# privacy-scaling-explorations/zkevm-specs

Measured on AMD Instinct MI355X. Metric: BN254 constraint-rows/sec, higher is better.
Workload: dtype u256 (BN254 Fr: 4xu64 canonical cells, u32-limb Montgomery); 1 GPU; EVM circuit, 2^18 execution steps per GPU, mixed-opcode synthetic trace (BASELINE configs[2]); RW table 816377 rows, bytecode table 43913 rows; steps_per_gpu=262144, rw_rows=816377, bytecode_rows=43913, witness_copies=3

## Files before the change

### zkevm_specs_amd/csrc/cpu_backend.cpp

```cpp
#include <stdio.h>
#include <string.h>
#include <chrono>
#include <functional>
#include <string>
#include <vector>

#include "../../include/zkevm_hip.h"
#include "dist_tally.hpp"
#include "state_circuit.hpp"
#include "evm_circuit.hpp"
#include "host_index.hpp"
#include "row_circuits.hpp"
#include "copy_circuit.hpp"
#include "sign_circuit.hpp"
#include "keccak_table.hpp"
#include "secp256k1.hpp"
#include "pi_circuit.hpp"
#include "state_assign.hpp"
#include "bytecode_assign.hpp"
#include "state_rekey.hpp"
#include "ecc_circuit.hpp"
#include "withdrawal_circuit.hpp"
#include "tx_assign.hpp"
#include "sig_assign.hpp"
// ... 42 lines not shown
    std::function<u32(u64)> row;
    std::vector<u32> status;
    u32 launches = 0;
    double ms = 0;
    u64 fail_count = 0, first_row = ~0ull;
    u32 first_code = 0;
    bool range_ok = false;
    bool range_may_be_empty = false;
    std::vector<u64> a64[4];
    std::vector<u32> a32[4];
    std::vector<uint8_t> a8, a8b;
    std::vector<uint16_t> a16;
    std::vector<u64> w64[4];
    std::vector<u32> out32;
    void (*pass)(zk_session*) = nullptr;
    int assign_kind = 0;
    u64 n_ops = 0;
    std::vector<u32> rekey_plan;
    std::vector<u32> rekey_jobs;
    u64 n_mpt = 0;
    CpuTable tab[12];
    std::vector<u64> keccak_rows;
    StateArgs state;
    EvmArgs evm;
    BytecodeArgs bytecode;
    ExpArgs exp;
    CopyArgs copy;
    SignArgs sign;
    PiArgs pi;
    PiCopyArgs picopy;
    AssignArgs assign;
    BcaArgs bca;
    std::vector<BcaChunk> bca_chunks;
    std::vector<uint8_t> bca_map;
    CpaArgs cpa;
    CpaPlan cpa_plan;
    EcdsaArgs ecdsa;
    KeccakGenArgs kgen;
    TxAssignArgs txa;
    SigAssignArgs sga;
    std::vector<u64> sga64[8];
    std::vector<u32> sga32[3];
    u64 n_sig_rows = 0;
    ExaArgs exa;
    ExaSizes exa_sizes;
    PiaArgs pia;
    PiaSizes pia_sizes;
    KeccakGenArgs pia_kgen;
    EccArgs ecc_assign;
    std::vector<u64> pia64[20];
    std::vector<u32> pia32[6];
    std::vector<uint8_t> pia8[4];
    std::vector<u64> txa_out64[4];
    std::vector<u32> txa_out32[3];
    u64 n_keccak = 0;
    ZkRwMeta rw_meta;
    HostCodeDir dir;
    std::vector<u64> aux64;
    bool status_external = false;
};

static void run_pass(zk_session* s, u32* status_out) {
    const auto t0 = std::chrono::steady_clock::now();
    u32* st = status_out ? status_out : s->status.data();
    const long long lo = (long long)s->lo, hi = (long long)s->hi;
    if (s->pass) {
        s->pass(s);
        if (status_out) memcpy(status_out, s->status.data(), s->n * sizeof(u32));
    } else {
#pragma omp parallel for schedule(dynamic, 256)
        for (long long i = lo; i < hi; i++) st[i] = s->row((u64)i);
    }
    u64 fails = 0, first = ~0ull;
    for (long long i = lo; i < hi; i++)
        if (st[i]) {
            if (!fails) first = (u64)i;
            fails++;
        }
    s->fail_count = fails;
    s->first_row = first;
    s->first_code = fails ? st[first] : 0u;
    s->ms += std::chrono::duration<double, std::milli>(std::chrono::steady_clock::now() - t0).count();
    s->launches++;
}
extern "C" int zk_launch(zk_session* s, uint32_t* status_dev) {
    ARG_TRY(s, "zk_launch: null session");
    s->status_external = status_dev != nullptr;
    run_pass(s, status_dev);
    return 0;
}
extern "C" int zk_collect(zk_session* s, zk_result* r) {
    ARG_TRY(s && r, "zk_collect: bad arguments");
    r->fail_count = s->fail_count;
    r->first_fail_row = s->first_row == ~0ull ? UINT64_MAX : s->first_row;
    r->first_fail_code = s->first_code;
    r->launches = s->launches;
    r->rows_evaluated = s->hi - s->lo;
    r->kernel_ms = s->launches ? s->ms / s->launches : 0.0;
    s->launches = 0;
    s->ms = 0;
    return 0;
}
extern "C" int zk_read_status(zk_session* s, uint32_t* status_host) {
    ARG_TRY(s && status_host, "zk_read_status: bad arguments");
    ARG_TRY(!s->status_external, "zk_read_status: the last pass wrote its statuses to the caller's status_dev buffer, not the session's");
    memcpy(status_host, s->status.data(), s->n * sizeof(u32));
    return 0;
}
extern "C" int zk_close(zk_session* s) {
    delete s;
    return 0;
}
extern "C" int zk_session_set_stream(zk_session*, void*) { return 0; }
extern "C" int zk_session_timing(zk_session*, double* open_ms, double* span_ms) {
    if (open_ms) *open_ms = -1.0;
    if (span_ms) *span_ms = -1.0;
    return 0;
}
struct zk_comm {
    int rank = 0, world = 1;
    void* nccl = nullptr;
    std::vector<uint64_t> buf;
};
#define RCCL_TRY(expr, what)                                                                                                                   \
    do {                                                                                                                                       \
        const int r_ = (expr);                                                                                                                 \
        if (r_ != 0) {                                                                                                                         \
            char buf_[256];                                                                                                                    \
            snprintf(buf_, sizeof buf_, "%s: RCCL error %d (%s)", what, r_, zkdist::rccl().GetErrorString ? zkdist::rccl().GetErrorString(r_) : "?"); \
            g_err = buf_;                                                                                                                      \
            return -3;                                                                                                                         \
        }                                                                                                                                      \
    } while (0)
static bool host_collective() { return getenv("ZK_RCCL_LIB") && zkdist::rccl().ok && zkdist::rccl().named_by_env && zkdist::rccl().buffers == 0; }
extern "C" int zk_dist_unique_id(uint8_t* id) {
    ARG_TRY(id, "zk_dist_unique_id: id is null");
    memset(id, 0, ZK_DIST_ID_BYTES);
    if (host_collective()) {
        zkdist::RcclId u;
        RCCL_TRY(zkdist::rccl().GetUniqueId(&u), "ncclGetUniqueId");
        memcpy(id, u.internal, ZK_DIST_ID_BYTES);
    }
    return 0;
}
extern "C" int zk_dist_close(zk_comm* c) {
    if (c && c->nccl) (void)zkdist::rccl().CommDestroy(c->nccl);
    delete c;
    return 0;
}
extern "C" int zk_dist_init(const uint8_t* id, int rank, int world, zk_comm** out) {
    ARG_TRY(id && out && world >= 1 && rank >= 0 && rank < world, "zk_dist_init: bad arguments");
    ARG_TRY(world == 1 || host_collective(),
            "zk_dist_init: the CPU backend has no collective of its own (world must be 1, or ZK_RCCL_LIB must name a library that gathers host buffers); reduce on the host");
    zk_comm* c = new zk_comm();
    c->rank = rank;
    c->world = world;
    c->buf.assign((size_t)(world + 1) * zkdist::TALLY_WORDS, 0);
    if (world > 1) {
        zkdist::RcclId u;
        memcpy(u.internal, id, ZK_DIST_ID_BYTES);
        if (int r = zkdist::rccl().CommInitRank(&c->nccl, world, u, rank)) {
            char buf[256];
            snprintf(buf, sizeof buf, "ncclCommInitRank: RCCL error %d", r);
            g_err = buf;
            c->nccl = nullptr;
            zk_dist_close(c);
            return -3;
        }
    }
    *out = c;
    return 0;
}
extern "C" int zk_dist_tally(zk_comm* c, const zk_result* local, uint64_t row_offset, zk_result* global) {
    ARG_TRY(c && local && global, "zk_dist_tally: bad arguments");
    uint64_t* mine = c->buf.data();
    uint64_t* all = mine + zkdist::TALLY_WORDS;
    zkdist::tally_pack(mine, local, row_offset);
    if (c->world == 1) memcpy(all, mine, zkdist::TALLY_WORDS * sizeof(uint64_t));
    else RCCL_TRY(zkdist::rccl().AllGather(mine, all, zkdist::TALLY_WORDS, zkdist::RCCL_UINT64, c->nccl, nullptr), "ncclAllGather");
    zkdist::tally_reduce(all, c->world, local, global);
    return 0;
}
extern "C" int zk_last_host_phases(double* us4) {
    if (us4) for (int k = 0; k < 4; k++) us4[k] = -1.0;
    return 0;
}
extern "C" int zk_timing_sums(double* sums_ms, uint64_t* count, int) {
    if (sums_ms) for (int k = 0; k < 3; k++) sums_ms[k] = -1.0;
    if (count) *count = 0;
    return 0;
}
extern "C" int zk_last_timing(double* open_ms, double* pass_ms, double* span_ms) {
    if (open_ms) *open_ms = -1.0;
    if (pass_ms) *pass_ms = -1.0;
    if (span_ms) *span_ms = -1.0;
    return 0;
}
extern "C" int zk_set_range(zk_session* s, uint64_t row_lo, uint64_t row_hi) {
    ARG_TRY(s && s->range_ok, "zk_set_range: not a row-circuit session");
    ARG_TRY((row_lo < row_hi || (s->range_may_be_empty && row_lo == row_hi)) && row_hi <= s->n, "zk_set_range: bad range");
    s->lo = row_lo;
    s->hi = row_hi;
    std::fill(s->status.begin(), s->status.end(), 0u);
    return 0;
}
extern "C" int zk_state_set_range(zk_session* s, uint64_t row_lo, uint64_t row_hi) { return zk_set_range(s, row_lo, row_hi); }

static zk_session* new_session(u64 n, bool range_ok) {
    zk_session* s = new zk_session();
    s->n = n;
    s->lo = 0;
    s->hi = n;
    s->status.assign(n ? n : 1, 0u);
    s->range_ok = range_ok;
    return s;
}
static int one_shot(zk_session* s, uint32_t* status_out, zk_result* result) {
    int rc = zk_launch(s, nullptr);
    if (!rc) rc = zk_collect(s, result);
    if (!rc && status_out) rc = zk_read_status(s, status_out);
    zk_close(s);
    return rc;
}
#define NO_DEVICE_PTRS(opts, name) ARG_TRY(!((opts) & ZK_OPT_DEVICE_PTRS), name ": ZK_OPT_DEVICE_PTRS has no meaning on the CPU backend")
#ifndef ZK_OPT_STATE_COMPACT
#define ZK_OPT_STATE_COMPACT 32u
#endif

extern "C" int zk_fr_op(int op, const uint64_t* a, const uint64_t* b, uint64_t* out, uint64_t n, uint32_t opts) {
    NO_DEVICE_PTRS(opts, "zk_fr_op");
    ARG_TRY(a && b && out, "zk_fr_op: null pointer");
    ARG_TRY(op < 19 || op > 25 || n % 12 == 0, "zk_fr_op 19..25: n must be a multiple of 12");
#pragma omp parallel for
    for (long long i = 0; i < (long long)n; i++) {
        const Fr x = fr_load(a + 4 * i), y = fr_load(b + 4 * i);
        Fr r;
        switch (op) {
        case 0: r = fr_add(x, y); break;
        case 1: r = fr_sub(x, y); break;
        case 2: r = fr_mul(x, y); break;
        case 3: r = fr_mont(x, y); break;
        case 4: r = fr_neg(x); break;
        case 5: r = fr_inv(x); break;
        case 6: r = fr_div(x, y); break;
        case 18: r = ecc_fq_mul_hook(x, y); break;
        case 26: r = sp_sqrt_p(x); break;
        case 27: r = sp_inv_p(x); break;
        case 19: case 20: case 21: case 22: case 23: case 24: case 25:
            if (i % 12 == 0 && i + 12 <= (long long)n) ecc_fq12_op_hook(op, a + 4 * i, b + 4 * i, out + 4 * i);
            continue;
        default: r = fr_zero();
        }
        for (int k = 0; k < 4; k++) out[4 * i + k] = (u64)r.v[2 * k] | ((u64)r.v[2 * k + 1] << 32);
    }
    return 0;
}

extern "C" int zk_state_open(const uint64_t* rows, const uint32_t* flags, uint64_t n, const uint64_t* mpt, uint64_t n_mpt,
                             uint32_t opts, zk_session** out) {
    NO_DEVICE_PTRS(opts, "zk_state_open");
    ARG_TRY(out && rows && n > 0 && n < (1ull << 32) && n_mpt < (1ull << 31), "zk_state_open: bad arguments");
    zk_session* s = new_session(n, true);
    const bool compact = opts & ZK_OPT_STATE_COMPACT;
    s->a64[0].assign(rows, rows + n * (compact ? 15 : ST_NCELLS) * 4);
    s->state.rows.skip = compact ? 42u : 0u;
    if (flags) s->a32[0].assign(flags, flags + n);
    else s->a32[0].assign(n, 0u);
    cpu_table(s->tab[0], mpt, nullptr, n_mpt, MPT_NCELLS, nullptr);
    {
        CpuTable& h = s->tab[0];
        for (u32 r = 0; r < (u32)n_mpt; r++) {
            const u64 hv = state_mpt_key_hash(h.t, r);
            u32 k = (u32)hv & h.t.mask;
            while (h.slots[k] != ZK_EMPTY_SLOT) k = (k + 1) & h.t.mask;
            h.slots[k] = state_mpt_slot_value(h.t, r, hv);
        }
    }
    s->state.rows.cells = s->a64[0].data();
    s->state.rows.flags = s->a32[0].data();
    s->state.rows.n = n;
    s->state.mpt = s->tab[0].t;
    s->state.eval_lo = 0;
    s->state.eval_hi = n;
    s->row = [s](u64 i) { return state_check_row(s->state, i); };
    *out = s;
    return 0;
}
extern "C" int zk_state_verify(const uint64_t* rows, const uint32_t* flags, uint64_t n, const uint64_t* mpt, uint64_t n_mpt,
                               uint32_t opts, uint32_t* status_out, zk_result* result) {
    ARG_TRY(result, "zk_state_verify: result is null");
    zk_session* s = nullptr;
    const int rc = zk_state_open(rows, flags, n, mpt, n_mpt, opts, &s);
    return rc ? rc : one_shot(s, status_out, result);
}

extern "C" int zk_evm_open(const zk_evm_tables* t, uint32_t opts, zk_session** out) {
    NO_DEVICE_PTRS(opts, "zk_evm_open");
    ARG_TRY(t && out && t->steps && t->n_steps >= 2 && t->n_steps < (1ull << 32), "zk_evm_open: bad arguments");
    ARG_TRY(t->aux_cells == 0 || (t->aux_cells >= 2 && t->aux_cells <= 64), "zk_evm_open: aux_cells must be 0 (= 2) or 2..64");
    zk_session* s = new_session(t->n_steps - 1, false);
    EvmArgs& a = s->evm;
    s->a64[0].assign(t->steps, t->steps + t->n_steps * STEP_NCELLS * 4);
    a.dyn = nullptr;
    a.step_recs = nullptr;
    a.defer_list = nullptr;
    a.defer_count = nullptr;
    a.steps = s->a64[0].data();
    a.n_steps = t->n_steps;
    cpu_table(s->tab[0], t->rw, t->rw_flags, t->n_rw, RW_NCELLS, rw_key_hash);
    cpu_table(s->tab[1], t->bytecode, nullptr, t->n_bytecode, BYTECODE_NCELLS, bc_key_hash);
    cpu_table(s->tab[2], t->tx, t->tx_flags, t->n_tx, TX_NCELLS, tx_key_hash);
    cpu_table(s->tab[3], t->block, t->block_flags, t->n_block, BLOCK_NCELLS, blk_key_hash);
    cpu_table(s->tab[4], t->copy, nullptr, t->n_copy, COPY_T_NCELLS, copy_key_hash);
    cpu_table(s->tab[5], t->keccak, nullptr, t->n_keccak, KECCAK_NCELLS, keccak_key_hash);
    cpu_table(s->tab[6], t->exp, nullptr, t->n_exp, EXP_T_NCELLS, expt_key_hash);
    cpu_table(s->tab[7], t->sig, nullptr, t->n_sig, SIG_T_NCELLS, sig_key_hash);
    cpu_table(s->tab[8], t->ecc, nullptr, t->n_ecc, ECC_T_NCELLS, ecc_key_hash);
    cpu_table(s->tab[9], t->withdrawals, nullptr, t->n_withdrawals, 4, nullptr);
    a.rw = s->tab[0].t; a.bytecode = s->tab[1].t; a.tx = s->tab[2].t; a.block = s->tab[3].t; a.copy = s->tab[4].t;
    a.keccak = s->tab[5].t; a.exp = s->tab[6].t; a.sig = s->tab[7].t; a.ecc = s->tab[8].t; a.withdrawals = s->tab[9].t;
    {
        const HostEvmAgg g = evm_aggregates_host(t->tx, t->tx_flags, t->n_tx, t->withdrawals, t->n_withdrawals);
        a.agg_max_txs = g.max_txs; a.agg_total_txs = g.total_txs; a.agg_invalid_txs = g.invalid_txs;
        a.agg_bad_invalid_rows = g.bad_invalid_rows; a.agg_total_wds = g.total_wds;
        a.agg_rw_dups = rw_duplicate_rows_host(t->rw, t->n_rw);
    }
    a.aux = nullptr;
    a.aux_kind = nullptr;
    a.aux_cells = t->aux_cells ? t->aux_cells : 2u;
    if (t->aux && t->aux_kind) {
        s->aux64.assign(t->aux, t->aux + t->n_steps * a.aux_cells * 4);
        s->a32[1].assign(t->aux_kind, t->aux_kind + t->n_steps);
        a.aux = s->aux64.data();
        a.aux_kind = s->a32[1].data();
    }
    a.perm = nullptr;
    a.prof = nullptr;
    a.n_pairs = (u32)(t->n_steps - 1);
    a.opts = (t->begin_with_first_step ? 1u : 0u) | (t->end_with_last_step ? 2u : 0u);
    a.rw_dense = 0;
    a.rw_base = 0;
    a.rw_keys = nullptr;
    a.codes.n = 0;
    a.codes.mask = 0;
    a.codes.packed = nullptr;
    a.codes.entries = nullptr;
    a.codes.slots = nullptr;
    if (!(opts & ZK_OPT_GENERIC_INDEX)) {
        s->rw_meta = rw_dense_meta_host(s->tab[0].t.n ? s->tab[0].cells.data() : nullptr, t->n_rw);
        a.rw_dense = s->rw_meta.dense;
        a.rw_base = s->rw_meta.base;
        if (s->rw_meta.dense) {
            s->a64[1].resize((size_t)t->n_rw * 4);
            for (u64 r = 0; r < t->n_rw; r++) {
                const RwKey k = rw_pack_row(a.rw, (u32)r);
                for (int j = 0; j < 4; j++) s->a64[1][4 * r + j] = k.w[j];
            }
            a.rw_keys = s->a64[1].data();
        }
        if (t->n_bytecode) {
            build_code_dir(s->tab[1].cells.data(), t->n_bytecode, s->dir);
            a.codes.entries = s->dir.entries.data();
            a.codes.slots = s->dir.slots.data();
            a.codes.mask = s->dir.mask;
            a.codes.n = (u32)s->dir.entries.size();
            a.codes.packed = s->dir.packed.data();
        }
    }
    s->row = [s](u64 i) {
        u32 c = evm_check_step<EVM_GROUP_ALL>(s->evm, i);
        if (c == ZK_NOT_MINE) c = evm_check_step<EVM_GROUP_WARM>(s->evm, i);
        if (c == ZK_NOT_MINE) c = evm_check_step<EVM_GROUP_COLD>(s->evm, i);
        return c;
    };
    *out = s;
    return 0;
}
extern "C" int zk_evm_verify(const zk_evm_tables* t, uint32_t opts, uint32_t* status_out, zk_result* result) {
    ARG_TRY(result, "zk_evm_verify: result is null");
    zk_session* s = nullptr;
    const int rc = zk_evm_open(t, opts, &s);
    return rc ? rc : one_shot(s, status_out, result);
}

extern "C" int zk_evm_verify_batch(const zk_evm_tables* const* t, uint64_t n, uint32_t opts, zk_result* results) {
    ARG_TRY((t && results) || n == 0, "zk_evm_verify_batch: bad arguments");
    for (uint64_t i = 0; i < n; i++) ARG_TRY(t[i], "zk_evm_verify_batch: null witness");
    for (uint64_t i = 0; i < n; i++) {
        const int rc = zk_evm_verify(t[i], opts, nullptr, &results[i]);
        if (rc) return rc;
    }
    return 0;
}

extern "C" int zk_bytecode_open(const uint64_t* rows, uint64_t n, const uint64_t* keccak, uint64_t n_keccak, const uint64_t* randomness,
                                uint32_t opts, zk_session** out) {
    NO_DEVICE_PTRS(opts, "zk_bytecode_open");
    ARG_TRY(out && rows && randomness && n > 0 && n < (1ull << 32) && n_keccak < (1ull << 31), "zk_bytecode_open: bad arguments");
    zk_session* s = new_session(n, true);
    s->a64[0].assign(rows, rows + n * BC_NCELLS * 4);
    cpu_table(s->tab[0], keccak, nullptr, n_keccak, KECCAK_NCELLS, keccak_key_hash);
    s->bytecode.rows.cells = s->a64[0].data();
    s->bytecode.rows.flags = nullptr;
    s->bytecode.rows.n = n;
    s->bytecode.keccak = s->tab[0].t;
    s->bytecode.r = cell_of(randomness);
    s->bytecode.r_mont = nullptr;
    s->row = [s](u64 i) { return bytecode_check_row(s->bytecode, i); };
    *out = s;
    return 0;
}
extern "C" int zk_bytecode_verify(const uint64_t* rows, uint64_t n, const uint64_t* keccak, uint64_t n_keccak, const uint64_t* randomness,
                                  uint32_t opts, uint32_t* status_out, zk_result* result) {
    ARG_TRY(result, "zk_bytecode_verify: result is null");
    zk_session* s = nullptr;
    const int rc = zk_bytecode_open(rows, n, keccak, n_keccak, randomness, opts, &s);
    return rc ? rc : one_shot(s, status_out, result);
}
extern "C" int zk_exp_open(const uint64_t* rows, uint64_t n, uint32_t opts, zk_session** out) {
    NO_DEVICE_PTRS(opts, "zk_exp_open");
    ARG_TRY(out && rows && n > 0 && n < (1ull << 32), "zk_exp_open: bad arguments");
    zk_session* s = new_session(n, true);
    s->a64[0].assign(rows, rows + n * EX_NCELLS * 4);
    s->exp.rows.cells = s->a64[0].data();
    s->exp.rows.flags = nullptr;
    s->exp.rows.n = n;
    s->row = [s](u64 i) { return exp_check_row(s->exp, i); };
    *out = s;
    return 0;
}
extern "C" int zk_exp_verify(const uint64_t* rows, uint64_t n, uint32_t opts, uint32_t* status_out, zk_result* result) {
    ARG_TRY(result, "zk_exp_verify: result is null");
    zk_session* s = nullptr;
    const int rc = zk_exp_open(rows, n, opts, &s);
    return rc ? rc : one_shot(s, status_out, result);
}

extern "C" int zk_copy_open(const zk_copy_tables* t, uint32_t opts, zk_session** out) {
    NO_DEVICE_PTRS(opts, "zk_copy_open");
    ARG_TRY(t && out && t->rows && t->randomness && t->n_rows > 0 && t->n_rows < (1ull << 32), "zk_copy_open: bad arguments");
    zk_session* s = new_session(t->n_rows, true);
    s->a64[0].assign(t->rows, t->rows + t->n_rows * CP_NCELLS * 4);
    if (t->row_flags) s->a32[0].assign(t->row_flags, t->row_flags + t->n_rows);
    cpu_table(s->tab[0], t->rw, t->rw_flags, t->n_rw, RW_NCELLS, rw_key_hash);
    cpu_table(s->tab[1], t->bytecode, nullptr, t->n_bytecode, BYTECODE_NCELLS, bc_key_hash);
    cpu_table(s->tab[2], t->tx, t->tx_flags, t->n_tx, TX_NCELLS, tx_key_hash);
    s->copy.rows.cells = s->a64[0].data();
    s->copy.rows.flags = t->row_flags ? s->a32[0].data() : nullptr;
    s->copy.rows.n = t->n_rows;
    s->copy.rw = s->tab[0].t;
    s->copy.bytecode = s->tab[1].t;
    s->copy.tx = s->tab[2].t;
    s->rw_meta = rw_dense_meta_host(t->n_rw ? s->tab[0].cells.data() : nullptr, t->n_rw);
    s->copy.rw_meta = (opts & ZK_OPT_GENERIC_INDEX) ? nullptr : &s->rw_meta;
    s->copy.r = cell_of(t->randomness);
    s->row = [s](u64 i) { return copy_check_row(s->copy, i); };
    *out = s;
    return 0;
}
extern "C" int zk_copy_verify(const zk_copy_tables* t, uint32_t opts, uint32_t* status_out, zk_result* result) {
    ARG_TRY(result, "zk_copy_verify: result is null");
    zk_session* s = nullptr;
    const int rc = zk_copy_open(t, opts, &s);
    return rc ? rc : one_shot(s, status_out, result);
}

extern "C" int zk_sign_open(const zk_sign_units* t, uint32_t opts, zk_session** out) {
    NO_DEVICE_PTRS(opts, "zk_sign_open");
    ARG_TRY(t && out && t->bytes && t->cells && t->meta && t->randomness && t->n_units > 0 && t->n_units < (1ull << 32), "zk_sign_open: bad arguments");
    const u64 n = t->n_units;
    zk_session* s = new_session(n, true);
    s->a8.assign(t->bytes, t->bytes + n * SG_NBYTES_ROWS * 32);
    s->a64[0].assign(t->cells, t->cells + n * SG_NCELLS * 4);
    s->a32[0].assign(t->meta, t->meta + n * 4);
    cpu_table(s->tab[0], t->keccak, nullptr, t->n_keccak, KECCAK_NCELLS, keccak_key_hash);
    cpu_table(s->tab[1], t->tx_rows, t->tx_flags, t->n_tx_rows, TX_NCELLS, nullptr);
    SignArgs& a = s->sign;
    a.bytes = s->a8.data();
    a.cells.cells = s->a64[0].data();
    a.cells.flags = nullptr;
    a.cells.n = n;
    a.meta = s->a32[0].data();
    a.keccak = s->tab[0].t;
    a.tx_rows = s->tab[1].t;
    a.tx_rows.n = (u32)t->n_tx_rows;
    a.r = cell_of(t->randomness);
    s->a64[1].resize(64 * 4);
    sign_fill_rpow(a.r, s->a64[1].data());
    a.rpow = s->a64[1].data();
    a.is_sig = t->is_sig ? 1u : 0u;
    s->row = [s](u64 i) { return sign_check_unit(s->sign, i); };
    *out = s;
    return 0;
}
extern "C" int zk_sign_verify(const zk_sign_units* t, uint32_t opts, uint32_t* status_out, zk_result* result) {
    ARG_TRY(result, "zk_sign_verify: result is null");
    zk_session* s = nullptr;
    const int rc = zk_sign_open(t, opts, &s);
    return rc ? rc : one_shot(s, status_out, result);
}

extern "C" int zk_pi_open(const uint64_t* rows, uint64_t n, const uint64_t* keccak, uint64_t n_keccak, const uint64_t* gas, uint64_t n_gas,
                          uint64_t circuit_len, const uint64_t* keccak_rand, const uint64_t* byte_pow_base, uint32_t opts, zk_session** out) {
    NO_DEVICE_PTRS(opts, "zk_pi_open");
    ARG_TRY(out && rows && keccak_rand && byte_pow_base && n > 0 && n < (1ull << 32), "zk_pi_open: bad arguments");
    zk_session* s = new_session(n, true);
    s->a64[0].assign(rows, rows + n * 24 * 4);
    cpu_table(s->tab[0], keccak, nullptr, n_keccak, KECCAK_NCELLS, keccak_key_hash);
    cpu_table(s->tab[1], gas, nullptr, n_gas, PI_GAS_NCELLS, pi_gas_key_hash);
    PiArgs& a = s->pi;
    a.rows.cells = s->a64[0].data();
    a.rows.flags = nullptr;
    a.rows.n = n;
    a.keccak = s->tab[0].t;
    a.gas = s->tab[1].t;
    a.keccak_rand_m = fr_to_mont(cell_of(keccak_rand));
    a.byte_pow_base_m = fr_to_mont(cell_of(byte_pow_base));
    a.circuit_len = fr_from_u64(circuit_len);
    s->row = [s](u64 i) { return pi_check_row(s->pi, i); };
    *out = s;
    return 0;
}
extern "C" int zk_pi_verify(const uint64_t* rows, uint64_t n, const uint64_t* keccak, uint64_t n_keccak, const uint64_t* gas, uint64_t n_gas,
                            uint64_t circuit_len, const uint64_t* keccak_rand, const uint64_t* byte_pow_base, uint32_t opts,
                            uint32_t* status_out, zk_result* result) {
    ARG_TRY(result, "zk_pi_verify: result is null");
    zk_session* s = nullptr;
    const int rc = zk_pi_open(rows, n, keccak, n_keccak, gas, n_gas, circuit_len, keccak_rand, byte_pow_base, opts, &s);
    return rc ? rc : one_shot(s, status_out, result);
}

extern "C" int zk_pi_copy_open(const uint64_t* cells, const uint8_t* bytes, const uint32_t* lens, uint64_t n, uint32_t opts, zk_session** out) {
    NO_DEVICE_PTRS(opts, "zk_pi_copy_open");
    ARG_TRY(out && cells && bytes && lens && n > 0 && n < (1ull << 32), "zk_pi_copy_open: bad arguments");
    zk_session* s = new_session(n, false);
    s->a64[0].assign(cells, cells + n * 4);
    s->a8.assign(bytes, bytes + n * 32);
    s->a32[0].assign(lens, lens + n);
    s->picopy.cells = s->a64[0].data();
    s->picopy.bytes = s->a8.data();
    s->picopy.lens = s->a32[0].data();
    s->picopy.n = n;
    s->row = [s](u64 i) { return pi_copy_check(s->picopy, i); };
    *out = s;
    return 0;
}
extern "C" int zk_pi_copy_verify(const uint64_t* cells, const uint8_t* bytes, const uint32_t* lens, uint64_t n, uint32_t opts, uint32_t* status_out,
                                 zk_result* result) {
    ARG_TRY(result, "zk_pi_copy_verify: result is null");
    zk_session* s = nullptr;
    const int rc = zk_pi_copy_open(cells, bytes, lens, n, opts, &s);
    return rc ? rc : one_shot(s, status_out, result);
}

extern "C" int zk_keccak_open(const uint8_t* data, uint64_t n_bytes, const uint64_t* offsets, uint64_t n_msgs, const uint64_t* randomness,
                              uint32_t mode, uint64_t* rows_dev, uint32_t opts, zk_session** out) {
    NO_DEVICE_PTRS(opts, "zk_keccak_open");
    ARG_TRY(out && offsets && randomness && n_msgs > 0 && n_msgs < (1ull << 32) && (data || n_bytes == 0) && mode <= 1u && !rows_dev,
            "zk_keccak_open: bad arguments");
    for (u64 k = 0; k < n_msgs; k++) ARG_TRY(offsets[k] <= offsets[k + 1], "zk_keccak_open: offsets must be non-decreasing");
    ARG_TRY(offsets[n_msgs] <= n_bytes, "zk_keccak_open: offsets exceed the data buffer");
    zk_session* s = new_session(n_msgs, false);
    s->a8.assign(data, data + n_bytes);
    s->a64[0].assign(offsets, offsets + n_msgs + 1);
    s->a64[1].resize(KT_RPOW_ROWS * 4);
    kt_fill_rpow(cell_of(randomness), s->a64[1].data());
    s->keccak_rows.assign(n_msgs * KT_NCELLS * 4, 0);
    KeccakGenArgs& g = s->kgen;
    g.data = s->a8.data();
    g.offsets = s->a64[0].data();
    g.n = n_msgs;
    g.rpow = s->a64[1].data();
    g.rows = s->keccak_rows.data();
    g.mode = mode;
    g.long_list = nullptr;
    g.long_count = nullptr;
    s->row = [s](u64 i) { return keccak_table_row(s->kgen, i); };
    *out = s;
    return 0;
}
extern "C" int zk_keccak_read_rows(zk_session* s, uint64_t* rows_host) {
    ARG_TRY(s && rows_host && !s->keccak_rows.empty(), "zk_keccak_read_rows: bad arguments");
    memcpy(rows_host, s->keccak_rows.data(), s->keccak_rows.size() * 8);
    return 0;
}
extern "C" int zk_keccak_table(const uint8_t* data, uint64_t n_bytes, const uint64_t* offsets, uint64_t n_msgs, const uint64_t* randomness,
                               uint32_t mode, uint64_t* rows_out, uint32_t opts, uint32_t* status_out, zk_result* result) {
    ARG_TRY(result && rows_out, "zk_keccak_table: null output");
    zk_session* s = nullptr;
    int rc = zk_keccak_open(data, n_bytes, offsets, n_msgs, randomness, mode, nullptr, opts, &s);
    if (rc) return rc;
    rc = zk_launch(s, nullptr);
    if (!rc) rc = zk_collect(s, result);
    if (!rc) rc = zk_keccak_read_rows(s, rows_out);
    if (!rc && status_out) rc = zk_read_status(s, status_out);
    zk_close(s);
    return rc;
}

extern "C" int zk_ecdsa_open_batches(const zk_ecdsa_batch* bt, uint32_t n_batches, uint32_t opts, zk_session** out) {
    NO_DEVICE_PTRS(opts, "zk_ecdsa_open_batches");
    ARG_TRY(out && bt && (n_batches == 1 || n_batches == 2), "zk_ecdsa_open_batches: one or two batches");
    u64 n = 0;
    for (u32 k = 0; k < n_batches; k++) {
        ARG_TRY(bt[k].bytes && bt[k].n > 0 && bt[k].n < (1ull << 31) && bt[k].layout <= 2u && (!bt[k].v || bt[k].v_stride >= 1) && !bt[k].out_dev,
                "zk_ecdsa_open: bad arguments");
// ... 1056 lines not shown
```

### zkevm_specs_amd/csrc/evm_circuit.hpp

```cpp
#pragma once
#include "common.hpp"
#include "evm_tables.h"
#include "keccak.hpp"
#include "secp_constants.h"
#include "bigz.hpp"

enum { S_STATE = 0, S_RWC, S_CALL_ID, S_IS_ROOT, S_IS_CREATE, S_CH_LO, S_CH_HI, S_PC, S_SP, S_GAS, S_MWS, S_REV, S_LOG, STEP_NCELLS };
enum { R_RWC = 0, R_RW, R_TAG, R_ID, R_ADDR, R_FT, R_KEY_LO, R_KEY_HI, R_VAL_LO, R_VAL_HI, R_PREV_LO, R_PREV_HI, R_AUX_LO, R_AUX_HI, RW_NCELLS };
enum { B_HASH_LO = 0, B_HASH_HI, B_TAG, B_INDEX, B_IS_CODE, B_VALUE, BYTECODE_NCELLS };
enum { TX_NCELLS = 5, BLOCK_NCELLS = 4 };
enum { CT_IS_FIRST = 0, CT_SRC_ID_LO, CT_SRC_ID_HI, CT_SRC_TAG, CT_DST_ID_LO, CT_DST_ID_HI, CT_DST_TAG, CT_SRC_ADDR,
       CT_SRC_ADDR_END, CT_DST_ADDR, CT_LENGTH, CT_RLC_ACC, CT_RWC, CT_RWC_INC, COPY_T_NCELLS };
enum { XT_IS_STEP = 0, XT_ID, XT_IS_LAST, XT_BASE0, XT_BASE1, XT_BASE2, XT_BASE3, XT_EXP_LO, XT_EXP_HI, XT_RES_LO, XT_RES_HI,
       EXP_T_NCELLS };
enum { SIG_T_NCELLS = 9, ECC_T_NCELLS = 13 };
enum { AUX_PAIR = 3, AUX_ECRECOVER = 5, AUX_ECADD = 6, AUX_ECMUL = 7, AUX_ECPAIRING = 8 };
enum { CDT_Bytecode = 1, CDT_Memory, CDT_TxCalldata, CDT_TxLog, CDT_RlcAcc };

struct EvmDyn {
    u32 rw_sparse;
    u32 codes_n;
    u64 rw_base;
    u32 codes_mask;
    u32 agg_max_txs, agg_total_txs, agg_invalid_txs, agg_bad_invalid_rows, agg_total_wds;
    u32 dir_entries;
    u32 n_deferred;
    u32 agg_rw_dups;
};

struct EvmArgs {
    const EvmDyn* dyn;
    const u64* steps;
    const u32* step_recs;
    u64 n_steps;
    ZkTable rw, bytecode, tx, block;
    ZkTable copy, keccak, exp;
    ZkTable sig, ecc;
    ZkTable withdrawals;
    u32 agg_max_txs, agg_total_txs, agg_invalid_txs, agg_bad_invalid_rows, agg_total_wds;
    u32 agg_rw_dups;
    const u64* aux;
    const u32* aux_kind;
    u32 aux_cells;
    u32 rw_dense;
    u64 rw_base;
    const u64* rw_keys;
    ZkCodeDir codes;
    unsigned long long* prof;
    u32* defer_list;
    u32* defer_count;
    const u32* perm;
    u32 n_pairs;
    u32 opts;
    u32* defer_count_twin;
};

ZK_HD void evm_args_resolve(EvmArgs& a) {
#ifdef EVM_RESOLVE_OFF
    return;
#endif
    if (a.dyn) {
        const EvmDyn d = *a.dyn;
        a.rw_dense = (a.rw.n != 0u && d.rw_sparse == 0u) ? 1u : 0u;
        a.rw_base = d.rw_base;
        a.codes.n = d.codes_n;
        a.codes.mask = d.codes_mask;
        a.agg_max_txs = d.agg_max_txs; a.agg_total_txs = d.agg_total_txs; a.agg_invalid_txs = d.agg_invalid_txs;
        a.agg_bad_invalid_rows = d.agg_bad_invalid_rows; a.agg_total_wds = d.agg_total_wds;
        a.agg_rw_dups = d.agg_rw_dups;
    }
}

#ifndef EVM_HOT_BLOCK
#define EVM_HOT_BLOCK 128
#endif
#define EVM_STAGE_LANES EVM_HOT_BLOCK
#define EV_PROF_WAVE ((blockIdx.x * blockDim.x + threadIdx.x) >> 6)
#define EV_PROF_ON(a) ((a).prof && (threadIdx.x & 63) == 0 && EV_PROF_WAVE < 4096u)
#define EVM_STAGE_STRIDE (EVM_STAGE_LANES + 1)
#define EVM_STAGE_ENTRIES 40
#define EVM_STAGE_GAS 10
ZK_HD constexpr int evm_stage_entry(int s, int c) {
    return c == S_CH_LO || c == S_CH_HI ? 24 + s * 8 + (c - S_CH_LO) * 4
           : s * 12 + (c < S_CH_LO ? c : c == S_PC ? 5 : c == S_SP ? 6 : c == S_MWS ? 7 : c == S_REV ? 8 : c == S_LOG ? 9 : EVM_STAGE_GAS);
}
#define EVM_DIR_MAX_SLOTS 128
#define EVM_DIR_MAX_ENTRIES 32
#define EVM_DIR_SLOT_U64 (EVM_DIR_MAX_SLOTS / 2)
#define EVM_DIR_LDS_U64 (EVM_DIR_SLOT_U64 + EVM_DIR_MAX_ENTRIES * 12)
#if defined(ZK_HOSTSIM)
typedef const u64* EVM_LDS_PTR;
typedef const u32* EVM_LDS32_PTR;
#else
typedef const __attribute__((address_space(3))) u64* EVM_LDS_PTR;
typedef const __attribute__((address_space(3))) u32* EVM_LDS32_PTR;
#endif

struct Word {
    Fr lo, hi;
};
struct WordOrValue {
    Word w;
    bool is_word;
};

#ifndef EVM_FAST
#define EVM_FAST 0
#endif
struct Ins {
    const EvmArgs* a;
    u32 defer;
    u64 idx;
    u32 err;
    u32 seq;
    u64 rw_off;
    u32 pc_off;
    int sp_off;
    Fr rwc, call_id, sp, pc;
    u32 code_state, code_header_row, code_byte_base, code_n_bytes, code_header_ok;
    u64 code_header_value;
    EVM_LDS32_PTR stage;
    EVM_LDS_PTR dir_lds;
    u32 pre_op;
    bool pre_op_ok;
    u32 op_info, op_info_byte;
};

#if defined(ZK_HOSTSIM)
#define EV_PROF(I, k) do { } while (0)
#else
#define EV_PROF(I, k) do { if (EV_PROF_ON(*(I).a)) (I).a->prof[EV_PROF_WAVE * 8 + (k)] = __builtin_readcyclecounter(); } while (0)
#endif

ZK_HD void ev_fail(Ins& I, u32 kind) {
    if (I.err == 0u) I.err = ZK_CODE(kind, I.seq);
}
ZK_HD void ev_require(Ins& I, bool cond, u32 kind = ZK_ASSERT) {
    I.seq++;
    const u32 take = (cond ? 0u : 1u) & (I.err == 0u ? 1u : 0u);
    I.err = take ? ZK_CODE(kind, I.seq) : I.err;
}
#define EV_TRY(stmt) do { stmt; if (I.err) return; } while (0)
#define EV_TRYV(stmt, ret) do { stmt; if (I.err) return ret; } while (0)

ZK_HD Fr ev_step_cell(const EvmArgs& a, u64 step, int c) { return fr_load(a.steps + (step * STEP_NCELLS + c) * 4); }
ZK_HD Fr ev_staged_cell(const Ins& I, int s, int c) {
    Fr r = fr_zero();
    const int e = evm_stage_entry(s, c);
    const int n = (c == S_CH_LO || c == S_CH_HI) ? 4 : c == S_GAS ? 2 : 1;
#pragma unroll
    for (int w = 0; w < n; w++) r.v[w] = I.stage[(e + w) * EVM_STAGE_STRIDE];
    return r;
}
#if EVM_FAST
ZK_HD Fr ev_curr(const Ins& I, int c) { return ev_staged_cell(I, 0, c); }
ZK_HD Fr ev_next(const Ins& I, int c) { return ev_staged_cell(I, 1, c); }
#else
ZK_HD Fr ev_curr(const Ins& I, int c) { return I.stage ? ev_staged_cell(I, 0, c) : ev_step_cell(*I.a, I.idx, c); }
ZK_HD Fr ev_next(const Ins& I, int c) { return I.stage ? ev_staged_cell(I, 1, c) : ev_step_cell(*I.a, I.idx + 1, c); }
#endif
ZK_HD Fr fr_u(u64 x) { return fr_from_u64(x); }
ZK_HD Word word_of(const Fr& lo, const Fr& hi) {
    Word w;
    w.lo = lo;
    w.hi = hi;
    return w;
}
ZK_HD Word word_zero() { return word_of(fr_zero(), fr_zero()); }
ZK_HD bool word_eq(const Word& a, const Word& b) { return fr_eq(a.lo, b.lo) && fr_eq(a.hi, b.hi); }

ZK_HD void constrain_zero(Ins& I, const Fr& v) { ev_require(I, fr_is_zero(v)); }
ZK_HD void constrain_equal(Ins& I, const Fr& a, const Fr& b) { ev_require(I, fr_eq(a, b)); }
ZK_HD void constrain_equal_word(Ins& I, const Word& a, const Word& b) { ev_require(I, word_eq(a, b)); }
ZK_HD void range_check(Ins& I, const Fr& v, int n_bytes) { ev_require(I, fr_byte_len(v) <= n_bytes, ZK_CONSTRAINT); }
ZK_HD Fr value_of(Ins& I, const WordOrValue& v) {
    ev_require(I, !v.is_word);
    return v.w.lo;
}
ZK_HD bool word_cells_fit(const Word& w) { return fr_fits128(w.lo) && fr_fits128(w.hi); }
ZK_HD U256 to_u256(Ins& I, const Word& w) {
    ev_require(I, word_cells_fit(w), ZK_OVERFLOW_ERROR);
    return u256_from_lo_hi(w.lo, w.hi);
}
ZK_HD U256 int_value(Ins& I, const Word& w) {
#if EVM_FAST
    if (!word_cells_fit(w)) I.defer = 1u;
#else
    if (!word_cells_fit(w) && I.err == 0u) I.err = ZK_CODE(ZK_UNSUPPORTED, I.seq);
#endif
    return u256_from_lo_hi(w.lo, w.hi);
}
ZK_HD bool words_wide(Ins& I, const Word& a, const Word& b, const Word& c, const Word& d) {
    const bool wide = !(word_cells_fit(a) && word_cells_fit(b) && word_cells_fit(c) && word_cells_fit(d));
#if EVM_FAST
    if (wide) I.defer = 1u;
    return false;
#else
    return wide;
#endif
}
ZK_HD bool words_wide(Ins& I, const Word& a, const Word& b, const Word& c) { return words_wide(I, a, b, c, c); }
ZK_HD bool words_wide(Ins& I, const Word& a, const Word& b) { return words_wide(I, a, b, b, b); }
ZK_HD bool words_wide(Ins& I, const Word& a) { return words_wide(I, a, a, a, a); }
ZK_HD bool word_is_zero_int(const Word& w) { return fr_is_zero(w.lo) && fr_is_zero(w.hi); }
ZK_HD Word word_from_u256(const U256& v) { return word_of(u256_lo(v), u256_hi(v)); }
ZK_HD Word word_from_int(Ins& I, const U256& v, bool neg = false, bool too_big = false) {
    I.seq++;
    if (too_big) ev_fail(I, ZK_ASSERT);
    else if (neg) ev_fail(I, ZK_OVERFLOW_ERROR);
    return word_from_u256(v);
}
#if !EVM_FAST
ZK_HD WideRes wide_words(u32 op, const Word& x0, const Word& x1, const Word& x2, const Word& x3) {
    return wide_witness(op, x0.lo, x0.hi, x1.lo, x1.hi, x2.lo, x2.hi, x3.lo, x3.hi);
}
ZK_HD Word word_from_wide(Ins& I, const WideRes& W, int k) { return word_from_int(I, W.o[k], (W.fl[k] & 1u) != 0u, (W.fl[k] & 2u) != 0u); }
#endif
ZK_HD U256 int_bytes32(Ins& I, const Word& w) {
    if (word_cells_fit(w)) return u256_from_lo_hi(w.lo, w.hi);
#if EVM_FAST
    I.defer = 1u;
    return fr_zero();
#else
    const WideRes W = wide_words(WIDE_INT256, w, w, w, w);
    if ((W.fl[0] & 2u) && I.err == 0u) I.err = ZK_CODE(ZK_OVERFLOW_ERROR, I.seq);
    return W.o[0];
#endif
}
ZK_HD Word word_checked(Ins& I, const Fr& lo, const Fr& hi) {
    ev_require(I, fr_fits128(lo) && fr_fits128(hi));
    return word_of(lo, hi);
}
ZK_HD void ev_compare(Ins& I, const Fr& lhs, const Fr& rhs, int n_bytes, u32& lt, u32& eq) {
    ev_require(I, fr_byte_len(lhs) <= n_bytes && fr_byte_len(rhs) <= n_bytes);
    lt = fr_lt(lhs, rhs);
    eq = fr_eq(lhs, rhs);
}
ZK_HD void compare_word(Ins& I, const Word& a, const Word& b, u32& lt, u32& eq) {
    u32 hl, he, ll, le;
    ev_compare(I, a.hi, b.hi, 16, hl, he);
    ev_compare(I, a.lo, b.lo, 16, ll, le);
    lt = hl + he * ll;
    eq = he * le;
}
ZK_HD bool ev_select(Ins& I, const Fr& cond) {
    ev_require(I, fr_le_u64(cond, 1));
    return fr_eq_u64(cond, 1);
}
ZK_HD bool ev_select_b(Ins& I, u32 cond01) {
    I.seq++;
    return cond01 == 1u;
}
ZK_HD u32 is_zero_word(const Word& w) { return fr_is_zero(fr_add(w.lo, w.hi)); }
ZK_HD u32 is_equal_word(const Word& a, const Word& b) {
    return fr_is_zero(fr_add(fr_sub(a.lo, b.lo), fr_sub(a.hi, b.hi)));
}
ZK_HD u32 fr_mod_small(const Fr& x, u32 m) {
    u64 rem = 0;
    for (int k = 7; k >= 0; k--) rem = ((rem << 32) | x.v[k]) % m;
    return (u32)rem;
}
ZK_HD Word evm_empty_code_hash() {
    return word_of(fr_from_u128(0x7bfad8045d85a470ull, 0xe500b653ca82273bull), fr_from_u128(0x927e7db2dcc703c0ull, 0xc5d2460186f7233cull));
}
ZK_HD Fr word_to_fq(Ins& I, const Word& w, int n_bytes) {
    U256 v = to_u256(I, w);
    bool hi_zero = true;
    for (int b = n_bytes; b < 32; b++) hi_zero = hi_zero && fr_byte(v, b) == 0;
    ev_require(I, hi_zero, ZK_CONSTRAINT);
    Fr r = fr_zero();
    for (int b = 0; b < n_bytes; b++) r.v[b >> 2] |= fr_byte(v, b) << (8 * (b & 3));
    return r;
}

ZK_HD u64 rw_key_hash_cell(const Fr& rwc) { return zk_hash_cell(0x51ed27u, rwc); }
ZK_HD u64 rw_key_hash(const ZkTable& t, u32 r) { return rw_key_hash_cell(zk_table_cell(t, r, R_RWC)); }
ZK_HD u64 bc_key_hash_cells(const Fr& lo, const Fr& hi, const Fr& tag, const Fr& index) {
    return zk_hash_cell(zk_hash_cell(zk_hash_cell(zk_hash_cell(0xb7e15u, lo), hi), tag), index);
}
ZK_HD u64 bc_key_hash(const ZkTable& t, u32 r) {
    return bc_key_hash_cells(zk_table_cell(t, r, 0), zk_table_cell(t, r, 1), zk_table_cell(t, r, 2), zk_table_cell(t, r, 3));
}
ZK_HD u64 tx_key_hash_cells(const Fr& a, const Fr& b, const Fr& c) {
    return zk_hash_cell(zk_hash_cell(zk_hash_cell(0x7f4a7u, a), b), c);
}
ZK_HD u64 tx_key_hash(const ZkTable& t, u32 r) {
    return tx_key_hash_cells(zk_table_cell(t, r, 0), zk_table_cell(t, r, 1), zk_table_cell(t, r, 2));
}
ZK_HD u64 blk_key_hash_cells(const Fr& a, const Fr& b) { return zk_hash_cell(zk_hash_cell(0x3c6efu, a), b); }
ZK_HD u64 blk_key_hash(const ZkTable& t, u32 r) { return blk_key_hash_cells(zk_table_cell(t, r, 0), zk_table_cell(t, r, 1)); }

ZK_HD u64 copy_key_hash_cells(const Fr& rwc, const Fr& src_addr) { return zk_hash_cell(zk_hash_cell(0xc09fu, rwc), src_addr); }
ZK_HD u64 copy_key_hash(const ZkTable& t, u32 r) { return copy_key_hash_cells(zk_table_cell(t, r, CT_RWC), zk_table_cell(t, r, CT_SRC_ADDR)); }
ZK_HD u64 expt_key_hash_cells(const Fr& id, const Fr& is_last, const Fr& exp_lo) { return zk_hash_cell(zk_hash_cell(zk_hash_cell(0xe4b7u, id), is_last), exp_lo); }
ZK_HD u64 sig_key_hash_cells(const Fr& msg_lo, const Fr& r_lo, const Fr& s_lo) { return zk_hash_cell(zk_hash_cell(zk_hash_cell(0x516u, msg_lo), r_lo), s_lo); }
ZK_HD u64 sig_key_hash(const ZkTable& t, u32 r) { return sig_key_hash_cells(zk_table_cell(t, r, 0), zk_table_cell(t, r, 3), zk_table_cell(t, r, 5)); }
ZK_HD u64 ecc_key_hash_cells(const Fr& op, const Fr& px_lo, const Fr& qx_lo, const Fr& input_rlc) {
    return zk_hash_cell(zk_hash_cell(zk_hash_cell(zk_hash_cell(0xecc0u, op), px_lo), qx_lo), input_rlc);
}
ZK_HD u64 ecc_key_hash(const ZkTable& t, u32 r) {
    return ecc_key_hash_cells(zk_table_cell(t, r, 0), zk_table_cell(t, r, 1), zk_table_cell(t, r, 5), zk_table_cell(t, r, 9));
}
ZK_HD u64 expt_key_hash(const ZkTable& t, u32 r) { return expt_key_hash_cells(zk_table_cell(t, r, XT_ID), zk_table_cell(t, r, XT_IS_LAST), zk_table_cell(t, r, XT_EXP_LO)); }


ZK_NOINLINE u64 table_probe_generic(ZkTable t, u64 h, const Fr* q, u32 mask) {
    u32 found = ZK_EMPTY_SLOT;
    bool ambiguous = false;
    if (t.n != 0) {
        u32 slot = (u32)h & t.mask;
        for (u32 probes = 0; probes <= t.mask; probes++) {
            const u32 r = t.slots[slot];
            if (r == ZK_EMPTY_SLOT) break;
            bool m = true;
            for (u32 c = 0; c < t.ncells; c++)
                if ((mask >> c) & 1u) m = m && fr_eq(zk_table_cell(t, r, c), q[c]);
            if (m) {
                if (found == ZK_EMPTY_SLOT) found = r;
                else if (!rows_identical(t, found, r)) ambiguous = true;
            }
            slot = (slot + 1) & t.mask;
        }
    }
    if (found == ZK_EMPTY_SLOT) return (u64)ZK_LOOKUP_UNSAT << 32;
    return (u64)found | (ambiguous ? ((u64)ZK_LOOKUP_AMBIGUOUS << 32) : 0ull);
}
template <int NCELLS>
ZK_HD u32 table_lookup(Ins& I, const ZkTable& t, u64 h, const Fr (&q)[NCELLS], u32 mask) {
#if EVM_FAST
    I.defer = 2u;
    I.seq++;
    return 0u;
#endif
    I.seq++;
    Fr tmp[NCELLS];
    for (int c = 0; c < NCELLS; c++) tmp[c] = ((mask >> c) & 1u) ? q[c] : fr_zero();
    const u64 res = table_probe_generic(t, h, tmp, mask);
    const u32 kind = (u32)(res >> 32);
    if (kind) ev_fail(I, kind);
    return kind == ZK_LOOKUP_UNSAT ? 0u : (u32)res;
}

template <int NCELLS, u32 MASK>
ZK_HD u32 table_lookup_inline(Ins& I, const ZkTable& t, u64 h, const Fr (&q)[NCELLS], Fr* out0 = nullptr, int out0_cell = 0, Fr* out1 = nullptr,
                              int out1_cell = 0) {
#if EVM_FAST
    if (out0) *out0 = fr_zero();
    if (out1) *out1 = fr_zero();
    I.defer = 2u;
    I.seq++;
    return 0u;
#endif
#ifdef ZK_WARM_GENERIC_LOOKUP
    {
        const u32 rg = table_lookup<NCELLS>(I, t, h, q, MASK);
        if (out0) *out0 = zk_table_cell(t, rg, out0_cell);
        if (out1) *out1 = zk_table_cell(t, rg, out1_cell);
        return rg;
    }
#endif
    I.seq++;
    u32 kind;
    const u32 found = table_probe_inline<NCELLS, MASK>(t, h, q, kind, out0, out0_cell, out1, out1_cell);
    if (kind == (u32)ZK_LOOKUP_UNSAT) { ev_fail(I, ZK_LOOKUP_UNSAT); return 0u; }
    if (kind) ev_fail(I, ZK_LOOKUP_AMBIGUOUS);
    return found;
}
// ... 4111 lines not shown
```

### zkevm_specs_amd/csrc/zkevm_hip.hip

```cpp
#include <hip/hip_runtime.h>
#include <hip/hip_ext.h>
#include <stdio.h>
#include <string.h>
#include <stdlib.h>
#include <chrono>
#include <string>
#include <vector>

#include <atomic>
#include <mutex>
#include <dlfcn.h>

#include "../../include/zkevm_hip.h"
#include "kernels.hpp"
#include "dist_tally.hpp"
#include "host_index.hpp"
#include "code_dir_build.hpp"

#define ZK_MAX_DEVICES 64
#define ZK_ECDSA_CHUNK_LANES (1ull << 17)
static std::mutex g_dev_mutex;
static hipStream_t g_own_stream[ZK_MAX_DEVICES] = {nullptr};
static hipStream_t g_batch_stream[ZK_MAX_DEVICES][2] = {{nullptr}};
static hipStream_t g_side_stream[ZK_MAX_DEVICES] = {nullptr};

static u32* g_secp_comb[ZK_MAX_DEVICES] = {nullptr};
static void* g_zero_row[ZK_MAX_DEVICES] = {nullptr};
static thread_local int t_device = -1;
static thread_local hipStream_t t_stream = nullptr;
static thread_local std::string g_err;
static thread_local double t_host_phase[4] = {0, 0, 0, 0};
static thread_local double t_timing_sum[3] = {0, 0, 0};
static thread_local uint64_t t_timing_count = 0;
static thread_local double t_timing[3] = {0, 0, 0};

#define HIP_TRY(expr)                                                                         \
    do {                                                                                      \
        hipError_t e_ = (expr);                                                               \
        if (e_ != hipSuccess) {                                                               \
            char buf_[512];                                                                   \
            snprintf(buf_, sizeof buf_, "%s failed: %s (%s:%d)", #expr, hipGetErrorString(e_), \
                     __FILE__, __LINE__);                                                     \
            g_err = buf_;                                                                     \
            return -(int)e_ - 1000;                                                           \
        }                                                                                     \
    } while (0)
#define ARG_TRY(cond, msg)  \
    do {                    \
        if (!(cond)) {      \
            g_err = msg;    \
            return -1;      \
        }                   \
    } while (0)

extern "C" const char* zk_last_error(void) { return g_err.c_str(); }

__attribute__((constructor)) static void zk_default_hw_queues() { setenv("GPU_MAX_HW_QUEUES", "16", 0); }
static void arena_release_all();

static hipStream_t g_block_stream[ZK_MAX_DEVICES][4] = {{nullptr}};
static int block_streams_ensure(int device) {
    for (int c = 0; c < 4; c++)
        if (!g_block_stream[device][c]) {
            int lo = 0, hi = 0;
            (void)hipDeviceGetStreamPriorityRange(&lo, &hi);
            static const bool state_low = [] { const char* e = getenv("ZK_BLOCK_STATE_PRIO"); return !(e && e[0] == 'h'); }();
            static const bool flat = [] { const char* e = getenv("ZK_BLOCK_PRIO"); return e && e[0] == 'n'; }();
            if (flat) HIP_TRY(hipStreamCreateWithFlags(&g_block_stream[device][c], hipStreamNonBlocking));
            else HIP_TRY(hipStreamCreateWithPriority(&g_block_stream[device][c], hipStreamNonBlocking, (c == 0) == state_low ? lo : hi));
        }
    return 0;
}
extern "C" int zk_init(int device) {
    int count = 0;
    HIP_TRY(hipGetDeviceCount(&count));
    ARG_TRY(device >= 0 && device < count && device < ZK_MAX_DEVICES, "zk_init: no such HIP device");
    HIP_TRY(hipSetDevice(device));
    hipStream_t own;
    {
        std::lock_guard<std::mutex> lock(g_dev_mutex);
        if (!g_own_stream[device]) {
            HIP_TRY(hipStreamCreateWithFlags(&g_own_stream[device], hipStreamNonBlocking));
            static const bool lazy = [] { const char* e = getenv("ZK_BLOCK_STREAMS_LAZY"); return e && e[0] == '1'; }();
            if (!lazy) { int brc = block_streams_ensure(device); if (brc) return brc; }
        }
        own = g_own_stream[device];
        if (!g_zero_row[device]) {
            HIP_TRY(hipMalloc(&g_zero_row[device], 512));
            HIP_TRY(hipMemset(g_zero_row[device], 0, 512));
        }
    }
    if (t_device != device || !t_stream) t_stream = own;
    t_device = device;
    return 0;
}
extern "C" void zk_shutdown(void) {
    arena_release_all();
    std::lock_guard<std::mutex> lock(g_dev_mutex);
    for (int d = 0; d < ZK_MAX_DEVICES; d++)
        if (g_own_stream[d]) {
            if (hipSetDevice(d) == hipSuccess) {
                (void)hipStreamDestroy(g_own_stream[d]);
                if (g_zero_row[d]) (void)hipFree(g_zero_row[d]);
                if (g_secp_comb[d]) (void)hipFree(g_secp_comb[d]);
                g_secp_comb[d] = nullptr;
            }
            for (int k = 0; k < 2; k++) {
                if (g_batch_stream[d][k]) (void)hipStreamDestroy(g_batch_stream[d][k]);
                g_batch_stream[d][k] = nullptr;
            }
            if (g_side_stream[d]) (void)hipStreamDestroy(g_side_stream[d]);
            g_side_stream[d] = nullptr;
            for (int k = 0; k < 4; k++) {
                if (g_block_stream[d][k]) (void)hipStreamDestroy(g_block_stream[d][k]);
                g_block_stream[d][k] = nullptr;
            }
            g_own_stream[d] = nullptr;
            g_zero_row[d] = nullptr;
        }
    t_stream = nullptr;
    t_device = -1;
}
extern "C" int zk_set_stream(void* st) {
    ARG_TRY(t_device >= 0, "zk_set_stream: call zk_init first");
    t_stream = st ? (hipStream_t)st : g_own_stream[t_device];
    return 0;
}
struct zk_session;
static int session_rebind_stream(zk_session* s, hipStream_t st);
extern "C" int zk_session_set_stream(zk_session* s, void* st) {
    ARG_TRY(s, "zk_session_set_stream: null session");
    return session_rebind_stream(s, (hipStream_t)st);
}

__global__ void tally_reset_kernel(ZkTally* t, u32* counter = nullptr) {
    t[threadIdx.x].fail_count = 0ull;
    t[threadIdx.x].first_fail = ~0ull;
    if (counter && threadIdx.x == 0) *counter = 0u;
}


__global__ void slots_fill_kernel(u32* slots, u32 n) {
    u32 i = blockIdx.x * blockDim.x + threadIdx.x;
    if (i < n) slots[i] = ZK_EMPTY_SLOT;
}

template <u64 (*HASH)(const ZkTable&, u32)>
__global__ void index_build_kernel(ZkTable t, u32* slots, const ZkRwMeta* unless_dense = nullptr) {
    u32 r = blockIdx.x * blockDim.x + threadIdx.x;
    if (r >= t.n || (unless_dense && unless_dense->dense)) return;
    u32 s = (u32)HASH(t, r) & t.mask;
    while (atomicCAS(&slots[s], ZK_EMPTY_SLOT, r) != ZK_EMPTY_SLOT) s = (s + 1) & t.mask;
}
__global__ void slots_fill_unless_dense_kernel(u32* slots, u32 n, const ZkRwMeta* unless_dense) {
    u32 i = blockIdx.x * blockDim.x + threadIdx.x;
    if (i < n && !unless_dense->dense) slots[i] = ZK_EMPTY_SLOT;
}
__global__ void mpt_index_build_kernel(ZkTable t, u32* slots) {
    u32 r = blockIdx.x * blockDim.x + threadIdx.x;
    if (r >= t.n) return;
    const u64 h = state_mpt_key_hash(t, r);
    u32 s = (u32)h & t.mask;
    const u32 v = state_mpt_slot_value(t, r, h);
    while (atomicCAS(&slots[s], ZK_EMPTY_SLOT, v) != ZK_EMPTY_SLOT) s = (s + 1) & t.mask;
}
__global__ void rw_dense_check_kernel(ZkTable t, ZkRwMeta* meta) {
    const u32 r = blockIdx.x * blockDim.x + threadIdx.x;
    if (r >= t.n) return;
    const u64* p = t.cells + (u64)r * RW_NCELLS * 4;
    const u64* p0 = t.cells;
    const u64 base = p0[0];
    const bool ok = (p0[1] | p0[2] | p0[3]) == 0 && (p[1] | p[2] | p[3]) == 0 && p[0] == base + r && base + r >= base;
    if (r == 0) meta->base = base;
    if (!ok) atomicAnd(&meta->dense, 0u);
}

struct EvmSortArgs {
    const u64* steps;
    u32 n_pairs;
    u32* hist;
    u32* hist_next;
    u32* taken;
    uint16_t* bin16;
    u32* group_start;
    u32* perm;
    ZkTally* tally;
    u32* defer_count;
    u32* early_host;
    u32 early_seq;
};
#define EVM_EARLY_WORD 36u
__device__ __forceinline__ void evm_state_hist_body(u32 vblock, const u64* steps, u32 n_pairs, u32* hist, u32* taken, uint16_t* bin16, ZkTally* tally,
                                                    u32* defer_count) {
    __shared__ u32 local[EVM_N_BINS];
    if (vblock == 0) {
        if (threadIdx.x == 0 && defer_count) *defer_count = 0u;
        if (threadIdx.x == 0) {
            tally->fail_count = 0ull;
            tally->first_fail = ~0ull;
        }
        for (u32 k = threadIdx.x; k < EVM_N_BINS; k += blockDim.x) taken[k] = 0;
    }
    for (u32 k = threadIdx.x; k < EVM_N_BINS; k += blockDim.x) local[k] = 0;
    __syncthreads();
    u32 i = vblock * blockDim.x + threadIdx.x;
    if (i < n_pairs) {
        const u32 bin = evm_state_bin((u32)steps[((u64)i * STEP_NCELLS + S_STATE) * 4]);
        bin16[i] = (uint16_t)bin;
        atomicAdd(&local[bin], 1u);
    }
    __syncthreads();
    for (u32 k = threadIdx.x; k < EVM_N_BINS; k += blockDim.x)
        if (local[k]) atomicAdd(&hist[k], local[k]);
}
__global__ void evm_state_hist_kernel(const u64* steps, u32 n_pairs, u32* hist, u32* taken, uint16_t* bin16, ZkTally* tally, u32* defer_count) {
    evm_state_hist_body(blockIdx.x, steps, n_pairs, hist, taken, bin16, tally, defer_count);
}
__device__ __forceinline__ void evm_state_scatter_body(u32 vblock, const uint16_t* bin16, u32 n_pairs, const u32* hist, u32* hist_next,
                                                       u32* taken, u32* group_start, u32* perm, u32* early_host = nullptr, u32 early_seq = 0u) {
    __shared__ u32 sa[EVM_N_BINS], sb[EVM_N_BINS];
    __shared__ u32 local[EVM_N_BINS];
    __shared__ u32 base[EVM_N_BINS];
    __shared__ u32 gsh[EVM_N_GROUPS + 1];
    const u32 k = threadIdx.x;
    u32 c = 0, c_real = 0;
    if (k < EVM_N_BINS) {
        c_real = hist[k];
        c = k < (u32)EVM_GROUP_WARM * 128u ? ((c_real + 63u) & ~63u) : c_real;
        sa[k] = c;
        local[k] = 0;
        if (vblock == 0) hist_next[k] = 0;
    }
    __syncthreads();
    u32* src = sa;
    u32* dst = sb;
    for (u32 off = 1; off < EVM_N_BINS; off <<= 1) {
        if (k < EVM_N_BINS) dst[k] = src[k] + (k >= off ? src[k - off] : 0u);
        __syncthreads();
        u32* t = src; src = dst; dst = t;
    }
    u32 excl = 0;
    if (k < EVM_N_BINS) {
        excl = src[k] - c;
        if (vblock == 0) {
            if ((k & 127u) == 0) group_start[k >> 7] = gsh[k >> 7] = excl;
            if (k == EVM_N_BINS - 1) group_start[EVM_N_GROUPS] = gsh[EVM_N_GROUPS] = src[k];
            for (u32 j = c_real; j < c; j++) perm[excl + j] = EVM_NO_PAIR;
        }
    }
    const u32 i = vblock * blockDim.x + threadIdx.x;
    u32 bin = 0, rank = 0;
    if (i < n_pairs) {
        bin = bin16[i];
        rank = atomicAdd(&local[bin], 1u);
    }
    __syncthreads();
    if (vblock == 0 && k == 0 && early_host) {
        __hip_atomic_store(&early_host[EVM_EARLY_WORD], gsh[EVM_GROUP_WARM + 1] - gsh[EVM_GROUP_WARM], __ATOMIC_RELAXED, __HIP_MEMORY_SCOPE_SYSTEM);
        __hip_atomic_store(&early_host[EVM_EARLY_WORD + 1], gsh[EVM_GROUP_COLD + 1] - gsh[EVM_GROUP_COLD], __ATOMIC_RELAXED, __HIP_MEMORY_SCOPE_SYSTEM);
        __threadfence_system();
        __hip_atomic_store(&early_host[EVM_EARLY_WORD + 2], early_seq, __ATOMIC_RELEASE, __HIP_MEMORY_SCOPE_SYSTEM);
    }
    if (k < EVM_N_BINS && local[k]) base[k] = excl + atomicAdd(&taken[k], local[k]);
    __syncthreads();
    if (i < n_pairs) perm[base[bin] + rank] = i;
}
__global__ __launch_bounds__(1024) void evm_state_scatter_kernel(const uint16_t* bin16, u32 n_pairs, const u32* hist, u32* hist_next,
                                                                 u32* taken, u32* group_start, u32* perm) {
    evm_state_scatter_body(blockIdx.x, bin16, n_pairs, hist, hist_next, taken, group_start, perm);
}
__global__ __launch_bounds__(256) void evm_open_fill_kernel(uint4* ff, u64 n_ff, uint4* zero, u64 n_zero) {
    const u64 stride = (u64)gridDim.x * blockDim.x;
    const uint4 F = make_uint4(~0u, ~0u, ~0u, ~0u), Z = make_uint4(0u, 0u, 0u, 0u);
    for (u64 i = (u64)blockIdx.x * blockDim.x + threadIdx.x; i < n_ff; i += stride) ff[i] = F;
    for (u64 i = (u64)blockIdx.x * blockDim.x + threadIdx.x; i < n_zero; i += stride) zero[i] = Z;
}
__device__ __forceinline__ void rw_prepare_quad(const ZkTable& t, u64* keys, EvmDyn* dyn, u32 vthread) {
    const u32 r = vthread >> 2, q = vthread & 3u;
    const bool in = r < t.n;
    uint4 c0 = make_uint4(0, 0, 0, 0), c1 = c0, c2 = c0;
    u64 base = 0;
    u32 flags = 3u;
    if (in) {
        const uint4* p = reinterpret_cast<const uint4*>(t.cells + (u64)r * RW_NCELLS * 4) + q;
        c0 = p[0];
        c1 = p[4];
        c2 = p[8];
        if (q == 0) {
            base = t.cells[0];
            if (t.flags) flags = t.flags[r];
        }
    }
    bool fit, dense_ok;
    u64 w0 = 0, w1 = 0, w2 = 0, w3 = 0;
    const bool z0hi = (c0.y | c0.z | c0.w) == 0u, z1hi = (c1.y | c1.z | c1.w) == 0u, z2hi = (c2.y | c2.z | c2.w) == 0u;
    const bool z0 = z0hi && c0.x == 0u, z1 = z1hi && c1.x == 0u, z2 = z2hi && c2.x == 0u;
    if (q == 0) {
        const u64 rwc = (u64)c0.x | ((u64)c0.y << 32);
        dense_ok = (c0.z | c0.w) == 0u && rwc == base + r && base + r >= base;
        fit = z1hi && c1.x <= 255u;
        w0 = (u64)(c1.x & 0xffu) << 8 | ((u64)(flags & 3u) << 56) | (1ull << 63);
        w2 = (u64)c2.x | ((u64)c2.y << 32);
        w3 = (u64)c2.z | ((u64)c2.w << 32);
    } else if (q == 1) {
        dense_ok = z0;
        fit = z1 && z2hi;
        w0 = (u64)c2.x << 24;
    } else if (q == 2) {
        dense_ok = true;
        fit = z0hi && c0.x <= 255u && (c1.z | c1.w) == 0u && z2hi && c2.x <= 255u;
        w0 = (u64)(c0.x & 0xffu) | ((u64)(c2.x & 0xffu) << 16);
        w1 = (u64)c1.x | ((u64)c1.y << 32);
    } else {
        dense_ok = true;
        fit = z0 && z1 && z2;
    }
    const u32 qshift = threadIdx.x & 60u;
    const bool fits = ((__ballot(fit) >> qshift) & 0xfull) == 0xfull;
    const unsigned long long nd = __ballot(in && !dense_ok);
    if (nd != 0ull && (threadIdx.x & 63u) == 0) atomicOr(&dyn->rw_sparse, 1u);
    if (r == 0 && q == 0 && in) dyn->rw_base = base;
#pragma unroll
    for (int m = 1; m <= 2; m <<= 1) {
        w0 |= __shfl_xor(w0, m);
        w1 |= __shfl_xor(w1, m);
        w2 |= __shfl_xor(w2, m);
        w3 |= __shfl_xor(w3, m);
    }
    if (!fits) w0 = w1 = w2 = w3 = 0;
    if (in && q < 2) {
        const u64 a = q == 0 ? w0 : w2, b2 = q == 0 ? w1 : w3;
        reinterpret_cast<uint4*>(keys + (u64)r * 4)[q] = make_uint4((u32)a, (u32)(a >> 32), (u32)b2, (u32)(b2 >> 32));
    }
}
#define EVM_OPEN_TABLES 8
struct EvmOpenTables {
    ZkTable t[EVM_OPEN_TABLES];
    u32 block_start[EVM_OPEN_TABLES + 2];
    const u64* wds;
    u32 n_wds;
    EvmDyn* dyn;
    ZkTally* tally;
    ZkTable rw;
    u64* rw_keys;
    u32 dir_block0, rw_block0;
    DirBuild dir;
    const u64* steps;
    u32 n_steps;
    u32* step_recs;
    u32 rec_block0;
    EvmSortArgs sort;
    u32 hist_block0;
    u32 lat_period;
#ifdef ZK_DIAG_P1
    u32 diag_skip;
#endif
};
__device__ __forceinline__ void evm_open_small_tables(const EvmOpenTables& o, u32 block) {
    int k = 0;
#pragma unroll
    for (int j = 1; j <= EVM_OPEN_TABLES; j++) k += block >= o.block_start[j] ? 1 : 0;
    const u32 r = (block - o.block_start[k]) * blockDim.x + threadIdx.x;
    if (k == EVM_OPEN_TABLES) {
        const bool nz = r < o.n_wds && !fr_is_zero(fr_load(o.wds + ((u64)r * 4 + 3) * 4));
        const unsigned long long b = __ballot(nz);
        if (b && (threadIdx.x & 63u) == 0) atomicAdd(&o.dyn->agg_total_wds, (u32)__popcll(b));
        return;
    }
    const ZkTable& t = o.t[k];
    const bool in = r < t.n;
    if (k == 0) {
        bool caller = false, present = false, invalid = false, bad = false;
        if (in) {
            const Fr tag = zk_table_cell(t, r, 1), lo = zk_table_cell(t, r, 3), hi = zk_table_cell(t, r, 4);
            caller = fr_eq_u64(tag, 4);
            present = caller && !(fr_is_zero(lo) && fr_is_zero(hi));
            const bool inv_row = fr_eq_u64(tag, 10);
            bad = inv_row && t.flags && (t.flags[r] & 1u);
            invalid = inv_row && fr_eq_u64(lo, 1);
        }
        const unsigned long long bc = __ballot(caller), bp = __ballot(present), bi = __ballot(invalid), bb = __ballot(bad);
        if ((threadIdx.x & 63u) == 0) {
            if (bc) atomicAdd(&o.dyn->agg_max_txs, (u32)__popcll(bc));
            if (bp) atomicAdd(&o.dyn->agg_total_txs, (u32)__popcll(bp));
            if (bi) atomicAdd(&o.dyn->agg_invalid_txs, (u32)__popcll(bi));
            if (bb) atomicOr(&o.dyn->agg_bad_invalid_rows, 1u);
        }
    }
    if (!in) return;
    u64 h;
    switch (k) {
    case 0: h = tx_key_hash(t, r); break;
    case 1: h = blk_key_hash(t, r); break;
    case 2: h = bc_key_hash(t, r); break;
    case 3: h = copy_key_hash(t, r); break;
    case 4: h = keccak_key_hash(t, r); break;
    case 5: h = expt_key_hash(t, r); break;
    case 6: h = sig_key_hash(t, r); break;
    default: h = ecc_key_hash(t, r); break;
    }
    u32* slots = const_cast<u32*>(t.slots);
    u32 s = (u32)h & t.mask;
    while (atomicCAS(&slots[s], ZK_EMPTY_SLOT, r) != ZK_EMPTY_SLOT) s = (s + 1) & t.mask;
}
__global__ __launch_bounds__(256) void evm_open_phase1_kernel(EvmOpenTables o) {
    if (blockIdx.x == 0 && threadIdx.x < 2) {
        o.tally[threadIdx.x].fail_count = 0ull;
        o.tally[threadIdx.x].first_fail = ~0ull;
    }
    u32 b = blockIdx.x;
    if (o.lat_period > 1u && b < o.rec_block0) {
        const u32 q = b / o.lat_period;
        b = (b == q * o.lat_period && q < o.rw_block0) ? q : o.rw_block0 + b - (q + 1u < o.rw_block0 ? q + 1u : o.rw_block0);
    }
#ifdef ZK_DIAG_P1
    {
        const u32 range = b < o.dir_block0 ? 1u : b < o.hist_block0 ? 2u : b < o.rw_block0 ? 4u : b < o.rec_block0 ? 8u : 16u;
        if (o.diag_skip & range) return;
    }
#endif
    if (b < o.dir_block0) evm_open_small_tables(o, b);
    else if (b < o.hist_block0) dirb_events_row(o.dir, (b - o.dir_block0) * blockDim.x + threadIdx.x);
    else if (b < o.rw_block0) evm_state_hist_body(b - o.hist_block0, o.sort.steps, o.sort.n_pairs, o.sort.hist, o.sort.taken, o.sort.bin16, o.sort.tally, o.sort.defer_count);
    else if (b < o.rec_block0) rw_prepare_quad(o.rw, o.rw_keys, o.dyn, (b - o.rw_block0) * blockDim.x + threadIdx.x);
    else evm_step_record_quad(o.steps, o.n_steps, o.step_recs, (b - o.rec_block0) * blockDim.x + threadIdx.x);
}
#define EVM_OPEN_RW_GENERIC_BLOCKS 64u
#define EVM_OPEN_P2_BLOCK 1024u
__global__ __launch_bounds__(1024) void evm_open_phase2_kernel(EvmOpenTables o, u32 scatter_blocks, u32 dir_blocks, u32 force_generic) {
    if (blockIdx.x < scatter_blocks) {
        evm_state_scatter_body(blockIdx.x, o.sort.bin16, o.sort.n_pairs, o.sort.hist, o.sort.hist_next, o.sort.taken, o.sort.group_start, o.sort.perm,
                               o.sort.early_host, o.sort.early_seq);
        return;
    }
    const u32 b = blockIdx.x - scatter_blocks;
    if (b < dir_blocks) {
        dirb_finalize_entry(o.dir, b * blockDim.x + threadIdx.x);
        return;
    }
    if (!force_generic && o.dyn->rw_sparse == 0u) return;
    if (force_generic && b == dir_blocks && threadIdx.x == 0) o.dyn->rw_sparse = 1u;
    u32* slots = const_cast<u32*>(o.rw.slots);
    const u32 stride = (gridDim.x - scatter_blocks - dir_blocks) * blockDim.x;
    for (u32 r = (b - dir_blocks) * blockDim.x + threadIdx.x; r < o.rw.n; r += stride) {
        u32 s = (u32)rw_key_hash(o.rw, r) & o.rw.mask;
        bool dup = false;
        for (;;) {
            const u32 q = atomicCAS(&slots[s], ZK_EMPTY_SLOT, r);
            if (q == ZK_EMPTY_SLOT) break;
            if (!dup && q < o.rw.n) {
                bool same = true;
                for (int c = 0; c < RW_NCELLS && same; c++) same = fr_eq(zk_table_cell(o.rw, q, c), zk_table_cell(o.rw, r, c));
                dup = same;
            }
            s = (s + 1) & o.rw.mask;
        }
        if (dup) atomicAdd(&o.dyn->agg_rw_dups, 1u);
    }
}

__global__ void fr_op_kernel(int op, const u64* a, const u64* b, u64* out, u64 n) {
    u64 i = (u64)blockIdx.x * blockDim.x + threadIdx.x;
    if (i >= n) return;
    Fr x = fr_load(a + 4 * i), y = fr_load(b + 4 * i), r;
    switch (op) {
    case 0: r = fr_add(x, y); break;
    case 1: r = fr_sub(x, y); break;
    case 2: r = fr_mul(x, y); break;
    case 3: r = fr_mont(x, y); break;
    case 4: r = fr_neg(x); break;
    case 5: r = fr_inv(x); break;
    case 6: r = fr_div(x, y); break;
    case 16: r = sp_mul_p(x, y); break;
    case 17: r = sp_sqr_p(x); break;
    case 18: r = ecc_fq_mul_hook(x, y); break;
    case 26: r = sp_sqrt_p(x); break;
    case 27: r = sp_inv_p(x); break;
    default: r = fr_zero();
    }
    for (int k = 0; k < 4; k++) out[4 * i + k] = (u64)r.v[2 * k] | ((u64)r.v[2 * k + 1] << 32);
}

__global__ __launch_bounds__(64) void evm_publish_kernel(const u32* d, u32* h, u32 seq) {
    const u32 i = threadIdx.x;
    if (i < 32u) __hip_atomic_store(&h[i], d[i], __ATOMIC_RELAXED, __HIP_MEMORY_SCOPE_SYSTEM);
    __threadfence_system();
    if (i == 0u) __hip_atomic_store(&h[32], seq, __ATOMIC_RELEASE, __HIP_MEMORY_SCOPE_SYSTEM);
}
struct EvmResultBlock {
    EvmDyn dyn;
    u32 n_deferred_twin;
    u32 pad0[(64 - sizeof(EvmDyn)) / 4 - 1];
    ZkTally tally[2];
    u32 group_start[EVM_N_GROUPS + 1];
    u32 pad1[8 - (EVM_N_GROUPS + 1)];
};
static_assert(sizeof(EvmDyn) <= 64 && sizeof(EvmResultBlock) == 128, "EvmResultBlock layout");
enum SessionKind { SESSION_SGA = 21, SESSION_ECC_ASSIGN = 20, SESSION_ECC = 19, SESSION_PIA = 18, SESSION_EXA = 17, SESSION_TXA = 16, SESSION_WITHDRAWAL = 15, SESSION_REKEY = 14, SESSION_PICOPY = 13, SESSION_PI = 12, SESSION_CPA = 11, SESSION_STATE = 1, SESSION_EVM = 2, SESSION_BYTECODE = 3, SESSION_EXP = 4, SESSION_COPY = 5, SESSION_SIGN = 6, SESSION_KECCAK = 7, SESSION_ASSIGN = 8, SESSION_ECDSA = 9, SESSION_BCA = 10 };

struct zk_session {
    SessionKind kind;
    int device = t_device;
    hipStream_t stream = t_stream;
    u64 n = 0;
    u64 eval_lo = 0, eval_hi = 0;
    bool eval_empty = false;
    std::vector<void*> owned;
    std::vector<int> owned_class;
    ZkTally* d_tally = nullptr;
    u32* d_status = nullptr;
    bool status_external = false;
    std::vector<hipEvent_t> ev;
    u32 launches = 0;
    u32 tally_pass = 0;
    ZkTally* tally_last = nullptr;
    StateArgs state;
    EvmArgs evm;
    BytecodeArgs bytecode;
    ExpArgs exp;
    CopyArgs copy;
    SignArgs sign;
    KeccakGenArgs keccak_gen;
    AssignArgs assign;
    EcdsaArgs ecdsa;
    BcaArgs bca;
    CpaArgs cpa;
    PiArgs pi;
    PiCopyArgs picopy;
    WithdrawalArgs withdrawal;
    TxAssignArgs txa;
    SigAssignArgs sga;
    ExaArgs exa;
    u64 exa_n_table = 0;
    EccPairArgs ecc;
    std::vector<u32> ecc_pair_off;
    PiaArgs pia;
    PiaSizes pia_sizes;
    KeccakGenArgs pia_kgen;
    u64 pia_host[4] = {0, 0, 0, 0};
    RekeyArgs rekey;
    RwkPlan rekey_plan_host;
    bool assign_from_rw = false;
    bool fused_order_ready = false;
    bool fused_verify = false;
    u32* rekey_status = nullptr;
    u64 cpa_n_table = 0, cpa_n_rw = 0;
    u32* d_hist = nullptr;
    u32* d_cursor = nullptr;
    u32* d_hist2 = nullptr;
    uint16_t* d_bin16 = nullptr;
    u32 evm_pass = 0;
    bool perm_ready = false;
    u32 evm_tally_idx = 0;
    bool perm_valid = false;
    int evm_ranges_known = 0;
    bool evm_warm_empty = false, evm_cold_empty = false;
    u32 evm_warm_lanes = 0;
    bool deferred_pending = false;
    u32* last_status = nullptr;
    u32* d_group_start = nullptr;
    u32* d_perm = nullptr;
    hipEvent_t ev_open0 = nullptr, ev_open1 = nullptr;
    bool side_stream = false;
    hipEvent_t ev_fork = nullptr, ev_join = nullptr;
    void* d_result = nullptr;
    void* h_result = nullptr;
    u32 publish_seq = 0;
    bool publish_enqueued = false;
    u32* h_result_dev = nullptr;
    u32 early_seq = 0;
    bool tail_pending = false;
    u32 tail_cold_grid = 0;
    u32* tail_status = nullptr;
    hipEvent_t tail_e1 = nullptr;
    bool stream_drained = false;
};

static const int MAX_EVENT_PAIRS = 256;

static int session_rebind_stream(zk_session* s, hipStream_t st) {
    HIP_TRY(hipSetDevice(s->device));
    if (!st) st = g_own_stream[s->device];
    if (st == s->stream) return 0;
    HIP_TRY(hipStreamSynchronize(s->stream));
    s->stream = st;
    return 0;
}

#define ZK_ARENA_CLASSES 48
struct DevArena {
    std::mutex m;
    std::vector<void*> free_[ZK_ARENA_CLASSES];
    std::vector<hipEvent_t> events;
    std::vector<void*> pinned;
    size_t cached_bytes = 0;
};
static DevArena g_arena[ZK_MAX_DEVICES];
static size_t arena_limit() {
    static const size_t lim = [] { const char* e = getenv("ZK_ARENA_MAX_BYTES"); return e ? (size_t)strtoull(e, nullptr, 10) : ((size_t)16 << 30); }();
    return lim;
}
static bool arena_off() {
    static const bool off = [] { const char* e = getenv("ZK_NO_ARENA"); return e && e[0] == '1'; }();
    return off;
}
static int arena_class(size_t bytes) {
    int c = 8;
    while (((size_t)1 << c) < bytes) c++;
    return c;
}
static int arena_take(int device, size_t bytes, void** p, int* cls) {
    const int c = arena_class(bytes ? bytes : 16);
    *cls = c;
    if (!arena_off() && c < ZK_ARENA_CLASSES) {
        DevArena& A = g_arena[device];
        std::lock_guard<std::mutex> lock(A.m);
        if (!A.free_[c].empty()) {
            *p = A.free_[c].back();
            A.free_[c].pop_back();
            A.cached_bytes -= (size_t)1 << c;
            return 0;
        }
    }
    HIP_TRY(hipMalloc(p, arena_off() ? (bytes ? bytes : 16) : ((size_t)1 << c)));
    return 0;
}
static void arena_give(int device, void* p, int cls) {
    if (!arena_off() && cls < ZK_ARENA_CLASSES) {
        DevArena& A = g_arena[device];
        std::lock_guard<std::mutex> lock(A.m);
        if (A.cached_bytes + ((size_t)1 << cls) <= arena_limit()) {
            A.free_[cls].push_back(p);
            A.cached_bytes += (size_t)1 << cls;
            return;
        }
    }
    (void)hipFree(p);
}
#define ZK_PINNED_BYTES 256
static bool evm_poll_enabled() {
    static const bool poll = [] { const char* e = getenv("ZK_POLL_RESULT"); return !(e && e[0] == '0'); }();
    return poll;
}
static bool evm_lazy_tail_enabled() {
    static const bool lazy = [] { const char* e = getenv("ZK_LAZY_TAIL"); return !(e && e[0] == '0'); }();
    return lazy && evm_poll_enabled();
}
static int arena_pinned(int device, void** p) {
    {
        DevArena& A = g_arena[device];
        std::lock_guard<std::mutex> lock(A.m);
        if (!A.pinned.empty()) {
            *p = A.pinned.back();
            A.pinned.pop_back();
            return 0;
        }
    }
    HIP_TRY(hipHostMalloc(p, ZK_PINNED_BYTES, hipHostMallocDefault));
    return 0;
}
static int arena_event(int device, hipEvent_t* e) {
    {
        DevArena& A = g_arena[device];
        std::lock_guard<std::mutex> lock(A.m);
        if (!A.events.empty()) {
            *e = A.events.back();
            A.events.pop_back();
            return 0;
        }
    }
    HIP_TRY(hipEventCreate(e));
    return 0;
}
static void arena_release_all() {
    for (int d = 0; d < ZK_MAX_DEVICES; d++) {
        DevArena& A = g_arena[d];
        std::lock_guard<std::mutex> lock(A.m);
        bool any = !A.events.empty() || !A.pinned.empty();
        for (int c = 0; c < ZK_ARENA_CLASSES; c++) any = any || !A.free_[c].empty();
        if (!any || hipSetDevice(d) != hipSuccess) continue;
        for (int c = 0; c < ZK_ARENA_CLASSES; c++) {
            for (void* p : A.free_[c]) (void)hipFree(p);
            A.free_[c].clear();
        }
        for (hipEvent_t e : A.events) (void)hipEventDestroy(e);
        A.events.clear();
        for (void* h : A.pinned) (void)hipHostFree(h);
        A.pinned.clear();
        A.cached_bytes = 0;
    }
}

static int dev_alloc(zk_session* s, void** p, size_t bytes) {
    int cls = 0;
    int rc = arena_take(s->device, bytes, p, &cls);
    if (rc) return rc;
    s->owned.push_back(*p);
    s->owned_class.push_back(cls);
    return 0;
}
static int stage(zk_session* s, const void* src, size_t bytes, bool device_ptrs, const void** out) {
    if (bytes == 0 || !src) {
        *out = g_zero_row[s->device];
        return 0;
    }
    if (device_ptrs) {
        *out = src;
        return 0;
    }
    void* d = nullptr;
    int rc = dev_alloc(s, &d, bytes);
    if (rc) return rc;
    HIP_TRY(hipMemcpyAsync(d, src, bytes, hipMemcpyHostToDevice, s->stream));
    *out = d;
    return 0;
}

static int d2h_now(hipStream_t st, void* dst, const void* src, size_t bytes) {
    HIP_TRY(hipMemcpyAsync(dst, src, bytes, hipMemcpyDeviceToHost, st));
    HIP_TRY(hipStreamSynchronize(st));
    return 0;
}
struct HostView { const void* dev; const void* host; size_t bytes; };
static thread_local HostView t_host_view[4];
static thread_local int t_n_host_view = 0;
static int fetch_small(hipStream_t st, void* dst, const void* src, size_t bytes) {
    for (int k = 0; k < t_n_host_view; k++)
        if (t_host_view[k].dev == src && t_host_view[k].bytes >= bytes) { memcpy(dst, t_host_view[k].host, bytes); return 0; }
    return d2h_now(st, dst, src, bytes);
}

template <u64 (*HASH)(const ZkTable&, u32)>
static int build_index(zk_session* s, ZkTable& t, bool mpt_fingerprints = false, const ZkRwMeta* unless_dense = nullptr) {
    u32 cap = 16;
    while (cap < 2 * t.n + 2) cap <<= 1;
    u32* slots = nullptr;
    int rc = dev_alloc(s, (void**)&slots, (size_t)cap * sizeof(u32));
    if (rc) return rc;
    t.mask = cap - 1;
    t.slots = slots;
    if (unless_dense) hipLaunchKernelGGL(slots_fill_unless_dense_kernel, dim3((cap + 255) / 256), dim3(256), 0, s->stream, slots, cap, unless_dense);
    else hipLaunchKernelGGL(slots_fill_kernel, dim3((cap + 255) / 256), dim3(256), 0, s->stream, slots, cap);
    if (t.n && mpt_fingerprints) hipLaunchKernelGGL(mpt_index_build_kernel, dim3((t.n + 255) / 256), dim3(256), 0, s->stream, t, slots);
    else if (t.n) hipLaunchKernelGGL(HIP_KERNEL_NAME(index_build_kernel<HASH>), dim3((t.n + 255) / 256), dim3(256), 0, s->stream, t, slots, unless_dense);
    HIP_TRY(hipGetLastError());
    return 0;
}

static int session_common_init(zk_session* s) {
    int rc = dev_alloc(s, (void**)&s->d_tally, 2 * sizeof(ZkTally));
    if (rc) return rc;
    hipLaunchKernelGGL(tally_reset_kernel, dim3(1), dim3(2), 0, s->stream, s->d_tally, (u32*)nullptr);
    s->tally_last = s->d_tally;
    rc = dev_alloc(s, (void**)&s->d_status, (size_t)s->n * sizeof(u32));
    if (rc) return rc;
    HIP_TRY(hipMemsetAsync(s->d_status, 0, (size_t)s->n * sizeof(u32), s->stream));
    return 0;
}

extern "C" int zk_close(zk_session* s) {
    if (!s) return 0;
    (void)hipSetDevice(s->device);
    if (!s->stream_drained) (void)hipStreamSynchronize(s->stream);
    for (size_t k = 0; k < s->owned.size(); k++) arena_give(s->device, s->owned[k], s->owned_class[k]);
    {
        DevArena& A = g_arena[s->device];
        std::lock_guard<std::mutex> lock(A.m);
        for (hipEvent_t e : s->ev) A.events.push_back(e);
        if (s->ev_open0) A.events.push_back(s->ev_open0);
        if (s->ev_open1) A.events.push_back(s->ev_open1);
        if (s->ev_fork) A.events.push_back(s->ev_fork);
        if (s->ev_join) A.events.push_back(s->ev_join);
        if (s->h_result) A.pinned.push_back(s->h_result);
    }
    delete s;
    return 0;
}

extern "C" int zk_state_open(const uint64_t* rows, const uint32_t* flags, uint64_t n, const uint64_t* mpt,
                             uint64_t n_mpt, uint32_t opts, zk_session** out) {
    ARG_TRY(t_device >= 0, "zk_state_open: call zk_init first");
    HIP_TRY(hipSetDevice(t_device));
    ARG_TRY(out && rows && n > 0 && n < (1ull << 32), "zk_state_open: bad arguments");
    ARG_TRY(n_mpt < (1ull << 31), "zk_state_open: MPT table too large");
    const bool dev = opts & ZK_OPT_DEVICE_PTRS;
    const bool compact = opts & ZK_OPT_STATE_COMPACT;
    zk_session* s = new zk_session();
    s->kind = SESSION_STATE;
    s->n = n;
    int rc = 0;
    const void* p = nullptr;
    if ((rc = stage(s, rows, (size_t)n * (compact ? 15 : ST_NCELLS) * 32, dev, &p))) goto fail;
    s->state.rows.cells = (const u64*)p;
    s->state.rows.skip = compact ? 42u : 0u;
    if ((rc = stage(s, flags, (size_t)n * 4, dev, &p))) goto fail;
    s->state.rows.flags = (const u32*)p;
    s->state.rows.n = n;
    s->state.eval_lo = 0;
    s->state.eval_hi = n;
    if ((rc = stage(s, mpt, (size_t)n_mpt * MPT_NCELLS * 32, dev, &p))) goto fail;
    s->state.mpt.cells = (const u64*)p;
    s->state.mpt.flags = nullptr;
    s->state.mpt.n = (u32)n_mpt;
    s->state.mpt.ncells = MPT_NCELLS;
    if ((rc = build_index<state_mpt_key_hash>(s, s->state.mpt, true))) goto fail;
    if ((rc = session_common_init(s))) goto fail;
    *out = s;
    return 0;
fail:
    zk_close(s);
    return rc;
}

static int table_stage(zk_session* s, ZkTable& t, const uint64_t* cells, const uint32_t* flags, uint64_t n,
                       u32 ncells, bool dev) {
    const void* p = nullptr;
    int rc;
    if ((rc = stage(s, cells, (size_t)n * ncells * 32, dev, &p))) return rc;
    t.cells = (const u64*)p;
    if ((rc = stage(s, flags, (size_t)n * 4, dev, &p))) return rc;
    t.flags = (n && flags) ? (const u32*)p : nullptr;
    t.n = (u32)n;
    t.ncells = ncells;
    return 0;
}

#ifndef ZK_HIST_BLOCK
#define ZK_HIST_BLOCK 1024
#endif
static int evm_build_perm(zk_session* s) {
    const u32 n = s->evm.n_pairs;
    u32* h_cur = (s->evm_pass & 1u) ? s->d_hist2 : s->d_hist;
    u32* h_next = (s->evm_pass & 1u) ? s->d_hist : s->d_hist2;
    s->evm_pass++;
    hipLaunchKernelGGL(evm_state_hist_kernel, dim3((n + ZK_HIST_BLOCK - 1) / ZK_HIST_BLOCK), dim3(ZK_HIST_BLOCK), 0, s->stream, s->evm.steps, n, h_cur, s->d_cursor, s->d_bin16, s->d_tally, s->evm.defer_count);
    hipLaunchKernelGGL(evm_state_scatter_kernel, dim3((n + 1023) / 1024), dim3(1024), 0, s->stream, s->d_bin16, n, h_cur, h_next, s->d_cursor,
                       s->d_group_start, s->d_perm);
    HIP_TRY(hipGetLastError());
    return 0;
}

static inline u32 index_cap(u64 n) {
    u32 cap = 16;
    while (cap < 2 * n + 2) cap <<= 1;
    return cap;
}

extern "C" int zk_evm_open(const zk_evm_tables* t, uint32_t opts, zk_session** out) {
    ARG_TRY(t_device >= 0, "zk_evm_open: call zk_init first");
    HIP_TRY(hipSetDevice(t_device));
    ARG_TRY(t && out && t->steps && t->n_steps >= 2 && t->n_steps < (1ull << 32), "zk_evm_open: bad arguments");
    ARG_TRY(t->n_rw < (1ull << 31) && t->n_bytecode < (1ull << 31) && t->n_tx < (1ull << 31) && t->n_block < (1ull << 31) &&
            t->n_copy < (1ull << 31) && t->n_keccak < (1ull << 31) && t->n_exp < (1ull << 31) && t->n_withdrawals < (1ull << 31) &&
            t->n_sig < (1ull << 31) && t->n_ecc < (1ull << 31),
            "zk_evm_open: table too large");
    ARG_TRY(t->aux_cells == 0 || (t->aux_cells >= 2 && t->aux_cells <= 64), "zk_evm_open: aux_cells must be 0 (= 2) or 2..64");
    const bool dev = opts & ZK_OPT_DEVICE_PTRS;
    const bool generic = opts & ZK_OPT_GENERIC_INDEX;
    zk_session* s = new zk_session();
    s->kind = SESSION_EVM;
    s->n = t->n_steps - 1;
    s->side_stream = (opts & ZK_OPT_SIDE_STREAM) != 0;
    int rc = 0;
    const void* p = nullptr;
    EvmArgs& E = s->evm;
    if ((rc = stage(s, t->steps, (size_t)t->n_steps * STEP_NCELLS * 32, dev, &p))) goto fail;
    E.steps = (const u64*)p;
    E.n_steps = t->n_steps;
    E.n_pairs = (u32)(t->n_steps - 1);
    if ((rc = table_stage(s, E.rw, t->rw, t->rw_flags, t->n_rw, RW_NCELLS, dev))) goto fail;
    if ((rc = table_stage(s, E.bytecode, t->bytecode, nullptr, t->n_bytecode, BYTECODE_NCELLS, dev))) goto fail;
    if ((rc = table_stage(s, E.tx, t->tx, t->tx_flags, t->n_tx, TX_NCELLS, dev))) goto fail;
    if ((rc = table_stage(s, E.block, t->block, t->block_flags, t->n_block, BLOCK_NCELLS, dev))) goto fail;
    if ((rc = table_stage(s, E.copy, t->copy, nullptr, t->n_copy, COPY_T_NCELLS, dev))) goto fail;
    if ((rc = table_stage(s, E.keccak, t->keccak, nullptr, t->n_keccak, KECCAK_NCELLS, dev))) goto fail;
    if ((rc = table_stage(s, E.exp, t->exp, nullptr, t->n_exp, EXP_T_NCELLS, dev))) goto fail;
    if ((rc = table_stage(s, E.sig, t->sig, nullptr, t->n_sig, SIG_T_NCELLS, dev))) goto fail;
    if ((rc = table_stage(s, E.ecc, t->ecc, nullptr, t->n_ecc, ECC_T_NCELLS, dev))) goto fail;
    if ((rc = table_stage(s, E.withdrawals, t->withdrawals, nullptr, t->n_withdrawals, 4, dev))) goto fail;
    E.withdrawals.slots = nullptr;
    E.withdrawals.mask = 0;
    E.aux = nullptr;
    E.aux_kind = nullptr;
    E.aux_cells = t->aux_cells ? t->aux_cells : 2u;
    if (t->aux && t->aux_kind) {
        if ((rc = stage(s, t->aux, (size_t)t->n_steps * E.aux_cells * 32, dev, &p))) goto fail;
        E.aux = (const u64*)p;
        if ((rc = stage(s, t->aux_kind, (size_t)t->n_steps * 4, dev, &p))) goto fail;
        E.aux_kind = (const u32*)p;
    }
    {
        ZkTable* const small[EVM_OPEN_TABLES] = {&E.tx, &E.block, &E.bytecode, &E.copy, &E.keccak, &E.exp, &E.sig, &E.ecc};
        const bool want_dir = !generic && t->n_bytecode != 0;
        size_t n_ff = 0;
        u32 caps[EVM_OPEN_TABLES];
        for (int k = 0; k < EVM_OPEN_TABLES; k++) { caps[k] = index_cap(small[k]->n); n_ff += caps[k]; }
        const u32 cap_rw = index_cap(E.rw.n), cap_big = want_dir ? index_cap(t->n_bytecode) : 0u;
        n_ff += (size_t)cap_rw + 2 * (size_t)cap_big + (want_dir ? DIRB_SMALL_SLOTS : 0u);
        u32* ff = nullptr;
        if ((rc = dev_alloc(s, (void**)&ff, n_ff * sizeof(u32)))) goto fail;
        u32* cur = ff;
        for (int k = 0; k < EVM_OPEN_TABLES; k++) { small[k]->slots = cur; small[k]->mask = caps[k] - 1; cur += caps[k]; }
        E.rw.slots = cur; E.rw.mask = cap_rw - 1; cur += cap_rw;
        u32* const dir_rep = cur; cur += cap_big;
        u32* const dir_first = cur; cur += cap_big;
        u32* const small_slots = cur;
        const size_t dyn_bytes = 256, hist_bytes = EVM_N_BINS * sizeof(u32), status_bytes = (((size_t)s->n * sizeof(u32)) + 15) & ~(size_t)15;
        const size_t zero_bytes = dyn_bytes + 2 * hist_bytes + status_bytes + 3 * (size_t)cap_big * 4;
        char* zero = nullptr;
        if ((rc = dev_alloc(s, (void**)&zero, zero_bytes))) goto fail;
        EvmResultBlock* const rb = (EvmResultBlock*)zero;
        EvmDyn* dyn = &rb->dyn;
        s->d_result = rb;
        if ((rc = arena_pinned(s->device, &s->h_result))) goto fail;
        {
            void* hd = nullptr;
            if (hipHostGetDevicePointer(&hd, s->h_result, 0) == hipSuccess) s->h_result_dev = (u32*)hd;
            (void)hipGetLastError();
        }
        static_assert(sizeof(EvmResultBlock) <= 256, "the result block outgrew its slot");
        static_assert((EVM_N_BINS * sizeof(u32)) % 16 == 0, "zero region pieces are 16-byte multiples");
        s->d_hist = (u32*)(zero + dyn_bytes);
        s->d_hist2 = (u32*)(zero + dyn_bytes + hist_bytes);
        s->d_status = (u32*)(zero + dyn_bytes + 2 * hist_bytes);
        u32* const dir_last = (u32*)(zero + dyn_bytes + 2 * hist_bytes + status_bytes);
        E.dyn = dyn;
        E.defer_count = &dyn->n_deferred;
        if ((rc = dev_alloc(s, (void**)&E.defer_list, (size_t)E.n_pairs * sizeof(u32)))) goto fail;
        s->d_tally = rb->tally;
        s->tally_last = s->d_tally;
        {
            const u64 n16 = n_ff / 4 + zero_bytes / 16;
            const u32 fill_grid = (u32)(n16 / 256 < 2048 ? (n16 + 255) / 256 : 2048);
            if (arena_event(s->device, &s->ev_open0) || arena_event(s->device, &s->ev_open1)) s->ev_open0 = s->ev_open1 = nullptr;
            hipExtLaunchKernelGGL(evm_open_fill_kernel, dim3(fill_grid ? fill_grid : 1u), dim3(256), 0, s->stream, s->ev_open0, nullptr, 0, (uint4*)ff,
                                  (u64)(n_ff / 4), (uint4*)zero, (u64)(zero_bytes / 16));
        }
        E.rw_dense = 0;
        E.rw_base = 0;
        E.rw_keys = nullptr;
        E.codes.n = 0;
        E.codes.mask = 0;
        E.codes.packed = nullptr;
        E.codes.entries = nullptr;
        E.codes.slots = nullptr;
        E.agg_max_txs = E.agg_total_txs = E.agg_invalid_txs = E.agg_bad_invalid_rows = E.agg_total_wds = E.agg_rw_dups = 0;
        EvmOpenTables o;
        memset(&o, 0, sizeof o);
        u32 blk = 0;
        for (int k = 0; k < EVM_OPEN_TABLES; k++) { o.t[k] = *small[k]; o.block_start[k] = blk; blk += (small[k]->n + 255u) / 256u; }
        o.block_start[EVM_OPEN_TABLES] = blk;
        blk += (u32)((t->n_withdrawals + 255) / 256);
        o.block_start[EVM_OPEN_TABLES + 1] = blk;
        o.wds = E.withdrawals.cells;
        o.n_wds = (u32)t->n_withdrawals;
        o.dyn = dyn;
        o.tally = s->d_tally;
        o.rw = E.rw;
        if (t->n_rw && !generic) {
            u64* d_keys = nullptr;
            if ((rc = dev_alloc(s, (void**)&d_keys, (size_t)t->n_rw * 32))) goto fail;
            E.rw_keys = d_keys;
            o.rw_keys = d_keys;
        }
        const u32 rw_row_blocks = o.rw_keys ? (u32)((t->n_rw + 63) / 64) : 0u;
        o.dir_block0 = blk;
        u32 dir_row_blocks = 0;
        if (want_dir) {
            DirBuild& d = o.dir;
            d.rows = E.bytecode.cells;
            d.n = (u32)t->n_bytecode;
            d.rep = dir_rep;
            d.first = dir_first;
            d.last = dir_last;
            d.runs = dir_last + cap_big;
            d.bad = dir_last + 2 * (size_t)cap_big;
            d.big_mask = cap_big - 1;
            d.small_slots = small_slots;
            d.dyn = dyn;
            if ((rc = dev_alloc(s, (void**)&d.packed, (size_t)d.n * sizeof(uint16_t)))) goto fail;
            if ((rc = dev_alloc(s, (void**)&d.entries, (size_t)DIRB_MAX_ENTRIES * sizeof(ZkCodeEntry)))) goto fail;
            if ((rc = dev_alloc(s, (void**)&d.list, (size_t)DIRB_MAX_ENTRIES * 4))) goto fail;
            dir_row_blocks = (d.n + 255u) / 256u;
            E.codes.entries = d.entries;
            E.codes.slots = d.small_slots;
            E.codes.packed = d.packed;
        }
        if ((rc = dev_alloc(s, (void**)&s->d_cursor, EVM_N_BINS * sizeof(u32)))) goto fail;
        if ((rc = dev_alloc(s, (void**)&s->d_bin16, (size_t)E.n_pairs * sizeof(uint16_t)))) goto fail;
        s->d_group_start = rb->group_start;
        if ((rc = dev_alloc(s, (void**)&s->d_perm, ((size_t)E.n_pairs + EVM_PERM_PAD + 2 * EVM_HOT_BLOCK) * sizeof(u32)))) goto fail;
        const bool sorted = !(opts & ZK_OPT_NO_STATE_SORT);
        o.hist_block0 = o.dir_block0 + dir_row_blocks;
        u32 hist_blocks = 0, scatter_blocks = 0;
        if (sorted) {
            o.sort.steps = E.steps; o.sort.n_pairs = E.n_pairs; o.sort.hist = s->d_hist; o.sort.hist_next = s->d_hist2;
            o.sort.taken = s->d_cursor; o.sort.bin16 = s->d_bin16; o.sort.group_start = s->d_group_start; o.sort.perm = s->d_perm;
            o.sort.tally = s->d_tally;
            o.sort.defer_count = E.defer_count;
            if ((opts & ZK_OPT_SINGLE_PASS) && s->h_result_dev && evm_lazy_tail_enabled() && !(opts & ZK_OPT_SIDE_STREAM)) {
                static std::atomic<u32> g_early_seq{0};
                u32 q = ++g_early_seq;
                if (!q) q = ++g_early_seq;
                __atomic_store_n(&((u32*)s->h_result)[EVM_EARLY_WORD + 2], 0u, __ATOMIC_RELEASE);
                s->early_seq = q;
                o.sort.early_host = s->h_result_dev;
                o.sort.early_seq = q;
            }
            hist_blocks = (E.n_pairs + 255u) / 256u;
            scatter_blocks = (E.n_pairs + EVM_OPEN_P2_BLOCK - 1u) / EVM_OPEN_P2_BLOCK;
            s->evm_pass = 1;
            s->perm_ready = true;
        }
        o.rw_block0 = o.hist_block0 + hist_blocks;
        o.rec_block0 = o.rw_block0 + rw_row_blocks;
        u32 rec_blocks = 0;
        E.step_recs = nullptr;
        if (!(opts & ZK_OPT_SINGLE_PASS)) {
            u32* recs = nullptr;
            if ((rc = dev_alloc(s, (void**)&recs, (size_t)t->n_steps * EVM_REC_WORDS * sizeof(u32)))) goto fail;
            o.steps = E.steps; o.n_steps = (u32)t->n_steps; o.step_recs = recs;
            E.step_recs = recs;
            rec_blocks = (u32)((t->n_steps + 63) / 64);
        }
        const u32 grid1 = o.rec_block0 + rec_blocks;
        {
            static const u32 spread = [] { const char* e = getenv("ZK_P1_LAT_SPREAD"); const int v = e ? atoi(e) : 2; return (u32)(v < 0 ? 0 : v); }();
            o.lat_period = (o.rw_block0 && spread) ? o.rec_block0 / (spread * o.rw_block0) : 0u;
        }
#ifdef ZK_DIAG_P1
        if (const char* e = getenv("ZK_DIAG_P1_SKIP")) o.diag_skip = (u32)atoi(e);
#endif
        {
            const u32 dir_blocks = want_dir ? DIRB_MAX_ENTRIES / EVM_OPEN_P2_BLOCK : 0u;
            const u32 rw_blocks = t->n_rw ? EVM_OPEN_RW_GENERIC_BLOCKS : 0u;
            bool phase2 = scatter_blocks + dir_blocks + rw_blocks != 0;
#ifdef ZK_DIAG_P1
            if (o.diag_skip) phase2 = false;
#endif
            hipExtLaunchKernelGGL(evm_open_phase1_kernel, dim3(grid1 ? grid1 : 1u), dim3(256), 0, s->stream, nullptr, phase2 ? nullptr : s->ev_open1, 0, o);
            if (phase2)
                hipExtLaunchKernelGGL(evm_open_phase2_kernel, dim3(scatter_blocks + dir_blocks + rw_blocks), dim3(EVM_OPEN_P2_BLOCK), 0, s->stream, nullptr,
                                      s->ev_open1, 0, o, scatter_blocks, dir_blocks, generic ? 1u : 0u);
        }
        if (hipGetLastError() != hipSuccess) { rc = -2; g_err = "zk_evm_open: a build kernel failed to launch"; goto fail; }
    }
    E.opts = (t->begin_with_first_step ? 1u : 0u) | (t->end_with_last_step ? 2u : 0u);
    E.prof = nullptr;
    if (getenv("ZK_EVM_PROF")) {
        if ((rc = dev_alloc(s, (void**)&E.prof, 1024 * 4 * 8 * sizeof(unsigned long long)))) goto fail;
        if (hipMemsetAsync(E.prof, 0, 1024 * 4 * 8 * sizeof(unsigned long long), s->stream) != hipSuccess) { rc = -2; goto fail; }
    }
    E.perm = (opts & ZK_OPT_NO_STATE_SORT) ? nullptr : s->d_perm;
    *out = s;
    return 0;
fail:
    zk_close(s);
    return rc;
}

static void session_timing(zk_session* s, double pass_ms, double* open_ms, double* span_ms);
static int evm_enqueue_tail(zk_session* s);
static bool evm_publish_enqueue(zk_session* s);
extern "C" int zk_evm_verify(const zk_evm_tables* t, uint32_t opts, uint32_t* status_out, zk_result* result) {
    ARG_TRY(result, "zk_evm_verify: result is null");
    zk_session* s = nullptr;
    const auto h0 = std::chrono::steady_clock::now();
    int rc = zk_evm_open(t, opts | ZK_OPT_SINGLE_PASS, &s);
    if (rc) return rc;
    const auto h1 = std::chrono::steady_clock::now();
    const bool dev = opts & ZK_OPT_DEVICE_PTRS;
    rc = zk_launch(s, (dev && status_out) ? status_out : nullptr);
    const auto h2 = std::chrono::steady_clock::now();
    if (!rc) rc = zk_collect(s, result);
    const auto h3 = std::chrono::steady_clock::now();
    if (!rc) {
        t_timing[1] = result->kernel_ms;
        session_timing(s, result->kernel_ms, &t_timing[0], &t_timing[2]);
        for (int k = 0; k < 3; k++) t_timing_sum[k] += t_timing[k];
        t_timing_count++;
    }
    if (!rc && status_out && !dev) rc = zk_read_status(s, status_out);
    zk_close(s);
    const auto h4 = std::chrono::steady_clock::now();
    t_host_phase[0] = std::chrono::duration<double, std::micro>(h1 - h0).count();
    t_host_phase[1] = std::chrono::duration<double, std::micro>(h2 - h1).count();
    t_host_phase[2] = std::chrono::duration<double, std::micro>(h3 - h2).count();
    t_host_phase[3] = std::chrono::duration<double, std::micro>(h4 - h3).count();
    return rc;
}

extern "C" int zk_evm_verify_batch(const zk_evm_tables* const* t, uint64_t n, uint32_t opts, zk_result* results) {
    ARG_TRY(t_device >= 0, "zk_evm_verify_batch: call zk_init first");
    ARG_TRY((t && results) || n == 0, "zk_evm_verify_batch: bad arguments");
    for (uint64_t i = 0; i < n; i++) ARG_TRY(t[i], "zk_evm_verify_batch: null witness");
    HIP_TRY(hipSetDevice(t_device));
    {
        std::lock_guard<std::mutex> lock(g_dev_mutex);
        for (int k = 0; k < 2; k++)
            if (!g_batch_stream[t_device][k]) HIP_TRY(hipStreamCreateWithFlags(&g_batch_stream[t_device][k], hipStreamNonBlocking));
    }
    const hipStream_t caller = t_stream;
    HIP_TRY(hipStreamSynchronize(caller));
    zk_session* pend[2] = {nullptr, nullptr};
    int rc = 0;
    for (uint64_t i = 0; i < n + 2 && !rc; i++) {
        const int slot = (int)(i & 1u);
        if (pend[slot]) {
            rc = zk_collect(pend[slot], &results[i - 2]);
            zk_close(pend[slot]);
            pend[slot] = nullptr;
        }
        if (!rc && i < n) {
            t_stream = g_batch_stream[t_device][slot];
            rc = zk_evm_open(t[i], opts | ZK_OPT_SINGLE_PASS, &pend[slot]);
            t_stream = caller;
            if (!rc) rc = zk_launch(pend[slot], nullptr);
        }
        zk_session* const o = pend[slot ^ 1];
        if (!rc && o && !o->publish_enqueued) {
            rc = evm_enqueue_tail(o);
            if (!rc) o->publish_enqueued = evm_publish_enqueue(o);
        }
    }
    for (int k = 0; k < 2; k++)
        if (pend[k]) zk_close(pend[k]);
    return rc;
}

extern "C" int zk_bytecode_open(const uint64_t* rows, uint64_t n, const uint64_t* keccak, uint64_t n_keccak,
                                const uint64_t* randomness, uint32_t opts, zk_session** out) {
    ARG_TRY(t_device >= 0, "zk_bytecode_open: call zk_init first");
    HIP_TRY(hipSetDevice(t_device));
    ARG_TRY(out && rows && randomness && n > 0 && n < (1ull << 32) && n_keccak < (1ull << 31), "zk_bytecode_open: bad arguments");
    const bool dev = opts & ZK_OPT_DEVICE_PTRS;
    zk_session* s = new zk_session();
    s->kind = SESSION_BYTECODE;
    s->n = n;
    int rc = 0;
    const void* p = nullptr;
    u64 rh[4];
    if ((rc = stage(s, rows, (size_t)n * BC_NCELLS * 32, dev, &p))) goto fail;
    s->bytecode.rows.cells = (const u64*)p;
    s->bytecode.rows.flags = nullptr;
    s->bytecode.rows.n = n;
    if ((rc = table_stage(s, s->bytecode.keccak, keccak, nullptr, n_keccak, KECCAK_NCELLS, dev))) goto fail;
    if ((rc = build_index<keccak_key_hash>(s, s->bytecode.keccak))) goto fail;
    if (dev) {
        if (fetch_small(s->stream, rh, randomness, 32)) { rc = -2; g_err = "randomness download failed"; goto fail; }
    } else {
        memcpy(rh, randomness, 32);
    }
    for (int k = 0; k < 4; k++) { s->bytecode.r.v[2 * k] = (u32)rh[k]; s->bytecode.r.v[2 * k + 1] = (u32)(rh[k] >> 32); }
    {
        u64* d_rm = nullptr;
        if ((rc = dev_alloc(s, (void**)&d_rm, 32))) goto fail;
        zk_launch_fr_to_mont(s->stream, s->bytecode.r, d_rm);
        s->bytecode.r_mont = d_rm;
    }
    if ((rc = session_common_init(s))) goto fail;
    *out = s;
    return 0;
fail:
    zk_close(s);
    return rc;
}

extern "C" int zk_exp_open(const uint64_t* rows, uint64_t n, uint32_t opts, zk_session** out) {
    ARG_TRY(t_device >= 0, "zk_exp_open: call zk_init first");
    HIP_TRY(hipSetDevice(t_device));
    ARG_TRY(out && rows && n > 0 && n < (1ull << 32), "zk_exp_open: bad arguments");
    const bool dev = opts & ZK_OPT_DEVICE_PTRS;
    zk_session* s = new zk_session();
    s->kind = SESSION_EXP;
    s->n = n;
    int rc = 0;
    const void* p = nullptr;
    if ((rc = stage(s, rows, (size_t)n * EX_NCELLS * 32, dev, &p))) goto fail;
    s->exp.rows.cells = (const u64*)p;
    s->exp.rows.flags = nullptr;
    s->exp.rows.n = n;
    if ((rc = session_common_init(s))) goto fail;
    *out = s;
    return 0;
fail:
    zk_close(s);
    return rc;
}

static int build_rw_meta(zk_session* s, const ZkTable& rw, const ZkRwMeta** out) {
    ZkRwMeta* d_meta = nullptr;
    int rc = dev_alloc(s, (void**)&d_meta, sizeof(ZkRwMeta));
    if (rc) return rc;
    static const ZkRwMeta init_dense = {1u, 0u, 0ull}, init_empty = {0u, 0u, 0ull};
    HIP_TRY(hipMemcpyAsync(d_meta, rw.n ? &init_dense : &init_empty, sizeof(ZkRwMeta), hipMemcpyHostToDevice, s->stream));
    if (rw.n) hipLaunchKernelGGL(rw_dense_check_kernel, dim3((rw.n + 255) / 256), dim3(256), 0, s->stream, rw, d_meta);
    *out = d_meta;
    return 0;
}

extern "C" int zk_copy_open(const zk_copy_tables* t, uint32_t opts, zk_session** out) {
    ARG_TRY(t_device >= 0, "zk_copy_open: call zk_init first");
    HIP_TRY(hipSetDevice(t_device));
    ARG_TRY(t && out && t->rows && t->randomness && t->n_rows > 0 && t->n_rows < (1ull << 32), "zk_copy_open: bad arguments");
    ARG_TRY(t->n_rw < (1ull << 31) && t->n_bytecode < (1ull << 31) && t->n_tx < (1ull << 31), "zk_copy_open: table too large");
    const bool dev = opts & ZK_OPT_DEVICE_PTRS;
    zk_session* s = new zk_session();
    s->kind = SESSION_COPY;
    s->n = t->n_rows;
    int rc = 0;
    const void* p = nullptr;
    u64 rh[4];
    if ((rc = stage(s, t->rows, (size_t)t->n_rows * CP_NCELLS * 32, dev, &p))) goto fail;
    s->copy.rows.cells = (const u64*)p;
    if ((rc = stage(s, t->row_flags, (size_t)t->n_rows * 4, dev, &p))) goto fail;
    s->copy.rows.flags = t->row_flags ? (const u32*)p : nullptr;
    s->copy.rows.n = t->n_rows;
    if ((rc = table_stage(s, s->copy.rw, t->rw, t->rw_flags, t->n_rw, RW_NCELLS, dev))) goto fail;
    if ((rc = table_stage(s, s->copy.bytecode, t->bytecode, nullptr, t->n_bytecode, BYTECODE_NCELLS, dev))) goto fail;
    if ((rc = table_stage(s, s->copy.tx, t->tx, t->tx_flags, t->n_tx, TX_NCELLS, dev))) goto fail;
    s->copy.rw_meta = nullptr;
    if (!(opts & ZK_OPT_GENERIC_INDEX) && (rc = build_rw_meta(s, s->copy.rw, &s->copy.rw_meta))) goto fail;
    if ((rc = build_index<rw_key_hash>(s, s->copy.rw, false, s->copy.rw_meta))) goto fail;
    if ((rc = build_index<bc_key_hash>(s, s->copy.bytecode))) goto fail;
    if ((rc = build_index<tx_key_hash>(s, s->copy.tx))) goto fail;
    if (dev) {
        if (fetch_small(s->stream, rh, t->randomness, 32)) { rc = -2; g_err = "randomness download failed"; goto fail; }
    } else {
        memcpy(rh, t->randomness, 32);
    }
    for (int k = 0; k < 4; k++) { s->copy.r.v[2 * k] = (u32)rh[k]; s->copy.r.v[2 * k + 1] = (u32)(rh[k] >> 32); }
    if ((rc = session_common_init(s))) goto fail;
    *out = s;
    return 0;
fail:
    zk_close(s);
    return rc;
}

static int one_shot(zk_session* s, bool dev, uint32_t* status_out, zk_result* result);
extern "C" int zk_sign_open(const zk_sign_units* t, uint32_t opts, zk_session** out) {
    ARG_TRY(t_device >= 0, "zk_sign_open: call zk_init first");
    HIP_TRY(hipSetDevice(t_device));
    ARG_TRY(t && out && t->bytes && t->cells && t->meta && t->randomness && t->n_units > 0 && t->n_units < (1ull << 32),
            "zk_sign_open: bad arguments");
    ARG_TRY(t->n_keccak < (1ull << 31) && t->n_tx_rows < (1ull << 32), "zk_sign_open: table too large");
    const bool dev = opts & ZK_OPT_DEVICE_PTRS;
    zk_session* s = new zk_session();
    s->kind = SESSION_SIGN;
    s->n = t->n_units;
    int rc = 0;
    const void* p = nullptr;
    u64 rh[4];
    if ((rc = stage(s, t->bytes, (size_t)t->n_units * SG_NBYTES_ROWS * 32, dev, &p))) goto fail;
    s->sign.bytes = (const uint8_t*)p;
    if ((rc = stage(s, t->cells, (size_t)t->n_units * SG_NCELLS * 32, dev, &p))) goto fail;
    s->sign.cells.cells = (const u64*)p;
    s->sign.cells.flags = nullptr;
    s->sign.cells.n = t->n_units;
    if ((rc = stage(s, t->meta, (size_t)t->n_units * 16, dev, &p))) goto fail;
    s->sign.meta = (const u32*)p;
    if ((rc = table_stage(s, s->sign.keccak, t->keccak, nullptr, t->n_keccak, KECCAK_NCELLS, dev))) goto fail;
    if ((rc = build_index<keccak_key_hash>(s, s->sign.keccak))) goto fail;
    if ((rc = table_stage(s, s->sign.tx_rows, t->tx_rows, t->tx_flags, t->n_tx_rows, TX_NCELLS, dev))) goto fail;
    s->sign.tx_rows.slots = nullptr;
    s->sign.tx_rows.mask = 0;
    s->sign.is_sig = t->is_sig ? 1u : 0u;
    if (dev) {
        if (fetch_small(s->stream, rh, t->randomness, 32)) { rc = -2; g_err = "randomness download failed"; goto fail; }
    } else {
        memcpy(rh, t->randomness, 32);
    }
    for (int k = 0; k < 4; k++) { s->sign.r.v[2 * k] = (u32)rh[k]; s->sign.r.v[2 * k + 1] = (u32)(rh[k] >> 32); }
    {
        u64* d_rpow = nullptr;
        if ((rc = dev_alloc(s, (void**)&d_rpow, 64 * 4 * sizeof(u64)))) goto fail;
        zk_launch_sign_rpow(s->stream, s->sign.r, d_rpow);
        s->sign.rpow = d_rpow;
    }
    if ((rc = session_common_init(s))) goto fail;
    *out = s;
    return 0;
fail:
    zk_close(s);
    return rc;
}
extern "C" int zk_sign_verify(const zk_sign_units* t, uint32_t opts, uint32_t* status_out, zk_result* result) {
    ARG_TRY(result, "zk_sign_verify: result is null");
    zk_session* s = nullptr;
    int rc = zk_sign_open(t, opts, &s);
    if (rc) return rc;
    return one_shot(s, opts & ZK_OPT_DEVICE_PTRS, status_out, result);
}

extern "C" int zk_keccak_open(const uint8_t* data, uint64_t n_bytes, const uint64_t* offsets, uint64_t n_msgs,
                              const uint64_t* randomness, uint32_t mode, uint64_t* rows_dev, uint32_t opts, zk_session** out) {
    ARG_TRY(t_device >= 0, "zk_keccak_open: call zk_init first");
    HIP_TRY(hipSetDevice(t_device));
    ARG_TRY(out && offsets && randomness && n_msgs > 0 && n_msgs < (1ull << 32) && (data || n_bytes == 0) && mode <= 1u,
            "zk_keccak_open: bad arguments");
    const bool dev = opts & ZK_OPT_DEVICE_PTRS;
    ARG_TRY(dev || !rows_dev, "zk_keccak_open: rows_dev needs ZK_OPT_DEVICE_PTRS");
    if (!dev) {
        for (u64 k = 0; k < n_msgs; k++) ARG_TRY(offsets[k] <= offsets[k + 1], "zk_keccak_open: offsets must be non-decreasing");
        ARG_TRY(offsets[n_msgs] <= n_bytes, "zk_keccak_open: offsets exceed the data buffer");
    }
    zk_session* s = new zk_session();
    s->kind = SESSION_KECCAK;
    s->n = n_msgs;
    int rc = 0;
    const void* p = nullptr;
    u64 rh[4];
    Fr r;
    if ((rc = stage(s, data, (size_t)n_bytes, dev, &p))) goto fail;
    s->keccak_gen.data = (const uint8_t*)p;
    if ((rc = stage(s, offsets, (size_t)(n_msgs + 1) * 8, dev, &p))) goto fail;
    s->keccak_gen.offsets = (const u64*)p;
    s->keccak_gen.n = n_msgs;
    s->keccak_gen.mode = mode;
    s->keccak_gen.long_list = nullptr;
    s->keccak_gen.long_count = nullptr;
    if (mode == KT_MODE_CIRCUIT && !getenv("ZK_KECCAK_NO_GROUPS")) {
        u32* d_list = nullptr;
        if ((rc = dev_alloc(s, (void**)&d_list, ((size_t)n_msgs + 1) * sizeof(u32)))) goto fail;
        s->keccak_gen.long_list = d_list + 1;
        s->keccak_gen.long_count = d_list;
    }
    if (dev) {
        if (fetch_small(s->stream, rh, randomness, 32)) { rc = -2; g_err = "randomness download failed"; goto fail; }
    } else {
        memcpy(rh, randomness, 32);
    }
    for (int k = 0; k < 4; k++) { r.v[2 * k] = (u32)rh[k]; r.v[2 * k + 1] = (u32)(rh[k] >> 32); }
    {
        u64* d_rpow = nullptr;
        if ((rc = dev_alloc(s, (void**)&d_rpow, KT_RPOW_ROWS * 4 * sizeof(u64)))) goto fail;
        zk_launch_keccak_rpow(s->stream, r, d_rpow);
        s->keccak_gen.rpow = d_rpow;
    }
    if (rows_dev) {
        s->keccak_gen.rows = rows_dev;
    } else {
        u64* d_rows = nullptr;
        if ((rc = dev_alloc(s, (void**)&d_rows, (size_t)n_msgs * KT_NCELLS * 32))) goto fail;
        s->keccak_gen.rows = d_rows;
    }
    if ((rc = session_common_init(s))) goto fail;
    *out = s;
    return 0;
fail:
    zk_close(s);
    return rc;
}
extern "C" int zk_keccak_read_rows(zk_session* s, uint64_t* rows_host) {
    ARG_TRY(s && rows_host && s->kind == SESSION_KECCAK, "zk_keccak_read_rows: bad arguments");
    HIP_TRY(hipMemcpyAsync(rows_host, s->keccak_gen.rows, (size_t)s->n * KT_NCELLS * 32, hipMemcpyDeviceToHost, s->stream));
    HIP_TRY(hipStreamSynchronize(s->stream));
    return 0;
}
extern "C" int zk_keccak_table(const uint8_t* data, uint64_t n_bytes, const uint64_t* offsets, uint64_t n_msgs,
                               const uint64_t* randomness, uint32_t mode, uint64_t* rows_out, uint32_t opts,
                               uint32_t* status_out, zk_result* result) {
    ARG_TRY(result && rows_out, "zk_keccak_table: null output");
    const bool dev = opts & ZK_OPT_DEVICE_PTRS;
    zk_session* s = nullptr;
    int rc = zk_keccak_open(data, n_bytes, offsets, n_msgs, randomness, mode, dev ? rows_out : nullptr, opts, &s);
    if (rc) return rc;
    rc = zk_launch(s, (dev && status_out) ? status_out : nullptr);
    if (!rc) rc = zk_collect(s, result);
    if (!rc && !dev) rc = zk_keccak_read_rows(s, rows_out);
    if (!rc && status_out && !dev) rc = zk_read_status(s, status_out);
    zk_close(s);
    return rc;
}

extern "C" int zk_state_assign_open(const uint64_t* ops, const uint32_t* op_flags, uint64_t n, uint64_t* rows_dev,
                                    uint32_t* row_flags_dev, uint64_t* mpt_dev, uint32_t opts, zk_session** out) {
    ARG_TRY(t_device >= 0, "zk_state_assign_open: call zk_init first");
    HIP_TRY(hipSetDevice(t_device));
    ARG_TRY(out && ops && op_flags && n > 0 && n < (1ull << 31), "zk_state_assign_open: bad arguments");
    const bool dev = opts & ZK_OPT_DEVICE_PTRS;
    ARG_TRY(dev || (!rows_dev && !row_flags_dev && !mpt_dev), "zk_state_assign_open: output buffers need ZK_OPT_DEVICE_PTRS");
    zk_session* s = new zk_session();
    s->kind = SESSION_ASSIGN;
    s->n = n;
    AssignArgs& a = s->assign;
    int rc = 0;
    const void* p = nullptr;
    u32 cap = 16;
    if ((rc = stage(s, ops, (size_t)n * ASG_NSLOTS * 32, dev, &p))) goto fail;
    a.ops = (const u64*)p;
    if ((rc = stage(s, op_flags, (size_t)n * 4, dev, &p))) goto fail;
    a.op_flags = (const u32*)p;
    a.n = n;
    a.nb = (u32)((n + ASG_BLOCK - 1) / ASG_BLOCK);
    a.rows = rows_dev;
    a.row_flags = row_flags_dev;
    a.mpt = mpt_dev;
    a.compact = (opts & ZK_OPT_STATE_COMPACT) ? 1u : 0u;
    if (!a.rows && (rc = dev_alloc(s, (void**)&a.rows, (size_t)n * (a.compact ? 15 : ASG_ROW_NCELLS) * 32))) goto fail;
    if (!a.row_flags && (rc = dev_alloc(s, (void**)&a.row_flags, (size_t)n * 4))) goto fail;
    if (!a.mpt && (rc = dev_alloc(s, (void**)&a.mpt, (size_t)n * ASG_MPT_NCELLS * 32))) goto fail;
    while (cap < 2 * n + 2) cap <<= 1;
// ... 766 lines not shown
    s->kind = SESSION_PIA;
    PiaSizes z;
    const int rc = pia_prepare(t, opts & ZK_OPT_DEVICE_PTRS, s, z);
    zk_close(s);
    if (rc) return rc;
    if (circuit_len) *circuit_len = z.n;
    if (n_gas) *n_gas = z.n_gas;
    if (n_constraints) *n_constraints = z.n_cc;
    return 0;
}
extern "C" int zk_pi_assign_open(const zk_pi_inputs* t, const zk_pi_wire* out_dev, uint32_t opts, zk_session** out) {
    ARG_TRY(t_device >= 0, "zk_pi_assign_open: call zk_init first");
    HIP_TRY(hipSetDevice(t_device));
    ARG_TRY(PIA_ARGS_OK(t) && out, "zk_pi_assign_open: bad arguments");
    const bool dev = opts & ZK_OPT_DEVICE_PTRS;
    ARG_TRY(dev || !out_dev, "zk_pi_assign_open: output buffers need ZK_OPT_DEVICE_PTRS");
    zk_session* s = new zk_session();
    s->kind = SESSION_PIA;
    PiaArgs& a = s->pia;
    PiaSizes& z = s->pia_sizes;
    int rc = pia_prepare(t, dev, s, z);
    if (rc) goto fail;
    if ((rc = pia_tables(s, z))) goto fail;
    s->n = z.n;
    if ((rc = dev_alloc(s, (void**)&a.gas_local, ((size_t)a.total_cd + 1) * 4))) goto fail;
    if ((rc = dev_alloc(s, (void**)&a.gas_tile, ((size_t)a.n_gas_tiles + 1) * 8))) goto fail;
    if ((rc = dev_alloc(s, (void**)&a.inv_txlo, ((size_t)PIA_TX_LEN * a.max_txs + 1) * 32))) goto fail;
    if ((rc = dev_alloc(s, (void**)&a.slice_acc, (size_t)a.n_tiles * 256 * 32))) goto fail;
    if ((rc = dev_alloc(s, (void**)&a.tile_acc, ((size_t)a.n_tiles + 1) * 32))) goto fail;
    if ((rc = dev_alloc(s, (void**)&a.carry, ((size_t)a.n_tiles + 1) * 32))) goto fail;
    if (out_dev) {
        a.rows = out_dev->rows; a.gas = out_dev->gas; a.keccak = out_dev->keccak; a.cc_cells = out_dev->cc_cells; a.cc_bytes = out_dev->cc_bytes;
        a.cc_lens = out_dev->cc_lens; a.block_table = out_dev->block_table; a.block_flags = out_dev->block_flags; a.tx_table = out_dev->tx_table;
        a.tx_flags = out_dev->tx_flags; a.wd_table = out_dev->wd_table; a.public_inputs = out_dev->public_inputs; a.raw_bytes = out_dev->raw_bytes;
        a.raw_lens = out_dev->raw_lens;
    } else {
        a.rows = a.gas = a.keccak = a.cc_cells = a.block_table = a.tx_table = a.wd_table = a.public_inputs = nullptr;
        a.cc_bytes = a.raw_bytes = nullptr;
        a.cc_lens = a.block_flags = a.tx_flags = a.raw_lens = nullptr;
    }
    if (!a.rows && (rc = dev_alloc(s, (void**)&a.rows, (size_t)z.n * PI_NCELLS * 32))) goto fail;
    if (!a.gas && (rc = dev_alloc(s, (void**)&a.gas, (size_t)z.n_gas * PI_GAS_NCELLS * 32))) goto fail;
    if (!a.keccak && (rc = dev_alloc(s, (void**)&a.keccak, 2 * 5 * 32))) goto fail;
    if (!a.cc_cells && (rc = dev_alloc(s, (void**)&a.cc_cells, (size_t)z.n_cc * 32))) goto fail;
    if (!a.cc_bytes && (rc = dev_alloc(s, (void**)&a.cc_bytes, (size_t)z.n_cc * 32))) goto fail;
    if (!a.cc_lens && (rc = dev_alloc(s, (void**)&a.cc_lens, (size_t)z.n_cc * 4))) goto fail;
    if (!a.block_table && (rc = dev_alloc(s, (void**)&a.block_table, (size_t)PIA_BLOCK_ENTRIES * 2 * 32))) goto fail;
    if (!a.block_flags && (rc = dev_alloc(s, (void**)&a.block_flags, (size_t)PIA_BLOCK_ENTRIES * 4))) goto fail;
    if (!a.tx_table && (rc = dev_alloc(s, (void**)&a.tx_table, (size_t)z.tx_table_rows * 5 * 32))) goto fail;
    if (!a.tx_flags && (rc = dev_alloc(s, (void**)&a.tx_flags, (size_t)z.tx_table_rows * 4))) goto fail;
    if (!a.wd_table && (rc = dev_alloc(s, (void**)&a.wd_table, (size_t)a.max_wd * 5 * 32))) goto fail;
    if (!a.public_inputs && (rc = dev_alloc(s, (void**)&a.public_inputs, 4 * 2 * 32))) goto fail;
    if (!a.raw_bytes && (rc = dev_alloc(s, (void**)&a.raw_bytes, (size_t)z.n))) goto fail;
    if (!a.raw_lens && (rc = dev_alloc(s, (void**)&a.raw_lens, (size_t)z.n_values * 4))) goto fail;
    if ((rc = session_common_init(s))) goto fail;
    *out = s;
    return 0;
fail:
    zk_close(s);
    return rc;
}
#define PIA_D2H(dst, src, bytes) do { if (dst) HIP_TRY(hipMemcpyAsync(dst, src, bytes, hipMemcpyDeviceToHost, s->stream)); } while (0)
extern "C" int zk_pi_assign_read(zk_session* s, const zk_pi_wire* h) {
    ARG_TRY(s && h && s->kind == SESSION_PIA, "zk_pi_assign_read: bad arguments");
    HIP_TRY(hipSetDevice(s->device));
    const PiaArgs& a = s->pia;
    const PiaSizes& z = s->pia_sizes;
    PIA_D2H(h->rows, a.rows, (size_t)z.n * PI_NCELLS * 32);
    PIA_D2H(h->gas, a.gas, (size_t)z.n_gas * PI_GAS_NCELLS * 32);
    PIA_D2H(h->keccak, a.keccak, 2 * 5 * 32);
    PIA_D2H(h->cc_cells, a.cc_cells, (size_t)z.n_cc * 32);
    PIA_D2H(h->cc_bytes, a.cc_bytes, (size_t)z.n_cc * 32);
    PIA_D2H(h->cc_lens, a.cc_lens, (size_t)z.n_cc * 4);
    PIA_D2H(h->block_table, a.block_table, (size_t)PIA_BLOCK_ENTRIES * 2 * 32);
    PIA_D2H(h->block_flags, a.block_flags, (size_t)PIA_BLOCK_ENTRIES * 4);
    PIA_D2H(h->tx_table, a.tx_table, (size_t)z.tx_table_rows * 5 * 32);
    PIA_D2H(h->tx_flags, a.tx_flags, (size_t)z.tx_table_rows * 4);
    PIA_D2H(h->wd_table, a.wd_table, (size_t)a.max_wd * 5 * 32);
    PIA_D2H(h->public_inputs, a.public_inputs, 4 * 2 * 32);
    PIA_D2H(h->raw_bytes, a.raw_bytes, (size_t)z.n);
    PIA_D2H(h->raw_lens, a.raw_lens, (size_t)z.n_values * 4);
    HIP_TRY(hipStreamSynchronize(s->stream));
    return 0;
}
extern "C" int zk_pi_assign(const zk_pi_inputs* t, const zk_pi_wire* out_wire, uint32_t opts, zk_result* result) {
    ARG_TRY(result && out_wire && out_wire->rows, "zk_pi_assign: null output");
    const bool dev = opts & ZK_OPT_DEVICE_PTRS;
    zk_session* s = nullptr;
    int rc = zk_pi_assign_open(t, dev ? out_wire : nullptr, opts, &s);
    if (rc) return rc;
    rc = zk_launch(s, nullptr);
    if (!rc) rc = zk_collect(s, result);
    if (!rc && !dev) rc = zk_pi_assign_read(s, out_wire);
    zk_close(s);
    return rc;
}

extern "C" int zk_pi_open(const uint64_t* rows, uint64_t n, const uint64_t* keccak, uint64_t n_keccak, const uint64_t* gas, uint64_t n_gas,
                          uint64_t circuit_len, const uint64_t* keccak_rand, const uint64_t* byte_pow_base, uint32_t opts, zk_session** out) {
    ARG_TRY(t_device >= 0, "zk_pi_open: call zk_init first");
    HIP_TRY(hipSetDevice(t_device));
    ARG_TRY(out && rows && keccak_rand && byte_pow_base && n > 0 && n < (1ull << 32) && n_keccak < (1ull << 31) && n_gas < (1ull << 31), "zk_pi_open: bad arguments");
    const bool dev = opts & ZK_OPT_DEVICE_PTRS;
    zk_session* s = new zk_session();
    s->kind = SESSION_PI;
    s->n = n;
    int rc = 0;
    const void* p = nullptr;
    u64 rh[8];
    if ((rc = stage(s, rows, (size_t)n * PI_NCELLS * 32, dev, &p))) goto fail;
    s->pi.rows.cells = (const u64*)p;
    s->pi.rows.flags = nullptr;
    s->pi.rows.n = n;
    if ((rc = table_stage(s, s->pi.keccak, keccak, nullptr, n_keccak, KECCAK_NCELLS, dev))) goto fail;
    if ((rc = build_index<keccak_key_hash>(s, s->pi.keccak))) goto fail;
    if ((rc = table_stage(s, s->pi.gas, gas, nullptr, n_gas, PI_GAS_NCELLS, dev))) goto fail;
    if ((rc = build_index<pi_gas_key_hash>(s, s->pi.gas))) goto fail;
    if (dev) {
        if (d2h_now(s->stream, rh, keccak_rand, 32) || d2h_now(s->stream, rh + 4, byte_pow_base, 32)) {
            rc = -2; g_err = "randomness download failed"; goto fail;
        }
    } else {
        memcpy(rh, keccak_rand, 32);
        memcpy(rh + 4, byte_pow_base, 32);
    }
    {
        Fr kr, bp;
        for (int k = 0; k < 4; k++) {
            kr.v[2 * k] = (u32)rh[k]; kr.v[2 * k + 1] = (u32)(rh[k] >> 32);
            bp.v[2 * k] = (u32)rh[4 + k]; bp.v[2 * k + 1] = (u32)(rh[4 + k] >> 32);
        }
        u64* d_m = nullptr;
        u64 hm[8];
        if ((rc = dev_alloc(s, (void**)&d_m, 64))) goto fail;
        zk_launch_fr_to_mont(s->stream, kr, d_m);
        zk_launch_fr_to_mont(s->stream, bp, d_m + 4);
        if (hipMemcpyAsync(hm, d_m, 64, hipMemcpyDeviceToHost, s->stream) != hipSuccess || hipStreamSynchronize(s->stream) != hipSuccess) {
            rc = -2; g_err = "constant download failed"; goto fail;
        }
        for (int k = 0; k < 4; k++) {
            s->pi.keccak_rand_m.v[2 * k] = (u32)hm[k]; s->pi.keccak_rand_m.v[2 * k + 1] = (u32)(hm[k] >> 32);
            s->pi.byte_pow_base_m.v[2 * k] = (u32)hm[4 + k]; s->pi.byte_pow_base_m.v[2 * k + 1] = (u32)(hm[4 + k] >> 32);
        }
    }
    s->pi.circuit_len = Fr{{(u32)circuit_len, (u32)(circuit_len >> 32), 0, 0, 0, 0, 0, 0}};
    if ((rc = session_common_init(s))) goto fail;
    *out = s;
    return 0;
fail:
    zk_close(s);
    return rc;
}
extern "C" int zk_pi_copy_open(const uint64_t* cells, const uint8_t* bytes, const uint32_t* lens, uint64_t n, uint32_t opts, zk_session** out) {
    ARG_TRY(t_device >= 0, "zk_pi_copy_open: call zk_init first");
    HIP_TRY(hipSetDevice(t_device));
    ARG_TRY(out && cells && bytes && lens && n > 0 && n < (1ull << 32), "zk_pi_copy_open: bad arguments");
    const bool dev = opts & ZK_OPT_DEVICE_PTRS;
    zk_session* s = new zk_session();
    s->kind = SESSION_PICOPY;
    s->n = n;
    int rc = 0;
    const void* p = nullptr;
    if ((rc = stage(s, cells, (size_t)n * 32, dev, &p))) goto fail;
    s->picopy.cells = (const u64*)p;
    if ((rc = stage(s, bytes, (size_t)n * 32, dev, &p))) goto fail;
    s->picopy.bytes = (const uint8_t*)p;
    if ((rc = stage(s, lens, (size_t)n * 4, dev, &p))) goto fail;
    s->picopy.lens = (const u32*)p;
    s->picopy.n = n;
    if ((rc = session_common_init(s))) goto fail;
    *out = s;
    return 0;
fail:
    zk_close(s);
    return rc;
}
extern "C" int zk_pi_copy_verify(const uint64_t* cells, const uint8_t* bytes, const uint32_t* lens, uint64_t n, uint32_t opts, uint32_t* status_out,
                                 zk_result* result) {
    ARG_TRY(result, "zk_pi_copy_verify: result is null");
    zk_session* s = nullptr;
    int rc = zk_pi_copy_open(cells, bytes, lens, n, opts, &s);
    if (rc) return rc;
    const bool dev = opts & ZK_OPT_DEVICE_PTRS;
    rc = zk_launch(s, (dev && status_out) ? status_out : nullptr);
    if (!rc) rc = zk_collect(s, result);
    if (!rc && status_out && !dev) rc = zk_read_status(s, status_out);
    zk_close(s);
    return rc;
}
extern "C" int zk_pi_verify(const uint64_t* rows, uint64_t n, const uint64_t* keccak, uint64_t n_keccak, const uint64_t* gas, uint64_t n_gas,
                            uint64_t circuit_len, const uint64_t* keccak_rand, const uint64_t* byte_pow_base, uint32_t opts,
                            uint32_t* status_out, zk_result* result) {
    ARG_TRY(result, "zk_pi_verify: result is null");
    zk_session* s = nullptr;
    int rc = zk_pi_open(rows, n, keccak, n_keccak, gas, n_gas, circuit_len, keccak_rand, byte_pow_base, opts, &s);
    if (rc) return rc;
    return one_shot(s, opts & ZK_OPT_DEVICE_PTRS, status_out, result);
}

extern "C" int zk_copy_verify(const zk_copy_tables* t, uint32_t opts, uint32_t* status_out, zk_result* result) {
    ARG_TRY(result, "zk_copy_verify: result is null");
    zk_session* s = nullptr;
    int rc = zk_copy_open(t, opts, &s);
    if (rc) return rc;
    return one_shot(s, opts & ZK_OPT_DEVICE_PTRS, status_out, result);
}

static int one_shot(zk_session* s, bool dev, uint32_t* status_out, zk_result* result) {
    int rc = zk_launch(s, (dev && status_out) ? status_out : nullptr);
    if (!rc) rc = zk_collect(s, result);
    if (!rc && status_out && !dev) rc = zk_read_status(s, status_out);
    zk_close(s);
    return rc;
}
extern "C" int zk_bytecode_verify(const uint64_t* rows, uint64_t n, const uint64_t* keccak, uint64_t n_keccak,
                                  const uint64_t* randomness, uint32_t opts, uint32_t* status_out, zk_result* result) {
    ARG_TRY(result, "zk_bytecode_verify: result is null");
    zk_session* s = nullptr;
    int rc = zk_bytecode_open(rows, n, keccak, n_keccak, randomness, opts, &s);
    if (rc) return rc;
    return one_shot(s, opts & ZK_OPT_DEVICE_PTRS, status_out, result);
}
extern "C" int zk_exp_verify(const uint64_t* rows, uint64_t n, uint32_t opts, uint32_t* status_out, zk_result* result) {
    ARG_TRY(result, "zk_exp_verify: result is null");
    zk_session* s = nullptr;
    int rc = zk_exp_open(rows, n, opts, &s);
    if (rc) return rc;
    return one_shot(s, opts & ZK_OPT_DEVICE_PTRS, status_out, result);
}

static inline u64 range_lo(const zk_session* s) { return (s->eval_hi || s->eval_empty) ? s->eval_lo : 0; }
static inline u64 range_hi(const zk_session* s) { return s->eval_empty ? s->eval_lo : s->eval_hi ? s->eval_hi : s->n; }
extern "C" int zk_set_range(zk_session* s, uint64_t row_lo, uint64_t row_hi) {
    ARG_TRY(s && (s->kind == SESSION_STATE || s->kind == SESSION_BYTECODE || s->kind == SESSION_COPY || s->kind == SESSION_EXP ||
                  s->kind == SESSION_SIGN || s->kind == SESSION_PI || s->kind == SESSION_WITHDRAWAL || s->kind == SESSION_ECC),
            "zk_set_range: not a row-circuit session (EVM sessions shard by the steps they are opened over)");
    ARG_TRY((row_lo < row_hi || (s->kind == SESSION_ECC && row_lo == row_hi)) && row_hi <= s->n, "zk_set_range: bad range");
    HIP_TRY(hipSetDevice(s->device));
    s->eval_lo = row_lo;
    s->eval_hi = row_hi;
    s->eval_empty = row_lo == row_hi;
    if (s->kind == SESSION_STATE) {
        s->state.eval_lo = row_lo;
        s->state.eval_hi = row_hi;
    }
    HIP_TRY(hipMemsetAsync(s->d_status, 0, (size_t)s->n * sizeof(u32), s->stream));
    return 0;
}
extern "C" int zk_state_set_range(zk_session* s, uint64_t row_lo, uint64_t row_hi) {
    ARG_TRY(s && s->kind == SESSION_STATE, "zk_state_set_range: not a State session");
    return zk_set_range(s, row_lo, row_hi);
}

extern "C" int zk_debug_read_deferred(zk_session* s, uint32_t* count, uint32_t* list, uint32_t max) {
    if (!s || s->kind != SESSION_EVM || !s->evm.defer_count) return -1;
    HIP_TRY(hipStreamSynchronize(s->stream));
    HIP_TRY(hipMemcpy(count, s->evm.defer_count, 4, hipMemcpyDeviceToHost));
    const uint32_t n = *count < max ? *count : max;
    if (n && list) HIP_TRY(hipMemcpy(list, s->evm.defer_list, (size_t)n * 4, hipMemcpyDeviceToHost));
    return 0;
}
extern "C" int zk_debug_read_prof(zk_session* s, unsigned long long* out) {
    if (!s || !s->evm.prof) return -1;
    HIP_TRY(hipStreamSynchronize(s->stream));
    HIP_TRY(hipMemcpy(out, s->evm.prof, 1024 * 4 * 8 * sizeof(unsigned long long), hipMemcpyDeviceToHost));
    return 0;
}

__global__ void __launch_bounds__(256) calib_gather_kernel(const uint4* __restrict__ buf, u64 n_rec, u32 vec_per_rec,
                                                           u32* __restrict__ sink) {
    const u64 i = (u64)blockIdx.x * blockDim.x + threadIdx.x;
    if (i >= n_rec) return;
    const uint4* p = buf + i * vec_per_rec;
    u32 acc = 0;
    for (u32 k = 0; k < vec_per_rec; ++k) {
        const uint4 v = p[k];
        acc ^= v.x ^ v.y ^ v.z ^ v.w;
    }
    if (acc == 0x9e3779b9u) sink[0] = acc;
}
extern "C" int zk_debug_calib_gather(uint64_t nbytes, uint32_t lane_bytes, float* ms_out) {
    ARG_TRY(lane_bytes && lane_bytes % 16 == 0 && nbytes >= lane_bytes, "zk_debug_calib_gather: bad sizes");
    const u64 n_rec = nbytes / lane_bytes;
    uint4* buf = nullptr;
    u32* sink = nullptr;
    HIP_TRY(hipMalloc(&buf, n_rec * lane_bytes));
    HIP_TRY(hipMalloc(&sink, 64));
    HIP_TRY(hipMemsetAsync(buf, 0x5a, n_rec * lane_bytes, t_stream));
    hipEvent_t e0, e1;
    HIP_TRY(hipEventCreate(&e0));
    HIP_TRY(hipEventCreate(&e1));
    HIP_TRY(hipEventRecord(e0, t_stream));
    calib_gather_kernel<<<dim3((unsigned)((n_rec + 255) / 256)), dim3(256), 0, t_stream>>>(buf, n_rec, lane_bytes / 16, sink);
    HIP_TRY(hipEventRecord(e1, t_stream));
    HIP_TRY(hipStreamSynchronize(t_stream));
    if (ms_out) HIP_TRY(hipEventElapsedTime(ms_out, e0, e1));
    hipEventDestroy(e0);
    hipEventDestroy(e1);
    hipFree(buf);
    hipFree(sink);
    return 0;
}

static int evm_enqueue_tail(zk_session* s) {
    if (s->kind != SESSION_EVM || !s->tail_pending) return 0;
    s->tail_pending = false;
    s->stream_drained = false;
    const u32* hw = (const u32*)s->h_result;
    const auto t0 = std::chrono::steady_clock::now();
    u64 spins = 0;
    bool seen = true;
    while (__atomic_load_n(&hw[EVM_EARLY_WORD + 2], __ATOMIC_ACQUIRE) != s->early_seq) {
        __builtin_ia32_pause();
        if ((++spins & 0xfffu) == 0 && std::chrono::steady_clock::now() - t0 > std::chrono::seconds(5)) { seen = false; break; }
    }
    u32 warm_lanes = 0;
    bool run_warm = true, run_cold = true;
    if (seen) {
        warm_lanes = hw[EVM_EARLY_WORD];
        const u32 cold_lanes = hw[EVM_EARLY_WORD + 1];
        run_warm = warm_lanes != 0;
        run_cold = cold_lanes != 0;
        s->evm_ranges_known = 1;
        s->evm_warm_empty = !run_warm;
        s->evm_warm_lanes = warm_lanes;
        s->evm_cold_empty = !run_cold;
    }
    s->early_seq = 0;
    if (run_warm) zk_launch_evm_warm(s->stream, s->tail_cold_grid, warm_lanes, s->evm, s->d_group_start, s->tail_status, s->tally_last, run_cold ? nullptr : s->tail_e1);
    if (run_cold) zk_launch_evm_cold(s->stream, s->tail_cold_grid, s->evm, s->d_group_start, s->tail_status, s->tally_last, s->tail_e1);
    HIP_TRY(hipGetLastError());
    return 0;
}

extern "C" int zk_launch(zk_session* s, uint32_t* status_dev) {
    ARG_TRY(s, "zk_launch: null session");
    s->stream_drained = false;
    HIP_TRY(hipSetDevice(s->device));
    { int trc = evm_enqueue_tail(s); if (trc) return trc; }
    s->publish_enqueued = false;
    s->status_external = status_dev != nullptr;
    hipEvent_t e0 = nullptr, e1 = nullptr;
    const bool timed = s->launches < (u32)MAX_EVENT_PAIRS;
    if (timed) {
        if (s->ev.size() < 2 * (size_t)(s->launches + 1)) {
            int erc = arena_event(s->device, &e0);
            if (erc) return erc;
            s->ev.push_back(e0);
            if ((erc = arena_event(s->device, &e1))) return erc;
            s->ev.push_back(e1);
        }
        e0 = s->ev[2 * s->launches];
        e1 = s->ev[2 * s->launches + 1];
    }
    const bool twin_tally = s->kind == SESSION_STATE || s->kind == SESSION_BYTECODE || s->kind == SESSION_COPY ||
                            s->kind == SESSION_SIGN || s->kind == SESSION_EXP || s->kind == SESSION_PI || s->kind == SESSION_PICOPY ||
                            s->kind == SESSION_WITHDRAWAL || s->kind == SESSION_ECC;
    ZkTally* const tally = twin_tally ? s->d_tally + (s->tally_pass++ & 1u) : s->d_tally;
    s->tally_last = tally;
    if (!twin_tally && !(s->kind == SESSION_EVM && s->evm.perm))
        hipLaunchKernelGGL(tally_reset_kernel, dim3(1), dim3((s->fused_verify && !s->fused_order_ready) ? 2 : 1), 0, s->stream, s->d_tally,
                           s->kind == SESSION_EVM ? s->evm.defer_count : (u32*)nullptr);
    u32* status = status_dev ? status_dev : s->d_status;
    bool evm_ext_events = timed && s->kind == SESSION_EVM && s->evm.perm;
    hipStream_t side = nullptr;
    if (s->kind == SESSION_EVM && s->evm.perm && s->side_stream &&
        !(s->evm_ranges_known && s->evm_warm_empty && s->evm_cold_empty)) {
        {
            std::lock_guard<std::mutex> lock(g_dev_mutex);
            if (!g_side_stream[s->device]) HIP_TRY(hipStreamCreateWithFlags(&g_side_stream[s->device], hipStreamNonBlocking));
        }
        if (!s->ev_fork) {
            int erc = arena_event(s->device, &s->ev_fork);
            if (!erc) erc = arena_event(s->device, &s->ev_join);
            if (erc) return erc;
        }
        side = g_side_stream[s->device];
        if (side == s->stream) side = nullptr;
    }
    if (side) evm_ext_events = false;
    const bool state_ext_events = timed && s->kind == SESSION_STATE && zk_state_rows_events_ride(s->state);
    if (state_ext_events) evm_ext_events = true;
    if (timed && !evm_ext_events && !side) HIP_TRY(hipEventRecord(e0, s->stream));
    switch (s->kind) {
    case SESSION_STATE: zk_launch_state_rows(s->stream, s->state, status, tally, state_ext_events ? e0 : nullptr, state_ext_events ? e1 : nullptr); break;
    case SESSION_BYTECODE: zk_launch_bytecode_rows(s->stream, s->bytecode, range_lo(s), range_hi(s), status, tally); break;
    case SESSION_COPY: zk_launch_copy_rows(s->stream, s->copy, range_lo(s), range_hi(s), status, tally); break;
    case SESSION_SIGN: zk_launch_sign_units(s->stream, s->sign, range_lo(s), range_hi(s), status, tally); break;
    case SESSION_EXP: zk_launch_exp_rows(s->stream, s->exp, range_lo(s), range_hi(s), status, tally); break;
    case SESSION_KECCAK: zk_launch_keccak_table(s->stream, s->keccak_gen, status, s->d_tally); break;
    case SESSION_ASSIGN:
        if (s->fused_verify) {
            if (!s->fused_order_ready) {
                zk_launch_state_rekey(s->stream, s->rekey, s->rekey_status, s->d_tally + 1);
                zk_launch_state_assign(s->stream, s->assign, nullptr, nullptr);
            }
            zk_launch_state_rows_fused(s->stream, s->state, s->assign, status, s->d_tally, s->d_tally + 1);
            break;
        }
        if (s->assign_from_rw) zk_launch_state_rekey(s->stream, s->rekey, s->rekey_status, s->d_tally);
        zk_launch_state_assign(s->stream, s->assign, status, s->d_tally);
        break;
    case SESSION_ECDSA: zk_launch_ecdsa(s->stream, s->ecdsa, status, s->d_tally); break;
    case SESSION_BCA: zk_launch_bytecode_assign(s->stream, s->bca, status, s->d_tally); break;
    case SESSION_PI: zk_launch_pi_rows(s->stream, s->pi, range_lo(s), range_hi(s), status, tally); break;
    case SESSION_WITHDRAWAL: zk_launch_withdrawal_rows(s->stream, s->withdrawal, range_lo(s), range_hi(s), status, tally); break;
    case SESSION_ECC: {
        const u64 np = s->ecc.a.n_add + s->ecc.a.n_mul, lo = range_lo(s), hi = range_hi(s);
        const u64 k_lo = lo > np ? lo - np : 0, k_hi = hi > np ? hi - np : 0;
        const bool pairs = k_hi > k_lo;
        zk_launch_ecc_range(s->stream, s->ecc, lo, hi, pairs ? s->ecc_pair_off[k_lo] : 0u, pairs ? s->ecc_pair_off[k_hi] : 0u, status, tally);
        break;
    }
    case SESSION_ECC_ASSIGN: zk_launch_ecc(s->stream, s->ecc.a, true, nullptr, s->d_tally); break;
    case SESSION_TXA: zk_launch_tx_assign(s->stream, s->txa, status, s->d_tally); break;
    case SESSION_SGA: zk_launch_sig_assign(s->stream, s->sga, status, s->d_tally); break;
    case SESSION_PICOPY: zk_launch_pi_copy(s->stream, s->picopy, status, tally); break;
    case SESSION_CPA: zk_launch_copy_assign(s->stream, s->cpa, status, s->d_tally); break;
    case SESSION_EXA: zk_launch_exp_assign(s->stream, s->exa, status, s->d_tally); break;
    case SESSION_PIA: {
        {
            std::lock_guard<std::mutex> lock(g_dev_mutex);
            if (!g_side_stream[s->device]) HIP_TRY(hipStreamCreateWithFlags(&g_side_stream[s->device], hipStreamNonBlocking));
        }
        if (!s->ev_fork) {
            int erc = arena_event(s->device, &s->ev_fork);
            if (!erc) erc = arena_event(s->device, &s->ev_join);
            if (erc) return erc;
        }
        hipStream_t pside = g_side_stream[s->device];
        if (pside == s->stream) pside = nullptr;
        zk_launch_pi_assign(s->stream, pside, s->ev_fork, s->ev_join, s->pia, s->pia_kgen, status, s->d_tally);
        break;
    }
    case SESSION_REKEY: zk_launch_state_rekey(s->stream, s->rekey, status, s->d_tally); break;
    case SESSION_EVM: {
        if (s->evm.perm) {
            static const bool resort = [] { const char* e = getenv("ZK_EVM_RESORT"); return e && e[0] == '1'; }();
            if (s->perm_ready) { s->perm_ready = false; s->perm_valid = true; s->evm_tally_idx = 0; }
            else if (s->perm_valid && !resort) s->evm_tally_idx ^= 1u;
            else { int prc = evm_build_perm(s); if (prc) return prc; s->perm_valid = true; s->evm_tally_idx = 0; }
            {
                EvmResultBlock* const rb = (EvmResultBlock*)s->d_result;
                u32* const dc[2] = {&rb->dyn.n_deferred, &rb->n_deferred_twin};
                s->evm.defer_count = dc[s->evm_tally_idx];
                s->evm.defer_count_twin = resort ? nullptr : dc[s->evm_tally_idx ^ 1u];
                s->tally_last = s->d_tally + s->evm_tally_idx;
            }
        }
        const u32 grid = (u32)((s->n + (s->evm.perm ? EVM_PERM_PAD : 0) + EVM_HOT_BLOCK - 1) / EVM_HOT_BLOCK);
        const u32 all_grid = (u32)((s->n + 255) / 256);
        const u32 cold_grid = s->evm.perm ? (all_grid < 256u ? all_grid : 256u) : all_grid;
        s->deferred_pending = true;
        s->last_status = status;
        const bool sorted = s->evm.perm != nullptr;
        const bool run_warm = !(sorted && s->evm_ranges_known && s->evm_warm_empty);
        const bool run_cold = !(sorted && s->evm_ranges_known && s->evm_cold_empty);
        if (side) {
            hipEvent_t fork = timed ? e0 : s->ev_fork;
            HIP_TRY(hipEventRecord(fork, s->stream));
            HIP_TRY(hipStreamWaitEvent(side, fork, 0));
            if (run_warm)
                zk_launch_evm_warm(side, cold_grid, s->evm_ranges_known ? s->evm_warm_lanes : 0u, s->evm, s->d_group_start, status, s->tally_last, nullptr);
            if (run_cold) zk_launch_evm_cold(side, cold_grid, s->evm, s->d_group_start, status, s->tally_last, nullptr);
            HIP_TRY(hipEventRecord(s->ev_join, side));
            zk_launch_evm_hot(s->stream, grid, s->evm, s->d_group_start, status, s->tally_last, nullptr, nullptr);
            HIP_TRY(hipStreamWaitEvent(s->stream, s->ev_join, 0));
            if (status_dev && s->evm.defer_count) {
                zk_launch_evm_deferred(s->stream, s->evm, status, s->tally_last);
                s->deferred_pending = false;
            }
            break;
        }
        if (sorted && !s->evm_ranges_known && s->early_seq && !status_dev && evm_ext_events) {
            zk_launch_evm_hot(s->stream, grid, s->evm, s->d_group_start, status, s->tally_last, e0, e1);
            s->tail_pending = true;
            s->tail_cold_grid = cold_grid;
            s->tail_status = status;
            s->tail_e1 = e1;
            break;
        }
        hipEvent_t e_hot1 = (evm_ext_events && !run_warm && !run_cold) ? e1 : nullptr;
        zk_launch_evm_hot(s->stream, grid, s->evm, s->d_group_start, status, s->tally_last, evm_ext_events ? e0 : nullptr, e_hot1);
        if (run_warm)
            zk_launch_evm_warm(s->stream, cold_grid, (sorted && s->evm_ranges_known) ? s->evm_warm_lanes : 0u, s->evm, s->d_group_start, status, s->tally_last,
                               (evm_ext_events && !run_cold) ? e1 : nullptr);
        if (run_cold) zk_launch_evm_cold(s->stream, cold_grid, s->evm, s->d_group_start, status, s->tally_last, evm_ext_events ? e1 : nullptr);
        if (status_dev && s->evm.defer_count) {
            zk_launch_evm_deferred(s->stream, s->evm, status, s->tally_last);
            s->deferred_pending = false;
        }
        break;
    }
    }
    if (timed && !evm_ext_events) HIP_TRY(hipEventRecord(e1, s->stream));
    HIP_TRY(hipGetLastError());
    s->launches++;
    return 0;
}

static int evm_finish_deferred(zk_session* s) {
    { int trc = evm_enqueue_tail(s); if (trc) return trc; }
    if (s->kind != SESSION_EVM || !s->deferred_pending || !s->evm.defer_count) return 0;
    u32 n_def = 0;
    HIP_TRY(hipMemcpyAsync(&n_def, s->evm.defer_count, 4, hipMemcpyDeviceToHost, s->stream));
    HIP_TRY(hipStreamSynchronize(s->stream));
    s->deferred_pending = false;
    if (n_def) {
        s->stream_drained = false;
        zk_launch_evm_deferred(s->stream, s->evm, s->last_status, s->tally_last);
        HIP_TRY(hipGetLastError());
    }
    return 0;
}

static bool evm_publish_enqueue(zk_session* s) {
    if (s->kind != SESSION_EVM || !s->d_result || !s->h_result || !s->h_result_dev || !evm_poll_enabled()) return false;
    u32* hw = (u32*)s->h_result;
    const u32 seq = ++s->publish_seq ? s->publish_seq : ++s->publish_seq;
    __atomic_store_n(&hw[32], 0u, __ATOMIC_RELEASE);
    hipLaunchKernelGGL(evm_publish_kernel, dim3(1), dim3(64), 0, s->stream, (const u32*)s->d_result, s->h_result_dev, seq);
    return hipGetLastError() == hipSuccess;
}

extern "C" int zk_collect(zk_session* s, zk_result* r) {
    ARG_TRY(s && r, "zk_collect: bad arguments");
    HIP_TRY(hipSetDevice(s->device));
    { int trc = evm_enqueue_tail(s); if (trc) return trc; }
    ZkTally t;
    u32 n_def = 0;
    const bool check_deferred = s->kind == SESSION_EVM && s->deferred_pending && s->evm.defer_count;
    u32 gs[EVM_N_GROUPS + 1] = {0};
    const bool read_ranges = s->kind == SESSION_EVM && s->evm.perm && !s->evm_ranges_known && s->launches > 0;
    if (s->kind == SESSION_EVM && s->d_result && s->h_result) {
        const bool poll = evm_poll_enabled();
        bool polled = false;
        if (poll) {
            static_assert(sizeof(EvmResultBlock) == 128 && ZK_PINNED_BYTES >= 4 * (EVM_EARLY_WORD + 3), "flag word behind the result block, early words behind that");
            u32* hw = (u32*)s->h_result;
            void* const hd = s->h_result_dev;
            if (hd) {
                const bool launched = s->publish_enqueued || evm_publish_enqueue(s);
                s->publish_enqueued = false;
                const u32 seq = s->publish_seq;
                if (launched) {
                    const auto t0 = std::chrono::steady_clock::now();
                    u64 spins = 0;
                    while (__atomic_load_n(&hw[32], __ATOMIC_ACQUIRE) != seq) {
                        __builtin_ia32_pause();
                        if ((++spins & 0xfffu) == 0 && std::chrono::steady_clock::now() - t0 > std::chrono::seconds(5)) break;
                    }
                    polled = __atomic_load_n(&hw[32], __ATOMIC_ACQUIRE) == seq;
                }
            }
            (void)hipGetLastError();
        }
        if (polled) {
            s->stream_drained = true;
        } else {
            HIP_TRY(hipMemcpyAsync(s->h_result, s->d_result, sizeof(EvmResultBlock), hipMemcpyDeviceToHost, s->stream));
            HIP_TRY(hipStreamSynchronize(s->stream));
        }
        const EvmResultBlock* h = (const EvmResultBlock*)s->h_result;
        n_def = s->evm_tally_idx ? h->n_deferred_twin : h->dyn.n_deferred;
        for (int k = 0; k <= EVM_N_GROUPS; k++) gs[k] = h->group_start[k];
        t = h->tally[s->tally_last - s->d_tally];
    } else {
        if (check_deferred) HIP_TRY(hipMemcpyAsync(&n_def, s->evm.defer_count, 4, hipMemcpyDeviceToHost, s->stream));
        if (read_ranges) HIP_TRY(hipMemcpyAsync(gs, s->d_group_start, sizeof gs, hipMemcpyDeviceToHost, s->stream));
        ZkTally t_asg = {0ull, ~0ull};
        if (s->fused_verify) HIP_TRY(hipMemcpyAsync(&t_asg, s->d_tally + 1, sizeof t_asg, hipMemcpyDeviceToHost, s->stream));
        HIP_TRY(hipMemcpyAsync(&t, s->tally_last, sizeof t, hipMemcpyDeviceToHost, s->stream));
        HIP_TRY(hipStreamSynchronize(s->stream));
        if (t_asg.fail_count) {
            char msg[240];
            snprintf(msg, sizeof msg, "zk_state_verify_from_rw: the State witness assignment failed for %llu RW rows / ops (first: %llu, code 0x%08x; "
                     "zk_state_assign_from_rw reports each)", (unsigned long long)t_asg.fail_count, (unsigned long long)(t_asg.first_fail >> 32),
                     (unsigned)(t_asg.first_fail & 0xffffffffull));
            g_err = msg;
            s->launches = 0;
            return -1;
        }
        if (s->fused_verify && s->launches > 0) s->fused_order_ready = true;
    }
    if (read_ranges) {
        s->evm_ranges_known = 1;
        s->evm_warm_empty = gs[EVM_GROUP_WARM] == gs[EVM_GROUP_WARM + 1];
        s->evm_warm_lanes = gs[EVM_GROUP_WARM + 1] - gs[EVM_GROUP_WARM];
        s->evm_cold_empty = gs[EVM_GROUP_COLD] == gs[EVM_GROUP_COLD + 1];
    }
    if (check_deferred) {
        s->deferred_pending = false;
        if (n_def) {
            s->stream_drained = false;
        zk_launch_evm_deferred(s->stream, s->evm, s->last_status, s->tally_last);
            HIP_TRY(hipGetLastError());
            HIP_TRY(hipMemcpyAsync(&t, s->tally_last, sizeof t, hipMemcpyDeviceToHost, s->stream));
            HIP_TRY(hipStreamSynchronize(s->stream));
        }
    }
    double ms = 0;
    u32 timed = s->launches < (u32)MAX_EVENT_PAIRS ? s->launches : (u32)MAX_EVENT_PAIRS;
    for (u32 k = 0; k < timed; k++) {
        float f = 0;
        hipError_t ee = hipEventElapsedTime(&f, s->ev[2 * k], s->ev[2 * k + 1]);
        if (ee == hipErrorNotReady) {
            (void)hipGetLastError();
            (void)hipEventSynchronize(s->ev[2 * k + 1]);
            ee = hipEventElapsedTime(&f, s->ev[2 * k], s->ev[2 * k + 1]);
        }
        HIP_TRY(ee);
        ms += f;
    }
    r->fail_count = t.fail_count;
    r->first_fail_row = t.first_fail == ~0ull ? UINT64_MAX : (t.first_fail >> 32);
    r->first_fail_code = t.first_fail == ~0ull ? 0u : (u32)(t.first_fail & 0xffffffffull);
    r->launches = s->launches;
    r->rows_evaluated = range_hi(s) - range_lo(s);
    r->kernel_ms = timed ? ms / timed : 0.0;
    s->launches = 0;
    return 0;
}

extern "C" int zk_read_status(zk_session* s, uint32_t* status_host) {
    ARG_TRY(s && status_host, "zk_read_status: bad arguments");
    ARG_TRY(!s->status_external, "zk_read_status: the last pass wrote its statuses to the caller's status_dev buffer, not the session's");
    HIP_TRY(hipSetDevice(s->device));
    { int drc = evm_finish_deferred(s); if (drc) return drc; }
    HIP_TRY(hipMemcpyAsync(status_host, s->d_status, (size_t)s->n * 4, hipMemcpyDeviceToHost, s->stream));
    HIP_TRY(hipStreamSynchronize(s->stream));
    return 0;
}

static void session_timing(zk_session* s, double pass_ms, double* open_ms, double* span_ms) {
    *open_ms = *span_ms = -1.0;
    if (s->kind != SESSION_EVM || !s->ev_open0 || !s->ev_open1) return;
    float f = 0;
    if (hipEventElapsedTime(&f, s->ev_open0, s->ev_open1) == hipSuccess) *open_ms = f;
    if (pass_ms > 0 && s->ev.size() >= 2 && hipEventElapsedTime(&f, s->ev_open0, s->ev[1]) == hipSuccess) *span_ms = f;
    (void)hipGetLastError();
}
extern "C" int zk_session_timing(zk_session* s, double* open_ms, double* span_ms) {
    ARG_TRY(s && open_ms && span_ms, "zk_session_timing: bad arguments");
    HIP_TRY(hipSetDevice(s->device));
    session_timing(s, 1.0, open_ms, span_ms);
    return 0;
}
extern "C" int zk_last_host_phases(double* us4) {
    if (us4) for (int k = 0; k < 4; k++) us4[k] = t_host_phase[k];
    return 0;
}
extern "C" int zk_timing_sums(double* sums_ms, uint64_t* count, int reset) {
    if (sums_ms) for (int k = 0; k < 3; k++) sums_ms[k] = t_timing_sum[k];
    if (count) *count = t_timing_count;
    if (reset) { t_timing_sum[0] = t_timing_sum[1] = t_timing_sum[2] = 0; t_timing_count = 0; }
    return 0;
}
extern "C" int zk_last_timing(double* open_ms, double* pass_ms, double* span_ms) {
    if (open_ms) *open_ms = t_timing[0];
    if (pass_ms) *pass_ms = t_timing[1];
    if (span_ms) *span_ms = t_timing[2];
    return 0;
}

extern "C" int zk_state_verify(const uint64_t* rows, const uint32_t* flags, uint64_t n, const uint64_t* mpt,
                               uint64_t n_mpt, uint32_t opts, uint32_t* status_out, zk_result* result) {
    ARG_TRY(result, "zk_state_verify: result is null");
    zk_session* s = nullptr;
    int rc = zk_state_open(rows, flags, n, mpt, n_mpt, opts, &s);
    if (rc) return rc;
    const bool dev = opts & ZK_OPT_DEVICE_PTRS;
    rc = zk_launch(s, (dev && status_out) ? status_out : nullptr);
    if (!rc) rc = zk_collect(s, result);
    if (!rc && status_out && !dev) rc = zk_read_status(s, status_out);
    zk_close(s);
    return rc;
}

extern "C" int zk_fr_op(int op, const uint64_t* a, const uint64_t* b, uint64_t* out, uint64_t n, uint32_t opts) {
    ARG_TRY(t_device >= 0, "zk_fr_op: call zk_init first");
    HIP_TRY(hipSetDevice(t_device));
    ARG_TRY(a && b && out, "zk_fr_op: null pointer");
    if (n == 0) return 0;
    const bool dev = opts & ZK_OPT_DEVICE_PTRS;
    const u64 *da = a, *db = b;
    u64* dout = out;
    void *ta = nullptr, *tb = nullptr, *to = nullptr;
    if (!dev) {
        HIP_TRY(hipMalloc(&ta, n * 32));
        HIP_TRY(hipMalloc(&tb, n * 32));
        HIP_TRY(hipMalloc(&to, n * 32));
        HIP_TRY(hipMemcpyAsync(ta, a, n * 32, hipMemcpyHostToDevice, t_stream));
        HIP_TRY(hipMemcpyAsync(tb, b, n * 32, hipMemcpyHostToDevice, t_stream));
        da = (const u64*)ta;
        db = (const u64*)tb;
        dout = (u64*)to;
    }
    if (op >= 19 && op <= 25) {
        ARG_TRY(n % 12 == 0, "zk_fr_op 19..25: n must be a multiple of 12");
        zk_launch_fq12_op(t_stream, op, da, db, dout, n / 12);
    } else {
        hipLaunchKernelGGL(fr_op_kernel, dim3((u32)((n + 255) / 256)), dim3(256), 0, t_stream, op, da, db, dout, n);
    }
    HIP_TRY(hipGetLastError());
    if (!dev) {
        HIP_TRY(hipMemcpyAsync(out, to, n * 32, hipMemcpyDeviceToHost, t_stream));
        HIP_TRY(hipStreamSynchronize(t_stream));
        (void)hipFree(ta);
        (void)hipFree(tb);
        (void)hipFree(to);
    }
    return 0;
}

using zkdist::rccl;
using zkdist::RcclId;
static const int RCCL_UINT64 = zkdist::RCCL_UINT64;
#define RCCL_TRY(expr, what)                                                                                        \
    do {                                                                                                            \
        const int r_ = (expr);                                                                                      \
        if (r_ != 0) {                                                                                              \
            char buf_[256];                                                                                         \
            snprintf(buf_, sizeof buf_, "%s: RCCL error %d (%s)", what, r_, rccl().GetErrorString ? rccl().GetErrorString(r_) : "?"); \
            g_err = buf_;                                                                                           \
            return -3;                                                                                              \
        }                                                                                                           \
    } while (0)

struct zk_comm {
    void* nccl = nullptr;
    int rank = 0, world = 1, device = 0;
    hipStream_t stream = nullptr;
    u64* d_buf = nullptr;
    u64* h_buf = nullptr;
};
#define ZK_TALLY_WORDS zkdist::TALLY_WORDS

extern "C" int zk_dist_unique_id(uint8_t* id) {
    ARG_TRY(id, "zk_dist_unique_id: id is null");
    ARG_TRY(rccl().ok, "zk_dist_unique_id: librccl.so.1 could not be loaded");
    RcclId u;
    RCCL_TRY(rccl().GetUniqueId(&u), "ncclGetUniqueId");
    memcpy(id, u.internal, ZK_DIST_ID_BYTES);
    return 0;
}
extern "C" int zk_dist_close(zk_comm* c) {
    if (!c) return 0;
    (void)hipSetDevice(c->device);
    if (c->stream) (void)hipStreamSynchronize(c->stream);
    if (c->nccl && rccl().ok) (void)rccl().CommDestroy(c->nccl);
    if (c->d_buf) (void)hipFree(c->d_buf);
    if (c->h_buf) (void)hipHostFree(c->h_buf);
    if (c->stream) (void)hipStreamDestroy(c->stream);
    delete c;
    return 0;
}
extern "C" int zk_dist_init(const uint8_t* id, int rank, int world, zk_comm** out) {
    ARG_TRY(t_device >= 0, "zk_dist_init: call zk_init first");
    ARG_TRY(id && out && world >= 1 && rank >= 0 && rank < world, "zk_dist_init: bad arguments");
    ARG_TRY(rccl().ok, "zk_dist_init: librccl.so.1 could not be loaded");
    ARG_TRY(rccl().buffers == 1, "zk_dist_init: ZK_RCCL_LIB names a collective library that takes HOST buffers (zk_collective_buffers() == 0): the "
                                 "HIP library hands it device memory");
    HIP_TRY(hipSetDevice(t_device));
    zk_comm* c = new zk_comm();
    c->rank = rank; c->world = world; c->device = t_device;
    RcclId u;
    memcpy(u.internal, id, ZK_DIST_ID_BYTES);
    int rc = 0;
    if (hipStreamCreateWithFlags(&c->stream, hipStreamNonBlocking) != hipSuccess ||
        hipMalloc((void**)&c->d_buf, (size_t)(world + 1) * ZK_TALLY_WORDS * sizeof(u64)) != hipSuccess ||
        hipHostMalloc((void**)&c->h_buf, (size_t)(world + 1) * ZK_TALLY_WORDS * sizeof(u64), hipHostMallocDefault) != hipSuccess) {
        g_err = "zk_dist_init: buffer allocation failed";
        rc = -2;
    } else if (int r = rccl().CommInitRank(&c->nccl, world, u, rank)) {
        char buf[256];
        snprintf(buf, sizeof buf, "ncclCommInitRank: RCCL error %d (%s)", r, rccl().GetErrorString ? rccl().GetErrorString(r) : "?");
        g_err = buf;
        c->nccl = nullptr;
        rc = -3;
    }
    if (rc) { zk_dist_close(c); return rc; }
    *out = c;
    return 0;
}
extern "C" int zk_dist_tally(zk_comm* c, const zk_result* local, uint64_t row_offset, zk_result* global) {
    ARG_TRY(c && local && global, "zk_dist_tally: bad arguments");
    HIP_TRY(hipSetDevice(c->device));
    u64* mine = c->h_buf + (size_t)c->world * ZK_TALLY_WORDS;
    zkdist::tally_pack(mine, local, row_offset);
    HIP_TRY(hipMemcpyAsync(c->d_buf, mine, ZK_TALLY_WORDS * sizeof(u64), hipMemcpyHostToDevice, c->stream));
    RCCL_TRY(rccl().AllGather(c->d_buf, c->d_buf + ZK_TALLY_WORDS, ZK_TALLY_WORDS, RCCL_UINT64, c->nccl, c->stream), "ncclAllGather");
    HIP_TRY(hipMemcpyAsync(c->h_buf, c->d_buf + ZK_TALLY_WORDS, (size_t)c->world * ZK_TALLY_WORDS * sizeof(u64), hipMemcpyDeviceToHost, c->stream));
    HIP_TRY(hipStreamSynchronize(c->stream));
    zkdist::tally_reduce(c->h_buf, c->world, local, global);
    return 0;
}

#include <condition_variable>
#include <functional>
#include <thread>
struct BlockWorkers {
    std::mutex call;
    std::mutex m;
    std::condition_variable cv_job, cv_done;
    std::function<void()> job[4];
    bool has_job[4] = {false, false, false, false};
    int pending = 0;
    bool started = false;
    void run(int c) {
        for (;;) {
            std::function<void()> f;
            {
                std::unique_lock<std::mutex> lock(m);
                cv_job.wait(lock, [&] { return has_job[c]; });
                f = std::move(job[c]);
                has_job[c] = false;
            }
            f();
            {
                std::lock_guard<std::mutex> lock(m);
                pending--;
            }
            cv_done.notify_all();
        }
    }
};
static BlockWorkers* g_block_workers[ZK_MAX_DEVICES] = {nullptr};
struct BlockShared {
    std::mutex m;
    std::condition_variable cv;
    bool keccak_enqueued = false, keccak_failed = false;
    zk_session* keep = nullptr;
    zk_session* keep_cpa = nullptr;
    bool cpa_enqueued = false, cpa_failed = false;
    hipEvent_t ev_cpa = nullptr;
    zk_session* keep_exa = nullptr;
    hipEvent_t ev_exa = nullptr;
    hipEvent_t ev_keccak = nullptr;
    int rc[4] = {0, 0, 0, 0};
    std::string err[4];
    double end_ms[4] = {0, 0, 0, 0}, start_ms[4] = {0, 0, 0, 0};
    std::chrono::steady_clock::time_point t0;
};
#define BLK_TRY(expr) do { if ((rc = (expr))) goto done; } while (0)
static int block_run_pass(zk_session* s, zk_result* r) {
    int rc = zk_launch(s, nullptr);
    if (!rc) rc = zk_collect(s, r);
    return rc;
}
extern "C" int zk_block_verify(const zk_block* b, uint32_t opts, zk_result* results, double* chain_ms) {
    ARG_TRY(t_device >= 0, "zk_block_verify: call zk_init first");
    ARG_TRY(b && results && (opts & ZK_OPT_DEVICE_PTRS), "zk_block_verify: needs a block, a result array and ZK_OPT_DEVICE_PTRS");
    ARG_TRY(b->evm.steps && b->evm.n_steps >= 2 && b->evm.rw && b->evm.n_rw && b->randomness && b->hashed_offsets && b->n_hashed >= b->n_codes &&
            b->code_offsets && b->code_lengths && b->n_bytecodes, "zk_block_verify: bad arguments");
    ARG_TRY(!b->exp_events.n_events || (b->exp_events.events && !b->n_exp_rows && !b->evm.n_exp),
            "zk_block_verify: exp_events given together with exp_rows / evm.exp (hand over one of the two forms)");
    HIP_TRY(hipSetDevice(t_device));
    const int device = t_device;
    const uint32_t dev_opts = ZK_OPT_DEVICE_PTRS, st_opts = ZK_OPT_DEVICE_PTRS | (opts & ZK_OPT_STATE_COMPACT);
    BlockShared sh;
    sh.t0 = std::chrono::steady_clock::now();
    BlockWorkers* W = nullptr;
    {
        std::lock_guard<std::mutex> lock(g_dev_mutex);
        { int brc = block_streams_ensure(device); if (brc) return brc; }
        if (!g_block_workers[device]) g_block_workers[device] = new BlockWorkers();
        W = g_block_workers[device];
    }
    std::lock_guard<std::mutex> one_block(W->call);
    if (!W->started) {
        for (int c = 0; c < 4; c++) std::thread([W, c] { W->run(c); }).detach();
        W->started = true;
    }
    for (int c = 0; c < ZK_BLOCK_NCIRCUITS; c++) { memset(&results[c], 0, sizeof(zk_result)); results[c].first_fail_row = UINT64_MAX; }
    u64 h_cells[3][4];
    std::vector<u64> h_code_off((size_t)b->n_bytecodes + 1);
    HostView views[4];
    int n_views = 0;
    bool views_ready = false, views_failed = false;
    { int erc = arena_event(device, &sh.ev_keccak); if (erc) return erc; }
    { int erc = arena_event(device, &sh.ev_cpa); if (erc) return erc; }
    { int erc = arena_event(device, &sh.ev_exa); if (erc) return erc; }
    auto enter = [&](int chain) {
        (void)zk_init(device);
        (void)zk_set_stream(g_block_stream[device][chain]);
        sh.start_ms[chain] = std::chrono::duration<double, std::milli>(std::chrono::steady_clock::now() - sh.t0).count();
        if (chain == 0) return true;
        std::unique_lock<std::mutex> lock(sh.m);
        sh.cv.wait(lock, [&] { return views_ready; });
        for (int k = 0; k < n_views; k++) t_host_view[k] = views[k];
        t_n_host_view = n_views;
        return !views_failed;
    };
    auto leave = [&](int chain, int rc) {
        t_n_host_view = 0;
        sh.rc[chain] = rc;
        if (rc) sh.err[chain] = g_err;
        sh.end_ms[chain] = std::chrono::duration<double, std::milli>(std::chrono::steady_clock::now() - sh.t0).count();
    };
    static const bool trace = [] { const char* e = getenv("ZK_BLOCK_TRACE"); return e && e[0] == '1'; }();
    struct Mark { int chain; const char* what; double ms; };
    std::vector<Mark> marks[4];
    auto mark = [&](int chain, const char* what) {
        if (trace) marks[chain].push_back(Mark{chain, what, std::chrono::duration<double, std::milli>(std::chrono::steady_clock::now() - sh.t0).count()});
    };
    const u64* bca_rows = nullptr;
    auto chain_state = [&] {
        enter(0);
        int rc = 0;
        zk_session *a = nullptr, *s = nullptr;
        uint64_t n_ops = 0, n_mpt = 0;
        zk_result ra;
        u32 n_mpt32 = 0;
        if (!(opts & (ZK_OPT_BLOCK_STATE_ROWS | ZK_OPT_STATE_COMPACT))) {
            BLK_TRY(zk_state_verify_from_rw_open(b->evm.rw, b->evm.rw_flags, b->evm.n_rw, dev_opts, &n_ops, &a));
            mark(0, "state opened (class scan + plan)");
            BLK_TRY(zk_launch(a, nullptr));
            mark(0, "state launched");
            BLK_TRY(zk_collect(a, &results[ZK_BLOCK_STATE]));
            mark(0, "state collected");
            goto done;
        }
        BLK_TRY(zk_state_assign_from_rw_open(b->evm.rw, b->evm.rw_flags, b->evm.n_rw, nullptr, nullptr, nullptr, st_opts, &n_ops, &a));
        BLK_TRY(zk_launch(a, nullptr));
        if (hipMemcpyAsync(&n_mpt32, a->assign.blk_cnt + a->assign.nb, 4, hipMemcpyDeviceToHost, a->stream) != hipSuccess) { rc = -2; g_err = "zk_block_verify: copy failed"; goto done; }
        BLK_TRY(zk_collect(a, &ra));
        if (ra.fail_count) { rc = -1; g_err = "zk_block_verify: the State witness assignment failed (zk_state_assign_from_rw reports the op)"; goto done; }
        n_mpt = n_mpt32;
        BLK_TRY(zk_state_open(a->assign.rows, a->assign.row_flags, n_ops, a->assign.mpt, n_mpt, st_opts, &s));
        BLK_TRY(block_run_pass(s, &results[ZK_BLOCK_STATE]));
    done:
        if (s) zk_close(s);
        if (a) zk_close(a);
        leave(0, rc);
    };
    auto chain_bytecode = [&] {
        const bool entered = enter(1);
        int rc = 0;
        zk_session *ks = nullptr, *bs = nullptr;
        zk_result rk;
        if (!entered) { rc = -2; g_err = "zk_block_verify: reading the block's randomness / offsets failed"; goto done; }
        if (b->n_codes) {
// ... 750 lines not shown
```

Measured before the change: 1.530 billion rows/s.

## Split EVM open onto high-priority side stream and defer RW generic index

Launches the RW key-pack kernel first on the main stream, then runs the fill, phase1 and phase2 open kernels on a per-slot high-priority side stream that joins the main stream lazily at launch or collect time. The RW sparse verdict moves to a per-session sequence-numbered buffer. The generic RW hash-index build is taken out of phase2 and enqueued only before the warm, cold or deferred kernels that need it. The aim is to overlap table setup with the hot EVM pass and keep the index build off the critical path. This adds stream and event management, and open timing is now attributed differently.

```diff
diff --git a/zkevm_specs_amd/csrc/cpu_backend.cpp b/zkevm_specs_amd/csrc/cpu_backend.cpp
--- a/zkevm_specs_amd/csrc/cpu_backend.cpp
+++ b/zkevm_specs_amd/csrc/cpu_backend.cpp
@@ -368,6 +368,8 @@
     EvmArgs& a = s->evm;
     s->a64[0].assign(t->steps, t->steps + t->n_steps * STEP_NCELLS * 4);
     a.dyn = nullptr;
+    a.verdict = nullptr;
+    a.verdict_seq = 0;
     a.step_recs = nullptr;
     a.defer_list = nullptr;
     a.defer_count = nullptr;
diff --git a/zkevm_specs_amd/csrc/evm_circuit.hpp b/zkevm_specs_amd/csrc/evm_circuit.hpp
--- a/zkevm_specs_amd/csrc/evm_circuit.hpp
+++ b/zkevm_specs_amd/csrc/evm_circuit.hpp
@@ -26,6 +26,10 @@
     u32 dir_entries;
     u32 n_deferred;
     u32 agg_rw_dups;
+};
+struct EvmVerdict {
+    unsigned long long sparse_seq;
+    u64 rw_base;
 };
 
 struct EvmArgs {
@@ -53,6 +57,8 @@
     u32 n_pairs;
     u32 opts;
     u32* defer_count_twin;
+    const EvmVerdict* verdict;
+    u64 verdict_seq;
 };
 
 ZK_HD void evm_args_resolve(EvmArgs& a) {
@@ -61,8 +67,14 @@
 #endif
     if (a.dyn) {
         const EvmDyn d = *a.dyn;
-        a.rw_dense = (a.rw.n != 0u && d.rw_sparse == 0u) ? 1u : 0u;
-        a.rw_base = d.rw_base;
+        if (a.verdict) {
+            const EvmVerdict v = *a.verdict;
+            a.rw_dense = (a.rw.n != 0u && v.sparse_seq != a.verdict_seq) ? 1u : 0u;
+            a.rw_base = v.rw_base;
+        } else {
+            a.rw_dense = (a.rw.n != 0u && d.rw_sparse == 0u) ? 1u : 0u;
+            a.rw_base = d.rw_base;
+        }
         a.codes.n = d.codes_n;
         a.codes.mask = d.codes_mask;
         a.agg_max_txs = d.agg_max_txs; a.agg_total_txs = d.agg_total_txs; a.agg_invalid_txs = d.agg_invalid_txs;
diff --git a/zkevm_specs_amd/csrc/zkevm_hip.hip b/zkevm_specs_amd/csrc/zkevm_hip.hip
--- a/zkevm_specs_amd/csrc/zkevm_hip.hip
+++ b/zkevm_specs_amd/csrc/zkevm_hip.hip
@@ -22,6 +22,7 @@
 static std::mutex g_dev_mutex;
 static hipStream_t g_own_stream[ZK_MAX_DEVICES] = {nullptr};
 static hipStream_t g_batch_stream[ZK_MAX_DEVICES][2] = {{nullptr}};
+static hipStream_t g_open_stream[ZK_MAX_DEVICES][3] = {{nullptr}};
 static hipStream_t g_side_stream[ZK_MAX_DEVICES] = {nullptr};
 
 static u32* g_secp_comb[ZK_MAX_DEVICES] = {nullptr};
@@ -71,6 +72,21 @@
         }
     return 0;
 }
+static int open_streams_ensure(int device, int first, int last) {
+    for (int c = first; c <= last; c++)
+        if (!g_open_stream[device][c]) {
+            int lo = 0, hi = 0;
+            (void)hipDeviceGetStreamPriorityRange(&lo, &hi);
+            static const bool flat = [] { const char* e = getenv("ZK_OPEN_PRIO"); return e && e[0] == 'n'; }();
+            if (flat) HIP_TRY(hipStreamCreateWithFlags(&g_open_stream[device][c], hipStreamNonBlocking));
+            else HIP_TRY(hipStreamCreateWithPriority(&g_open_stream[device][c], hipStreamNonBlocking, hi));
+        }
+    return 0;
+}
+static bool evm_open_split_enabled() {
+    static const bool split = [] { const char* e = getenv("ZK_OPEN_SPLIT"); return !(e && e[0] == '0'); }();
+    return split;
+}
 extern "C" int zk_init(int device) {
     int count = 0;
     HIP_TRY(hipGetDeviceCount(&count));
@@ -83,6 +99,7 @@
             HIP_TRY(hipStreamCreateWithFlags(&g_own_stream[device], hipStreamNonBlocking));
             static const bool lazy = [] { const char* e = getenv("ZK_BLOCK_STREAMS_LAZY"); return e && e[0] == '1'; }();
             if (!lazy) { int brc = block_streams_ensure(device); if (brc) return brc; }
+            if (evm_open_split_enabled()) { int orc = open_streams_ensure(device, 0, 0); if (orc) return orc; }
         }
         own = g_own_stream[device];
         if (!g_zero_row[device]) {
@@ -111,6 +128,10 @@
             }
             if (g_side_stream[d]) (void)hipStreamDestroy(g_side_stream[d]);
             g_side_stream[d] = nullptr;
+            for (int k = 0; k < 3; k++) {
+                if (g_open_stream[d][k]) (void)hipStreamDestroy(g_open_stream[d][k]);
+                g_open_stream[d][k] = nullptr;
+            }
             for (int k = 0; k < 4; k++) {
                 if (g_block_stream[d][k]) (void)hipStreamDestroy(g_block_stream[d][k]);
                 g_block_stream[d][k] = nullptr;
@@ -275,7 +296,7 @@
     for (u64 i = (u64)blockIdx.x * blockDim.x + threadIdx.x; i < n_ff; i += stride) ff[i] = F;
     for (u64 i = (u64)blockIdx.x * blockDim.x + threadIdx.x; i < n_zero; i += stride) zero[i] = Z;
 }
-__device__ __forceinline__ void rw_prepare_quad(const ZkTable& t, u64* keys, EvmDyn* dyn, u32 vthread) {
+__device__ __forceinline__ void rw_prepare_quad(const ZkTable& t, u64* keys, EvmDyn* dyn, EvmVerdict* v, u64 seq, u32 vthread) {
     const u32 r = vthread >> 2, q = vthread & 3u;
     const bool in = r < t.n;
     uint4 c0 = make_uint4(0, 0, 0, 0), c1 = c0, c2 = c0;
@@ -318,8 +339,13 @@
     const u32 qshift = threadIdx.x & 60u;
     const bool fits = ((__ballot(fit) >> qshift) & 0xfull) == 0xfull;
     const unsigned long long nd = __ballot(in && !dense_ok);
-    if (nd != 0ull && (threadIdx.x & 63u) == 0) atomicOr(&dyn->rw_sparse, 1u);
-    if (r == 0 && q == 0 && in) dyn->rw_base = base;
+    if (v) {
+        if (nd != 0ull && (threadIdx.x & 63u) == 0) atomicMax(&v->sparse_seq, (unsigned long long)seq);
+        if (r == 0 && q == 0 && in) v->rw_base = base;
+    } else {
+        if (nd != 0ull && (threadIdx.x & 63u) == 0) atomicOr(&dyn->rw_sparse, 1u);
+        if (r == 0 && q == 0 && in) dyn->rw_base = base;
+    }
 #pragma unroll
     for (int m = 1; m <= 2; m <<= 1) {
         w0 |= __shfl_xor(w0, m);
@@ -422,11 +448,38 @@
     if (b < o.dir_block0) evm_open_small_tables(o, b);
     else if (b < o.hist_block0) dirb_events_row(o.dir, (b - o.dir_block0) * blockDim.x + threadIdx.x);
     else if (b < o.rw_block0) evm_state_hist_body(b - o.hist_block0, o.sort.steps, o.sort.n_pairs, o.sort.hist, o.sort.taken, o.sort.bin16, o.sort.tally, o.sort.defer_count);
-    else if (b < o.rec_block0) rw_prepare_quad(o.rw, o.rw_keys, o.dyn, (b - o.rw_block0) * blockDim.x + threadIdx.x);
+    else if (b < o.rec_block0) rw_prepare_quad(o.rw, o.rw_keys, o.dyn, nullptr, 0ull, (b - o.rw_block0) * blockDim.x + threadIdx.x);
     else evm_step_record_quad(o.steps, o.n_steps, o.step_recs, (b - o.rec_block0) * blockDim.x + threadIdx.x);
+}
+__global__ __launch_bounds__(256) void evm_open_rw_pack_kernel(ZkTable rw, u64* keys, EvmVerdict* v, u64 seq, u32 force_sparse, u32 n_blocks) {
+    if (force_sparse && blockIdx.x == 0 && threadIdx.x == 0) atomicMax(&v->sparse_seq, (unsigned long long)seq);
+    if (!keys) return;
+    for (u32 vb = blockIdx.x; vb < n_blocks; vb += gridDim.x) rw_prepare_quad(rw, keys, nullptr, v, seq, vb * blockDim.x + threadIdx.x);
 }
 #define EVM_OPEN_RW_GENERIC_BLOCKS 64u
 #define EVM_OPEN_P2_BLOCK 1024u
+__device__ __forceinline__ void rw_generic_index_rows(const ZkTable& rw, EvmDyn* dyn, u32 first, u32 stride) {
+    u32* slots = const_cast<u32*>(rw.slots);
+    for (u32 r = first; r < rw.n; r += stride) {
+        u32 s = (u32)rw_key_hash(rw, r) & rw.mask;
+        bool dup = false;
+        for (;;) {
+            const u32 q = atomicCAS(&slots[s], ZK_EMPTY_SLOT, r);
+            if (q == ZK_EMPTY_SLOT) break;
+            if (!dup && q < rw.n) {
+                bool same = true;
+                for (int c = 0; c < RW_NCELLS && same; c++) same = fr_eq(zk_table_cell(rw, q, c), zk_table_cell(rw, r, c));
+                dup = same;
+            }
+            s = (s + 1) & rw.mask;
+        }
+        if (dup) atomicAdd(&dyn->agg_rw_dups, 1u);
+    }
+}
+__global__ __launch_bounds__(1024) void evm_rw_generic_index_kernel(ZkTable rw, EvmDyn* dyn, const EvmVerdict* v, u64 seq) {
+    if (v->sparse_seq != (unsigned long long)seq) return;
+    rw_generic_index_rows(rw, dyn, blockIdx.x * blockDim.x + threadIdx.x, gridDim.x * blockDim.x);
+}
 __global__ __launch_bounds__(1024) void evm_open_phase2_kernel(EvmOpenTables o, u32 scatter_blocks, u32 dir_blocks, u32 force_generic) {
     if (blockIdx.x < scatter_blocks) {
         evm_state_scatter_body(blockIdx.x, o.sort.bin16, o.sort.n_pairs, o.sort.hist, o.sort.hist_next, o.sort.taken, o.sort.group_start, o.sort.perm,
@@ -440,23 +493,7 @@
     }
     if (!force_generic && o.dyn->rw_sparse == 0u) return;
     if (force_generic && b == dir_blocks && threadIdx.x == 0) o.dyn->rw_sparse = 1u;
-    u32* slots = const_cast<u32*>(o.rw.slots);
-    const u32 stride = (gridDim.x - scatter_blocks - dir_blocks) * blockDim.x;
-    for (u32 r = (b - dir_blocks) * blockDim.x + threadIdx.x; r < o.rw.n; r += stride) {
-        u32 s = (u32)rw_key_hash(o.rw, r) & o.rw.mask;
-        bool dup = false;
-        for (;;) {
-            const u32 q = atomicCAS(&slots[s], ZK_EMPTY_SLOT, r);
-            if (q == ZK_EMPTY_SLOT) break;
-            if (!dup && q < o.rw.n) {
-                bool same = true;
-                for (int c = 0; c < RW_NCELLS && same; c++) same = fr_eq(zk_table_cell(o.rw, q, c), zk_table_cell(o.rw, r, c));
-                dup = same;
-            }
-            s = (s + 1) & o.rw.mask;
-        }
-        if (dup) atomicAdd(&o.dyn->agg_rw_dups, 1u);
-    }
+    rw_generic_index_rows(o.rw, o.dyn, (b - dir_blocks) * blockDim.x + threadIdx.x, (gridDim.x - scatter_blocks - dir_blocks) * blockDim.x);
 }
 
 __global__ void fr_op_kernel(int op, const u64* a, const u64* b, u64* out, u64 n) {
@@ -574,6 +611,10 @@
     u32* tail_status = nullptr;
     hipEvent_t tail_e1 = nullptr;
     bool stream_drained = false;
+    hipStream_t open_side = nullptr;
+    bool open_join_pending = false;
+    EvmVerdict* d_verdict = nullptr;
+    bool rw_index_pending = false;
 };
 
 static const int MAX_EVENT_PAIRS = 256;
@@ -593,6 +634,7 @@
     std::vector<void*> free_[ZK_ARENA_CLASSES];
     std::vector<hipEvent_t> events;
     std::vector<void*> pinned;
+    std::vector<void*> verdicts;
     size_t cached_bytes = 0;
 };
 static DevArena g_arena[ZK_MAX_DEVICES];
@@ -659,6 +701,20 @@
     HIP_TRY(hipHostMalloc(p, ZK_PINNED_BYTES, hipHostMallocDefault));
     return 0;
 }
+static int arena_verdict(int device, EvmVerdict** v) {
+    {
+        DevArena& A = g_arena[device];
+        std::lock_guard<std::mutex> lock(A.m);
+        if (!A.verdicts.empty()) {
+            *v = (EvmVerdict*)A.verdicts.back();
+            A.verdicts.pop_back();
+            return 0;
+        }
+    }
+    HIP_TRY(hipMalloc((void**)v, 256));
+    HIP_TRY(hipMemset(*v, 0, 256));
+    return 0;
+}
 static int arena_event(int device, hipEvent_t* e) {
     {
         DevArena& A = g_arena[device];
@@ -676,7 +732,7 @@
     for (int d = 0; d < ZK_MAX_DEVICES; d++) {
         DevArena& A = g_arena[d];
         std::lock_guard<std::mutex> lock(A.m);
-        bool any = !A.events.empty() || !A.pinned.empty();
+        bool any = !A.events.empty() || !A.pinned.empty() || !A.verdicts.empty();
         for (int c = 0; c < ZK_ARENA_CLASSES; c++) any = any || !A.free_[c].empty();
         if (!any || hipSetDevice(d) != hipSuccess) continue;
         for (int c = 0; c < ZK_ARENA_CLASSES; c++) {
@@ -687,6 +743,8 @@
         A.events.clear();
         for (void* h : A.pinned) (void)hipHostFree(h);
         A.pinned.clear();
+        for (void* v : A.verdicts) (void)hipFree(v);
+        A.verdicts.clear();
         A.cached_bytes = 0;
     }
 }
@@ -762,6 +820,7 @@
     if (!s) return 0;
     (void)hipSetDevice(s->device);
     if (!s->stream_drained) (void)hipStreamSynchronize(s->stream);
+    if (s->open_join_pending && s->open_side) (void)hipStreamSynchronize(s->open_side);
     for (size_t k = 0; k < s->owned.size(); k++) arena_give(s->device, s->owned[k], s->owned_class[k]);
     {
         DevArena& A = g_arena[s->device];
@@ -772,6 +831,7 @@
         if (s->ev_fork) A.events.push_back(s->ev_fork);
         if (s->ev_join) A.events.push_back(s->ev_join);
         if (s->h_result) A.pinned.push_back(s->h_result);
+        if (s->d_verdict) A.verdicts.push_back(s->d_verdict);
     }
     delete s;
     return 0;
@@ -864,6 +924,7 @@
     int rc = 0;
     const void* p = nullptr;
     EvmArgs& E = s->evm;
+    hipStream_t B = nullptr;
     if ((rc = stage(s, t->steps, (size_t)t->n_steps * STEP_NCELLS * 32, dev, &p))) goto fail;
     E.steps = (const u64*)p;
     E.n_steps = t->n_steps;
@@ -888,6 +949,38 @@
         E.aux = (const u64*)p;
         if ((rc = stage(s, t->aux_kind, (size_t)t->n_steps * 4, dev, &p))) goto fail;
         E.aux_kind = (const u32*)p;
+    }
+    E.rw_keys = nullptr;
+    E.verdict = nullptr;
+    E.verdict_seq = 0;
+    if (arena_event(s->device, &s->ev_open0) || arena_event(s->device, &s->ev_open1)) s->ev_open0 = s->ev_open1 = nullptr;
+    if ((opts & ZK_OPT_SINGLE_PASS) && !(opts & ZK_OPT_SIDE_STREAM) && evm_open_split_enabled() && s->ev_open0) {
+        int slot = 0;
+        for (int k = 0; k < 2; k++)
+            if (s->stream == g_batch_stream[s->device][k]) slot = 1 + k;
+        {
+            std::lock_guard<std::mutex> lock(g_dev_mutex);
+            rc = open_streams_ensure(s->device, slot, slot);
+        }
+        if (rc) goto fail;
+        B = g_open_stream[s->device][slot];
+        if ((rc = arena_verdict(s->device, &s->d_verdict))) goto fail;
+        static std::atomic<u64> g_verdict_seq{0};
+        E.verdict = s->d_verdict;
+        E.verdict_seq = ++g_verdict_seq;
+        if (t->n_rw && !generic) {
+            u64* d_keys = nullptr;
+            if ((rc = dev_alloc(s, (void**)&d_keys, (size_t)t->n_rw * 32))) goto fail;
+            E.rw_keys = d_keys;
+        }
+        const u32 pack_blocks = E.rw_keys ? (u32)((t->n_rw + 63) / 64) : 1u;
+        static const u32 pack_cap = [] { const char* e = getenv("ZK_PACK_GRID"); const int c = e ? atoi(e) : 0; return (u32)(c > 0 ? c : 0); }();
+        const u32 pack_grid = (pack_cap && pack_cap < pack_blocks) ? pack_cap : pack_blocks;
+        hipExtLaunchKernelGGL(evm_open_rw_pack_kernel, dim3(pack_grid), dim3(256), 0, s->stream, s->ev_open0, nullptr, 0, E.rw, const_cast<u64*>(E.rw_keys),
+                              s->d_verdict, E.verdict_seq, generic ? 1u : 0u, pack_blocks);
+        if (hipGetLastError() != hipSuccess || hipStreamWaitEvent(B, s->ev_open0, 0) != hipSuccess) {
+            rc = -2; g_err = "zk_evm_open: the RW pack failed to launch"; goto fail;
+        }
     }
     {
         ZkTable* const small[EVM_OPEN_TABLES] = {&E.tx, &E.block, &E.bytecode, &E.copy, &E.keccak, &E.exp, &E.sig, &E.ecc};
@@ -932,13 +1025,15 @@
         {
             const u64 n16 = n_ff / 4 + zero_bytes / 16;
             const u32 fill_grid = (u32)(n16 / 256 < 2048 ? (n16 + 255) / 256 : 2048);
-            if (arena_event(s->device, &s->ev_open0) || arena_event(s->device, &s->ev_open1)) s->ev_open0 = s->ev_open1 = nullptr;
-            hipExtLaunchKernelGGL(evm_open_fill_kernel, dim3(fill_grid ? fill_grid : 1u), dim3(256), 0, s->stream, s->ev_open0, nullptr, 0, (uint4*)ff,
-                                  (u64)(n_ff / 4), (uint4*)zero, (u64)(zero_bytes / 16));
+            if (B) {
+                s->open_side = B;
+                s->open_join_pending = true;
+            }
+            hipExtLaunchKernelGGL(evm_open_fill_kernel, dim3(fill_grid ? fill_grid : 1u), dim3(256), 0, B ? B : s->stream, B ? nullptr : s->ev_open0, nullptr, 0,
+                                  (uint4*)ff, (u64)(n_ff / 4), (uint4*)zero, (u64)(zero_bytes / 16));
         }
         E.rw_dense = 0;
         E.rw_base = 0;
-        E.rw_keys = nullptr;
         E.codes.n = 0;
         E.codes.mask = 0;
         E.codes.packed = nullptr;
@@ -957,7 +1052,7 @@
         o.dyn = dyn;
         o.tally = s->d_tally;
         o.rw = E.rw;
-        if (t->n_rw && !generic) {
+        if (t->n_rw && !generic && !B) {
             u64* d_keys = nullptr;
             if ((rc = dev_alloc(s, (void**)&d_keys, (size_t)t->n_rw * 32))) goto fail;
             E.rw_keys = d_keys;
@@ -1033,15 +1128,16 @@
 #endif
         {
             const u32 dir_blocks = want_dir ? DIRB_MAX_ENTRIES / EVM_OPEN_P2_BLOCK : 0u;
-            const u32 rw_blocks = t->n_rw ? EVM_OPEN_RW_GENERIC_BLOCKS : 0u;
+            const u32 rw_blocks = (t->n_rw && !B) ? EVM_OPEN_RW_GENERIC_BLOCKS : 0u;
+            s->rw_index_pending = t->n_rw && B;
             bool phase2 = scatter_blocks + dir_blocks + rw_blocks != 0;
 #ifdef ZK_DIAG_P1
             if (o.diag_skip) phase2 = false;
 #endif
-            hipExtLaunchKernelGGL(evm_open_phase1_kernel, dim3(grid1 ? grid1 : 1u), dim3(256), 0, s->stream, nullptr, phase2 ? nullptr : s->ev_open1, 0, o);
+            hipExtLaunchKernelGGL(evm_open_phase1_kernel, dim3(grid1 ? grid1 : 1u), dim3(256), 0, B ? B : s->stream, nullptr, phase2 ? nullptr : s->ev_open1, 0, o);
             if (phase2)
-                hipExtLaunchKernelGGL(evm_open_phase2_kernel, dim3(scatter_blocks + dir_blocks + rw_blocks), dim3(EVM_OPEN_P2_BLOCK), 0, s->stream, nullptr,
-                                      s->ev_open1, 0, o, scatter_blocks, dir_blocks, generic ? 1u : 0u);
+                hipExtLaunchKernelGGL(evm_open_phase2_kernel, dim3(scatter_blocks + dir_blocks + rw_blocks), dim3(EVM_OPEN_P2_BLOCK), 0, B ? B : s->stream, nullptr,
+                                      s->ev_open1, 0, o, scatter_blocks, dir_blocks, (generic && !B) ? 1u : 0u);
         }
         if (hipGetLastError() != hipSuccess) { rc = -2; g_err = "zk_evm_open: a build kernel failed to launch"; goto fail; }
     }
@@ -1099,6 +1195,7 @@
         std::lock_guard<std::mutex> lock(g_dev_mutex);
         for (int k = 0; k < 2; k++)
             if (!g_batch_stream[t_device][k]) HIP_TRY(hipStreamCreateWithFlags(&g_batch_stream[t_device][k], hipStreamNonBlocking));
+        if (evm_open_split_enabled()) { int orc = open_streams_ensure(t_device, 1, 2); if (orc) return orc; }
     }
     const hipStream_t caller = t_stream;
     HIP_TRY(hipStreamSynchronize(caller));
@@ -2471,6 +2568,18 @@
     return 0;
 }
 
+static int evm_join_open(zk_session* s) {
+    if (!s->open_join_pending) return 0;
+    HIP_TRY(hipStreamWaitEvent(s->stream, s->ev_open1, 0));
+    s->open_join_pending = false;
+    return 0;
+}
+static void evm_enqueue_rw_index(zk_session* s) {
+    if (!s->rw_index_pending) return;
+    s->rw_index_pending = false;
+    hipLaunchKernelGGL(evm_rw_generic_index_kernel, dim3(EVM_OPEN_RW_GENERIC_BLOCKS), dim3(EVM_OPEN_P2_BLOCK), 0, s->stream, s->evm.rw, const_cast<EvmDyn*>(s->evm.dyn),
+                       s->evm.verdict, s->evm.verdict_seq);
+}
 static int evm_enqueue_tail(zk_session* s) {
     if (s->kind != SESSION_EVM || !s->tail_pending) return 0;
     s->tail_pending = false;
@@ -2496,6 +2605,7 @@
         s->evm_cold_empty = !run_cold;
     }
     s->early_seq = 0;
+    if (run_warm || run_cold) evm_enqueue_rw_index(s);
     if (run_warm) zk_launch_evm_warm(s->stream, s->tail_cold_grid, warm_lanes, s->evm, s->d_group_start, s->tail_status, s->tally_last, run_cold ? nullptr : s->tail_e1);
     if (run_cold) zk_launch_evm_cold(s->stream, s->tail_cold_grid, s->evm, s->d_group_start, s->tail_status, s->tally_last, s->tail_e1);
     HIP_TRY(hipGetLastError());
@@ -2506,6 +2616,7 @@
     ARG_TRY(s, "zk_launch: null session");
     s->stream_drained = false;
     HIP_TRY(hipSetDevice(s->device));
+    { int jrc = evm_join_open(s); if (jrc) return jrc; }
     { int trc = evm_enqueue_tail(s); if (trc) return trc; }
     s->publish_enqueued = false;
     s->status_external = status_dev != nullptr;
@@ -2651,6 +2762,7 @@
         }
         hipEvent_t e_hot1 = (evm_ext_events && !run_warm && !run_cold) ? e1 : nullptr;
         zk_launch_evm_hot(s->stream, grid, s->evm, s->d_group_start, status, s->tally_last, evm_ext_events ? e0 : nullptr, e_hot1);
+        if (run_warm || run_cold || (status_dev && s->evm.defer_count)) evm_enqueue_rw_index(s);
         if (run_warm)
             zk_launch_evm_warm(s->stream, cold_grid, (sorted && s->evm_ranges_known) ? s->evm_warm_lanes : 0u, s->evm, s->d_group_start, status, s->tally_last,
                                (evm_ext_events && !run_cold) ? e1 : nullptr);
@@ -2669,6 +2781,7 @@
 }
 
 static int evm_finish_deferred(zk_session* s) {
+    if (s->kind == SESSION_EVM) { int jrc = evm_join_open(s); if (jrc) return jrc; }
     { int trc = evm_enqueue_tail(s); if (trc) return trc; }
     if (s->kind != SESSION_EVM || !s->deferred_pending || !s->evm.defer_count) return 0;
     u32 n_def = 0;
@@ -2677,6 +2790,7 @@
     s->deferred_pending = false;
     if (n_def) {
         s->stream_drained = false;
+        evm_enqueue_rw_index(s);
         zk_launch_evm_deferred(s->stream, s->evm, s->last_status, s->tally_last);
         HIP_TRY(hipGetLastError());
     }
@@ -2695,6 +2809,7 @@
 extern "C" int zk_collect(zk_session* s, zk_result* r) {
     ARG_TRY(s && r, "zk_collect: bad arguments");
     HIP_TRY(hipSetDevice(s->device));
+    if (s->kind == SESSION_EVM) { int jrc = evm_join_open(s); if (jrc) return jrc; }
     { int trc = evm_enqueue_tail(s); if (trc) return trc; }
     ZkTally t;
     u32 n_def = 0;
@@ -2762,7 +2877,8 @@
         s->deferred_pending = false;
         if (n_def) {
             s->stream_drained = false;
-        zk_launch_evm_deferred(s->stream, s->evm, s->last_status, s->tally_last);
+            evm_enqueue_rw_index(s);
+            zk_launch_evm_deferred(s->stream, s->evm, s->last_status, s->tally_last);
             HIP_TRY(hipGetLastError());
             HIP_TRY(hipMemcpyAsync(&t, s->tally_last, sizeof t, hipMemcpyDeviceToHost, s->stream));
             HIP_TRY(hipStreamSynchronize(s->stream));
@@ -2805,8 +2921,12 @@
     *open_ms = *span_ms = -1.0;
     if (s->kind != SESSION_EVM || !s->ev_open0 || !s->ev_open1) return;
     float f = 0;
-    if (hipEventElapsedTime(&f, s->ev_open0, s->ev_open1) == hipSuccess) *open_ms = f;
+    if (s->open_side) {
+        if (s->ev.size() >= 2 && hipEventElapsedTime(&f, s->ev_open0, s->ev[0]) == hipSuccess) *open_ms = f;
+    } else if (hipEventElapsedTime(&f, s->ev_open0, s->ev_open1) == hipSuccess) *open_ms = f;
     if (pass_ms > 0 && s->ev.size() >= 2 && hipEventElapsedTime(&f, s->ev_open0, s->ev[1]) == hipSuccess) *span_ms = f;
+    if (s->open_side && *open_ms >= 0 && *span_ms >= 0 && hipEventElapsedTime(&f, s->ev[0], s->ev[1]) == hipSuccess && *open_ms + (double)f > *span_ms)
+        *open_ms = *span_ms - (double)f;
     (void)hipGetLastError();
 }
 extern "C" int zk_session_timing(zk_session* s, double* open_ms, double* span_ms) {
```

New measurement: 1.472 billion rows/s. 3.8% lower.
